# clintpgeorge/LDAGroupedGibbsSampler

Measured on AMD Instinct MI355X. Metric: M tokens sampled/sec (whole node) per Gibbs sweep at K=100, higher is better.
Workload: dtype f64

## Files before the change

### ldagroupedgibbssampler_amd/csrc/ggs_api.hip

```cpp
#include <hip/hip_runtime.h>

#include <algorithm>
#include <cmath>
#include <cstdio>
#include <cstdlib>
#include <cstring>
#include <new>
#include <string>
#include <vector>

#include "ggs_kernels.hpp"
#include "ggs_z_sliced.hpp"
#include "ggs_z_stream.hpp"
#include "ggs_exact_sum.hpp"
#include "ggs_z_pcgs.hpp"
#include "ggs_z_pcgs_wave.hpp"
#include "ggs_z_collapsed.hpp"
#include "ggs_phi_poisson.hpp"
#include "ggs_alias.hpp"
#include "ggs_z_spalias.hpp"
#include "ggs_loglik.hpp"
#include "ggs_heldout.hpp"
#include "ggs_exchange.hpp"
#include "ggs_corpus_lists.hpp"

using namespace ggs;

namespace {

const char *debug_env(const char *name) {
  static const bool enabled = [] { const char *e = std::getenv("GGS_DEBUG"); return e && std::atoi(e) == 1; }();
  return enabled ? std::getenv(name) : nullptr;
}

struct Knob {
  bool set = false;
  int v = 0;
  double f = 0;
  explicit Knob(const char *name) { if (const char *e = debug_env(name)) { set = true; v = std::atoi(e); f = std::atof(e); } }
  bool is(int x) const { return set && v == x; }
};
struct Knobs {
  Knob zkernel{"GGS_DEBUG_ZKERNEL"}, group{"GGS_DEBUG_GROUP"}, regck{"GGS_DEBUG_REGCK"}, tworows{"GGS_DEBUG_TWOROWS"}, wpc{"GGS_DEBUG_WPC"};
  Knob phi64{"GGS_DEBUG_PHI64"}, split{"GGS_DEBUG_SPLIT"}, hot{"GGS_DEBUG_HOT"}, tile{"GGS_DEBUG_TILE"};
  Knob warm{"GGS_DEBUG_WARM"}, warm_rows{"GGS_DEBUG_WARM_ROWS"}, warm_fill{"GGS_DEBUG_WARM_FILL"}, warm_cpw{"GGS_DEBUG_WARM_CPW"};
  Knob theta_b{"GGS_DEBUG_THETA_B"}, theta_wgs{"GGS_DEBUG_THETA_WGS"}, zparts{"GGS_DEBUG_ZPARTS"}, beside{"GGS_DEBUG_BESIDE"};
  Knob pcgs_wave{"GGS_DEBUG_PCGS_WAVE"}, pcgs_stream{"GGS_DEBUG_PCGS_STREAM"};
  Knob margin{"GGS_DEBUG_MARGIN"}, replays{"GGS_DEBUG_REPLAYS"}, chain{"GGS_DEBUG_CHAIN"}, guided{"GGS_DEBUG_GUIDED"};
  Knob no_overlap{"GGS_DEBUG_NO_OVERLAP"}, theta_main{"GGS_DEBUG_THETA_MAIN"}, gamma_queue{"GGS_DEBUG_GAMMA_QUEUE"};
};

constexpr int kThetaBlock = 256;

struct KernelLaunch {
  const void *fn = nullptr;
  int block = 64, lds = 0, per_cu = 0;
};
struct LaunchPlan {
  int32_t kernel = 0;
  bool sliced() const { return kernel == 1; }
  bool stream() const { return kernel >= 2; }
  KernelLaunch z;
  int32_t tile_tokens = 64;
  bool two_rows = false;
  KernelLaunch cold, hot, warm;
  bool f32 = false;
  bool split = true, split_forced = false;
  int32_t wave_lds = 0, ring_base = 0, hot_wave_lds = 0, warm_wave_lds = 0, hot_pitch = 0, Kp32 = 0;
  int32_t hot_cap = 0, warm_cap = 0, warm_docs = 0;
  int32_t warm_tiers_max = 3, warm_min_fill_pct = 40, warm_min_chunks_per_wave = 3;
  struct ZCfg { int32_t parts = 1, z_per_cu = 0, theta_docs = 0, theta_lds = 0, theta_lds_beside_z = 0; } cfg_plain, cfg_parts;
  bool parts_forced = false;
  KernelLaunch theta;
  int32_t theta_docs_main = 0, theta_lds_main = 0;
  KernelLaunch lane, wave, alias, spalias, serial;
  bool wave_forced = false;
  int32_t alias_wpb = 0;
  std::vector<const KernelLaunch *> all() const { return {&z, &cold, &hot, &warm, &theta, &lane, &wave, &alias, &spalias, &serial}; }
};

constexpr int kEvRing = 8;
struct Events {
  hipEvent_t e[6] = {nullptr, nullptr, nullptr, nullptr, nullptr, nullptr};
  hipEvent_t x[3] = {nullptr, nullptr, nullptr};
  hipEvent_t th0 = nullptr, th1 = nullptr;
  bool used_ahead = false, exchanged = false;
  bool e4_is_e3 = false;
  bool theta_on_main = false;
  bool light = false;
};

}

struct ggs_handle {
  int32_t K = 0, V = 0, Kp = 0, pitch16 = 0, device = 0;
  double beta = 0;
  std::vector<double> alpha;
  uint64_t seed = 0;
  int32_t flags = 0, phi_burn_in = 0, phi_thin = 1;
  int32_t iteration = 0;
  int32_t n_sampled_phi = 0;

  int64_t D = 0, N = 0, C = 0, S = 0, doc_base = 0, tok_base = 0, global_tokens = -1;
  bool have_corpus = false, have_phi = false, in_sweep = false;
  int32_t num_cus = 0;
  LaunchPlan plan;
  const LaunchPlan::ZCfg *cfg = nullptr;
  int32_t *d_chunk_doc1 = nullptr;
  double margin_scale = 1.0;
  double margin_scale32 = 1.0;

  hipStream_t stream = nullptr;
  int64_t *d_doc_ptr = nullptr, *d_chunk_start = nullptr;
  int32_t *d_tok = nullptr, *d_z = nullptr, *d_chunk_doc = nullptr, *d_chunk_len = nullptr;
  int32_t *d_ct_tok = nullptr, *d_ct_idx = nullptr, *d_ct_ip = nullptr, *d_c_docs = nullptr, *d_hot_words = nullptr;
  int64_t Cs = 0, Cc = 0;
  int32_t *d_order = nullptr;
  int64_t pcgs_order_len = 0;
  bool pcgs_wave = false;
  bool collapsed = false;
  bool polyaurn = false;
  int32_t pa_L = 0;
  double pa_t00 = 0;
  double *d_pa_table = nullptr;
  unsigned long long *d_pa_acc = nullptr;
  bool spalias = false;
  bool alias_stale = true;
  double *d_alias_ps = nullptr, *d_alias_tn = nullptr;
  int32_t *d_alias_a = nullptr;
  KernelLaunch sp_z;
  int32_t sp_cap = 0;
  uint64_t *d_lcg = nullptr;
  bool lcg_ready = false;
  int32_t num_hot = 0;
  int32_t *d_perm = nullptr, *d_inv_perm = nullptr, *d_zw = nullptr, *d_seg_word = nullptr, *d_seg_begin = nullptr;
  double *d_theta_next = nullptr;
  hipStream_t side = nullptr;
  hipStream_t side_hot = nullptr;
  hipEvent_t ev_hot_fork = nullptr, ev_hot_join = nullptr;
  bool theta_main = true, chain_on_side = false, theta_main_always = false;
  bool whole_sweep = false;
  hipEvent_t hot_fork_from = nullptr;
  hipEvent_t ev_chain_done = nullptr;
  bool z_split = true, z_split_tried = false;
  int32_t warm_tiers = 0, num_warm = 0, warm_rows_max = 0;
  int64_t Cw = 0, warm_chunks_max = 0;
  int32_t *d_wt_pack = nullptr, *d_w_docs = nullptr, *d_warm_words = nullptr;
  int32_t *d_ht_pack = nullptr, *d_h_docs = nullptr;
  int64_t *d_warm_meta = nullptr;
  bool overlap_theta = true;
  int32_t gamma_queue_cap = 1 << 20;
  std::vector<int64_t> part_doc, part_chunk;
  hipEvent_t ev_part[8] = {nullptr, nullptr, nullptr, nullptr, nullptr, nullptr, nullptr, nullptr};
  int64_t theta_ahead_iter = INT64_MIN;
  float *d_phiT32 = nullptr;
  unsigned long long *d_replays = nullptr;
  int64_t z_f32_launches = 0;
  double *d_alpha = nullptr, *d_theta = nullptr, *d_phiT = nullptr, *d_mag = nullptr, *d_tot = nullptr, *d_phi_mean = nullptr;
  int32_t *d_n_wk = nullptr, *d_n_k = nullptr;
  double *d_sum_pref = nullptr, *d_sum_fn = nullptr;
  int32_t sum_nseg = 0;
  bool exact_sum = true;
  bool sum_guided = true;
  const void *guess_src = nullptr;
  int32_t guess_cols = 0;
  uint32_t *d_status = nullptr;
  int64_t *d_test_ptr = nullptr;
  int32_t *d_test_tok = nullptr, *d_test_docs = nullptr;
  std::vector<int32_t> test_short, test_long, test_huge;
  void *d_heldout_spill = nullptr;
  size_t heldout_spill_bytes = 0;
  double *d_test_ll = nullptr;
  std::vector<int64_t> test_ptr;
  int64_t test_doc_base = 0;
  bool have_test = false;
  void *d_scratch = nullptr;
  size_t scratch_bytes = 0;

  Exchange *xg = nullptr;
  hipStream_t own_stream = nullptr;
  int32_t Ks = 0, Ksm = 0, k0 = 0;
  int64_t *d_koff = nullptr;
  int32_t *d_cnt_send = nullptr, *d_cnt_own = nullptr, *d_cnt_all = nullptr, *d_n_k_own = nullptr;
  double *d_phi_own = nullptr, *d_phi_all0 = nullptr, *d_phi_all1 = nullptr, *d_mag_own = nullptr;
  int32_t *d_krank = nullptr, *d_kcol = nullptr;
  int32_t seg_split = 0, v_split = 0;
  hipStream_t comm_stream = nullptr;
  hipEvent_t ev_half_drawn = nullptr, ev_half_gathered = nullptr;
  int32_t *d_hseg_word = nullptr, *d_hseg_begin = nullptr, *d_hseg_end = nullptr;
  int64_t HS = 0;
  int32_t detail_every = 4;
  bool force_detail = false;
  int64_t sweeps_enqueued = 0;
  bool have_frac = false;
  double frac[5] = {0, 0, 0, 0, 0};
  int32_t count_mode = 0;
  bool counted_sparse = false;
  bool in_group = false;
  int64_t *d_sp_count = nullptr;
  int32_t *d_sp_cnt32 = nullptr, *d_sp_all = nullptr;
  int32_t *d_sp_wg_count = nullptr;
  int64_t *d_sp_wg_off = nullptr;
  int64_t sp_wgs = 0;
  int32_t *d_sp_send = nullptr, *d_sp_recv = nullptr;
  size_t sp_send_cap = 0, sp_recv_cap = 0;
  int64_t sp_pairs_last = 0;
  bool hot_join_pending = false, hot_counted = false;
  bool z_counted = false;
  bool cnt_send_zeroed = false;
  bool z_counts_forced = false;
  bool z_counts = true;
  SliceMap smap{};
  bool counts_global = true;
  bool cnt_own_valid = false;
  bool n_k_valid = false;
  std::vector<ggs_handle *> group;

  std::vector<void **> owned;
  Events evs[kEvRing];
  int ev_head = 0, ev_pending = 0;
  ggs_timings tm{};
  std::string err;
};

namespace {

int set_err(ggs_handle *h, int code, const std::string &msg) {
  if (h) h->err = msg;
  return code;
}

#define HIP_TRY(h, expr)                                                                        \
  do {                                                                                          \
    hipError_t _e = (expr);                                                                     \
    if (_e != hipSuccess)                                                                       \
      return set_err((h), GGS_ERR_HIP, std::string(#expr) + ": " + hipGetErrorString(_e));      \
  } while (0)

int bind_device(ggs_handle *h) {
  HIP_TRY(h, hipSetDevice(h->device));
  return GGS_OK;
}

template <typename T>
int dev_alloc(ggs_handle *h, T **p, size_t count) {
  void **slot = reinterpret_cast<void **>(p);
  if (std::find(h->owned.begin(), h->owned.end(), slot) == h->owned.end()) h->owned.push_back(slot);
  if (*p) { (void)hipFree(*p); *p = nullptr; }
  HIP_TRY(h, hipMalloc(slot, std::max<size_t>(count, 1) * sizeof(T)));
  return GGS_OK;
}
template <typename T>
int upload(ggs_handle *h, T **p, const T *src, size_t count) {
  const int rc = dev_alloc(h, p, count);
  if (rc) return rc;
  if (count) HIP_TRY(h, hipMemcpy(*p, src, sizeof(T) * count, hipMemcpyHostToDevice));
  return GGS_OK;
}
template <typename T>
int upload(ggs_handle *h, T **p, const std::vector<T> &v) { return upload(h, p, v.data(), v.size()); }

hipError_t launch(const ggs_handle *h, const KernelLaunch &l, int64_t items, void **args, hipStream_t st, int table_lds = 0) {
  const int waves = l.block / 64;
  const int64_t grid = std::max<int64_t>(1, std::min<int64_t>((items + waves - 1) / waves, (int64_t)h->num_cus * l.per_cu));
  return hipLaunchKernel(l.fn, dim3((unsigned)grid), dim3((unsigned)l.block), args, (size_t)(l.lds + table_lds), st);
}

void build_poisson_table(double beta, int32_t L, std::vector<double> &T) {
  const int n = 2 * L;
  T.assign((size_t)L * n, 0.0);
  std::vector<double> S((size_t)n);
  for (int32_t c = 0; c < L; ++c) {
    const double lambda = beta + (double)c;
    double pj = std::exp(-lambda), acc = 0.0;
    for (int j = 0; j < n; ++j) {
      if (j > 0) pj = pj * lambda / (double)j;
      acc += pj;
      S[(size_t)j] = acc;
    }
    for (int j = 0; j < n - 1; ++j) T[(size_t)c * n + j] = S[(size_t)j] / S[(size_t)n - 1];
    T[(size_t)c * n + n - 1] = 1.0;
  }
}

int ensure_scratch(ggs_handle *h, size_t bytes) {
  if (h->scratch_bytes >= bytes) return GGS_OK;
  if (h->d_scratch) (void)hipFree(h->d_scratch);
  h->d_scratch = nullptr; h->scratch_bytes = 0;
  HIP_TRY(h, hipMalloc(&h->d_scratch, bytes));
  h->scratch_bytes = bytes;
  return GGS_OK;
}

int grid_for(int64_t n, int block, int per_thread = 1) {
  const int64_t want = (n + (int64_t)block * per_thread - 1) / ((int64_t)block * per_thread);
  return (int)std::max<int64_t>(1, std::min<int64_t>(want, 256 * 8));
}

int check_status(ggs_handle *h) {
  uint32_t st = 0;
  HIP_TRY(h, hipMemcpyAsync(&st, h->d_status, sizeof st, hipMemcpyDeviceToHost, h->stream));
  HIP_TRY(h, hipStreamSynchronize(h->stream));
  if (!st) return GGS_OK;
  HIP_TRY(h, hipMemsetAsync(h->d_status, 0, sizeof(uint32_t), h->stream));
  if (st & ST_INVALID_TOPIC)
    return set_err(h, GGS_ERR_INVALID_TOPIC, h->collapsed ? "SimpleLDA: New topic not sampled."  : "LDAGroupedGibbsSampler: Topic sampled is invalid!");
  if (st & ST_NEGATIVE_COUNT) return set_err(h, GGS_ERR_NEGATIVE_COUNT, "Negative count for topic (Invalid count!)");
  if (st & ST_BAD_SHAPE) return set_err(h, GGS_ERR_BAD_ARG, "alpha and beta must be strictly positive (gamma shape <= 0)");
// ... 276 lines not shown
  pp.rows_per_tile = (int32_t)std::max<int64_t>(1, std::min<int64_t>(rows, (want + Ks - 1) / Ks));
  const int64_t tiles = (rows + pp.rows_per_tile - 1) / pp.rows_per_tile;
  hipLaunchKernelGGL(phi_poisson_kernel, dim3((unsigned)std::min<int64_t>(tiles, (int64_t)h->num_cus * 2)), dim3(kPoissonThreads), (size_t)Ks * 12, h->stream, pp);
  HIP_TRY(h, hipGetLastError());
  return GGS_OK;
}
int phi_slice_poisson_totals(ggs_handle *h, int32_t Ks, double *tot, int32_t *n_k) {
  if (Ks <= 0) return GGS_OK;
  hipLaunchKernelGGL(phi_poisson_totals_kernel, dim3((unsigned)((Ks + 255) / 256)), dim3(256), 0, h->stream, h->d_pa_acc, Ks, tot, n_k);
  HIP_TRY(h, hipGetLastError());
  return GGS_OK;
}
int launch_phi_slice(ggs_handle *h, bool initial, const int32_t *cnt, int32_t cnt_pitch, int32_t Ks, int32_t k0, double *out, int32_t out_pitch,
                     double *mag, double *tot, int32_t *n_k, double *phi_mean) {
  if (Ks <= 0) return GGS_OK;
  int rc;
  if (h->polyaurn) {
    if ((rc = phi_slice_poisson(h, initial, cnt, cnt_pitch, Ks, k0, out, out_pitch, 0, h->sum_nseg, true)) || (rc = phi_slice_poisson_totals(h, Ks, tot, n_k)))
      return rc;
    hipLaunchKernelGGL(phi_normalise_polyaurn_kernel, dim3(grid_for((int64_t)Ks * h->V, 256, 2)), dim3(256), 0, h->stream, out, tot, Ks, out_pitch, h->V,
                       phi_mean, out == h->d_phiT ? h->d_phiT32 : nullptr, h->plan.Kp32);
    HIP_TRY(h, hipGetLastError());
    return GGS_OK;
  }
  if ((rc = launch_magnitude_on(h, cnt, cnt_pitch, Ks, mag, n_k)) || (rc = phi_slice_gamma(h, initial, cnt, cnt_pitch, Ks, k0, out, out_pitch, mag, 0, h->sum_nseg)) ||
      (rc = phi_slice_total(h, out, out_pitch, Ks, tot)))
    return rc;
  hipLaunchKernelGGL(phi_normalise_kernel, dim3(grid_for((int64_t)Ks * h->V, 256, 2)), dim3(256), 0, h->stream, out, tot, Ks, out_pitch, h->V, phi_mean,
                     out == h->d_phiT ? h->d_phiT32 : nullptr, h->plan.Kp32);
  HIP_TRY(h, hipGetLastError());
  return GGS_OK;
}

size_t half0_elems(const ggs_handle *h) { return (size_t)h->v_split * h->Ksm; }
size_t half1_elems(const ggs_handle *h) { return (size_t)(h->V - h->v_split) * h->Ksm + (size_t)h->Ksm; }
int phi_step_a(ggs_handle *h) { return exchange_reduce_scatter(h); }
int phi_step_a_clear(ggs_handle *h) { return h->seg_split > 0 ? GGS_OK : clear_send_buffer_if_dead(h, h->stream); }
int phi_step_b1(ggs_handle *h, bool initial) {
  int rc;
  if (h->polyaurn) {
    if ((rc = phi_slice_poisson(h, initial, h->d_cnt_own, h->Ksm, h->Ks, h->k0, h->d_phi_own, h->Ksm, 0, h->seg_split, true))) return rc;
  } else if ((rc = launch_magnitude_on(h, h->d_cnt_own, h->Ksm, h->Ks, h->d_mag_own, h->d_n_k_own))) {
    return rc;
  }
  if (h->seg_split > 0) {
    if (!h->polyaurn && (rc = phi_slice_gamma(h, initial, h->d_cnt_own, h->Ksm, h->Ks, h->k0, h->d_phi_own, h->Ksm, h->d_mag_own, 0, h->seg_split))) return rc;
    HIP_TRY(h, hipEventRecord(h->ev_half_drawn, h->stream));
    HIP_TRY(h, hipStreamWaitEvent(h->comm_stream, h->ev_half_drawn, 0));
  }
  return GGS_OK;
}
int phi_step_g0(ggs_handle *h) {
  if (h->seg_split <= 0) return GGS_OK;
  return xcall(h, h->xg->ops.all_gather_f64(h->xg->ops.ctx, h->d_phi_own, h->d_phi_all0, (int64_t)half0_elems(h), h->comm_stream), "all_gather_f64");
}
int phi_step_b2(ggs_handle *h, bool initial) {
  int rc;
  if (h->seg_split > 0) {
    if ((rc = clear_send_buffer_if_dead(h, h->comm_stream))) return rc;
    HIP_TRY(h, hipEventRecord(h->ev_half_gathered, h->comm_stream));
  }
  if (h->polyaurn) {
    if ((rc = phi_slice_poisson(h, initial, h->d_cnt_own, h->Ksm, h->Ks, h->k0, h->d_phi_own, h->Ksm, h->seg_split, h->sum_nseg, false))) return rc;
    return phi_slice_poisson_totals(h, h->Ks, h->d_phi_own + (size_t)h->V * h->Ksm, h->d_n_k_own);
  }
  if ((rc = phi_slice_gamma(h, initial, h->d_cnt_own, h->Ksm, h->Ks, h->k0, h->d_phi_own, h->Ksm, h->d_mag_own, h->seg_split, h->sum_nseg))) return rc;
  return phi_slice_total(h, h->d_phi_own, h->Ksm, h->Ks, h->d_phi_own + (size_t)h->V * h->Ksm);
}
int phi_step_g1(ggs_handle *h) {
  return xcall(h, h->xg->ops.all_gather_f64(h->xg->ops.ctx, h->d_phi_own + half0_elems(h), h->d_phi_all1, (int64_t)half1_elems(h), h->stream), "all_gather_f64");
}
int phi_join_halves(ggs_handle *h) {
  if (h->seg_split > 0) HIP_TRY(h, hipStreamWaitEvent(h->stream, h->ev_half_gathered, 0));
  return GGS_OK;
}
int phi_step_c(ggs_handle *h, bool accumulate_mean) {
  PhiRepackParams rp{};
  rp.all0 = h->d_phi_all0; rp.all1 = h->d_phi_all1; rp.krank = h->d_krank; rp.kcol = h->d_kcol; rp.phiT = h->d_phiT;
  rp.phi_mean = accumulate_mean ? h->d_phi_mean : nullptr;
  rp.c0 = (int64_t)half0_elems(h); rp.c1 = (int64_t)half1_elems(h); rp.K = h->K; rp.Kp = h->Kp; rp.V = h->V; rp.Ksm = h->Ksm; rp.v_split = h->v_split;
  rp.phiT32 = h->d_phiT32; rp.Kp32 = h->plan.Kp32;
  if (h->polyaurn) hipLaunchKernelGGL(phi_repack_polyaurn_kernel, dim3(grid_for((int64_t)h->K * h->V, 256, 2)), dim3(256), 0, h->stream, rp);
  else hipLaunchKernelGGL(phi_repack_kernel, dim3(grid_for((int64_t)h->K * h->V, 256, 2)), dim3(256), 0, h->stream, rp);
  HIP_TRY(h, hipGetLastError());
  h->have_phi = true;
  h->alias_stale = true;
  return GGS_OK;
}

int launch_alias_build(ggs_handle *h) {
  if (!h->spalias) return GGS_OK;
  AliasParams ap{};
  ap.phiT = h->d_phiT; ap.alpha = h->d_alpha; ap.ps = h->d_alias_ps; ap.a = h->d_alias_a; ap.type_norm = h->d_alias_tn;
  ap.V = h->V; ap.K = h->K; ap.Kp = h->Kp; ap.wpb = h->plan.alias_wpb;
  void *args[] = {&ap};
  HIP_TRY(h, launch(h, h->plan.alias, ((int64_t)h->V + ap.wpb - 1) / ap.wpb, args, h->stream));
  h->alias_stale = false;
  return GGS_OK;
}

int launch_phi(ggs_handle *h, bool initial, bool accumulate_mean, Events *E = nullptr) {
  int rc;
  if (h->xg) {
    if ((rc = phi_step_a(h)) || (rc = phi_step_a_clear(h))) return rc;
    if (E) HIP_TRY(h, hipEventRecord(E->x[0], h->stream));
    if ((rc = phi_step_b1(h, initial)) || (rc = phi_step_g0(h)) || (rc = phi_step_b2(h, initial))) return rc;
    if (E) HIP_TRY(h, hipEventRecord(E->x[1], h->stream));
    if ((rc = phi_join_halves(h)) || (rc = phi_step_g1(h))) return rc;
    if (E) HIP_TRY(h, hipEventRecord(E->x[2], h->stream));
    if ((rc = phi_step_c(h, accumulate_mean))) return rc;
    return launch_alias_build(h);
  }
  if ((rc = launch_phi_slice(h, initial, h->d_n_wk, h->K, h->K, 0, h->d_phiT, h->Kp, h->d_mag, h->d_tot, h->d_n_k, accumulate_mean ? h->d_phi_mean : nullptr)))
    return rc;
  h->n_k_valid = true;
  h->have_phi = true;
  return launch_alias_build(h);
}

int launch_theta(ggs_handle *h, hipStream_t stream, double *dst, int32_t iteration, int64_t d0 = 0, int64_t d1 = -1, int32_t lds = 0, int32_t docs_per_block = 0) {
  if (d1 < 0) d1 = h->D;
  if (d1 <= d0) return GGS_OK;
  if (docs_per_block <= 0) docs_per_block = h->cfg->theta_docs;
  ThetaParams tp{};
  tp.doc_ptr = h->d_doc_ptr + d0; tp.z = h->d_z; tp.alpha = h->d_alpha; tp.theta = dst + (size_t)d0 * h->K; tp.status = h->d_status;
  tp.num_docs = d1 - d0; tp.doc_base = h->doc_base + d0; tp.seed = h->seed; tp.iteration = (uint32_t)iteration;
  tp.K = h->K; tp.docs_per_block = docs_per_block; tp.queue_cap = std::min(kGammaQueue, h->gamma_queue_cap);
  const int64_t grid = (d1 - d0 + docs_per_block - 1) / docs_per_block;
  void *args[] = {&tp};
  HIP_TRY(h, hipLaunchKernel(h->plan.theta.fn, dim3((unsigned)grid), dim3(kThetaBlock), args, (size_t)(lds ? lds : h->cfg->theta_lds), stream));
  return GGS_OK;
}

#define GGS_KMAX_SWITCH(KERNEL)                                                                                                     \
  switch ((K + 7) / 8) {                                                                                                            \
    case 1: return reinterpret_cast<const void *>(KERNEL<8>);      case 2: return reinterpret_cast<const void *>(KERNEL<16>);       \
    case 3: return reinterpret_cast<const void *>(KERNEL<24>);     case 4: return reinterpret_cast<const void *>(KERNEL<32>);       \
    case 5: return reinterpret_cast<const void *>(KERNEL<40>);     case 6: return reinterpret_cast<const void *>(KERNEL<48>);       \
    case 7: return reinterpret_cast<const void *>(KERNEL<56>);     case 8: return reinterpret_cast<const void *>(KERNEL<64>);       \
    case 9: return reinterpret_cast<const void *>(KERNEL<72>);     case 10: return reinterpret_cast<const void *>(KERNEL<80>);      \
    case 11: return reinterpret_cast<const void *>(KERNEL<88>);    case 12: return reinterpret_cast<const void *>(KERNEL<96>);      \
    case 13: return reinterpret_cast<const void *>(KERNEL<104>);   case 14: return reinterpret_cast<const void *>(KERNEL<112>);     \
    case 15: return reinterpret_cast<const void *>(KERNEL<120>);   case 16: return reinterpret_cast<const void *>(KERNEL<128>);     \
    case 17: return reinterpret_cast<const void *>(KERNEL<136>);   case 18: return reinterpret_cast<const void *>(KERNEL<144>);     \
    case 19: return reinterpret_cast<const void *>(KERNEL<152>);   case 20: return reinterpret_cast<const void *>(KERNEL<160>);     \
    case 21: return reinterpret_cast<const void *>(KERNEL<168>);   case 22: return reinterpret_cast<const void *>(KERNEL<176>);     \
    case 23: return reinterpret_cast<const void *>(KERNEL<184>);   default: return reinterpret_cast<const void *>(KERNEL<192>);     \
  }
const void *sliced_kernel_for(int K) { GGS_KMAX_SWITCH(z_sliced_kernel) }
const void *sliced32_kernel_for(int K) { GGS_KMAX_SWITCH(z_sliced32_kernel) }

const void *hot_kernel_for(int K) { GGS_KMAX_SWITCH(z_hot_kernel) }
const void *warm_kernel_for(int K) { GGS_KMAX_SWITCH(z_warm_kernel) }
const void *pcgs_kernel_for(int K) { GGS_KMAX_SWITCH(pcgs_sliced_kernel) }
const void *polyaurn_kernel_for(int K) { GGS_KMAX_SWITCH(polyaurn_sliced_kernel) }
const void *collapsed_kernel_for(int K) {
  switch ((K + 7) / 8) {
#define GGS_CK(N) case N: return reinterpret_cast<const void *>(pcgs_sliced_kernel<8 * N, true>);
    GGS_CK(1) GGS_CK(2) GGS_CK(3) GGS_CK(4) GGS_CK(5) GGS_CK(6) GGS_CK(7) GGS_CK(8) GGS_CK(9) GGS_CK(10) GGS_CK(11) GGS_CK(12)
    GGS_CK(13) GGS_CK(14) GGS_CK(15) GGS_CK(16) GGS_CK(17) GGS_CK(18) GGS_CK(19) GGS_CK(20) GGS_CK(21) GGS_CK(22) GGS_CK(23)
#undef GGS_CK
    default: return reinterpret_cast<const void *>(pcgs_sliced_kernel<192, true>);
  }
}

const void *pcgs_wave_kernel_for(int nb, bool collapsed, bool polyaurn) {
#define GGS_WK(N) if (nb <= N) return polyaurn ? reinterpret_cast<const void *>(polyaurn_wave_kernel<N>) : collapsed ? reinterpret_cast<const void *>(pcgs_wave_kernel<N, true>) : reinterpret_cast<const void *>(pcgs_wave_kernel<N, false>);
  GGS_WK(1) GGS_WK(2) GGS_WK(4) GGS_WK(8) GGS_WK(16)
#undef GGS_WK
  return polyaurn ? reinterpret_cast<const void *>(polyaurn_wave_kernel<32>) : collapsed ? reinterpret_cast<const void *>(pcgs_wave_kernel<32, true>) : reinterpret_cast<const void *>(pcgs_wave_kernel<32, false>);
}
constexpr int kPcgsWaveMaxTopics = 32 * 128;
constexpr int kPcgsWaveFromTopics = 176, kCollapsedWaveFromTopics = 96;
constexpr int kPolyaurnWaveFromTopics = 168;

const void *tile_kernel_for(int K) {
  const int nt = (K + 63) / 64;
  return nt <= 1 ? reinterpret_cast<const void *>(z_kernel<1>) : nt <= 2 ? reinterpret_cast<const void *>(z_kernel<2>)
       : nt <= 4 ? reinterpret_cast<const void *>(z_kernel<4>) : nt <= 8 ? reinterpret_cast<const void *>(z_kernel<8>)
       : nt <= 16 ? reinterpret_cast<const void *>(z_kernel<16>) : reinterpret_cast<const void *>(z_kernel<20>);
}
const void *stream_kernel_for(bool two_pass, bool regck, int group) {
  if (two_pass) return reinterpret_cast<const void *>(z_stream_kernel);
  if (!regck) return reinterpret_cast<const void *>(z_stream1_kernel<false, 4>);
  return group == 1 ? reinterpret_cast<const void *>(z_stream1_kernel<true, 1>) : group == 2 ? reinterpret_cast<const void *>(z_stream1_kernel<true, 2>)
                                                                                             : reinterpret_cast<const void *>(z_stream1_kernel<true, 4>);
}
const void *pcgs_lane_kernel_for(int K, bool sliced, bool collapsed, bool polyaurn) {
  if (sliced) return collapsed ? collapsed_kernel_for(K) : polyaurn ? polyaurn_kernel_for(K) : pcgs_kernel_for(K);
  return collapsed ? reinterpret_cast<const void *>(pcgs_z_kernel<true>) : polyaurn ? reinterpret_cast<const void *>(polyaurn_z_kernel) : reinterpret_cast<const void *>(pcgs_z_kernel<false>);
}

int plan_launches(const int K, const int V, const int32_t flags, const Knobs &kn, LaunchPlan &pl) {
  const bool pcgs = (flags & GGS_FLAG_PCGS) != 0, collapsed = (flags & GGS_FLAG_COLLAPSED) != 0, polyaurn = (flags & GGS_FLAG_POLYAURN) != 0;
  const int Kp = (K + 1) & ~1, pitch16 = (Kp / 2) | 1;
  const bool sliced_ok = K <= kSlicedMaxTopics && V < (1 << kSlotShift);
  bool sliced = sliced_ok && K <= kSlicedDefaultTopics, stream = !sliced && K > 2 * kSliceTopics, two_pass = false;
  if (kn.zkernel.set) {
    const int mode = kn.zkernel.v;
    sliced = sliced_ok && mode == 1;
    stream = (mode == 2 || mode == 3) ? K > 2 * kSliceTopics : (stream && mode != 0);
    two_pass = mode == 3;
    if (sliced) stream = false;
  }
  pl.kernel = sliced ? 1 : stream ? (two_pass ? 3 : 2) : 0;
  if (stream) {
    const int ns = stream_slices(K);
    int group = ns <= kRegCheckpoints ? 1 : ns <= 2 * kRegCheckpoints ? 2 : 4;
    if (kn.group.set && (kn.group.v == 1 || kn.group.v == 2 || kn.group.v == 4)) group = kn.group.v;
    bool regck = !two_pass && z_stream1_groups(K, group) <= kRegCheckpoints;
    if (kn.regck.set) regck = regck && kn.regck.v != 0;
    if (!regck) group = 4;
    pl.two_rows = !two_pass && (kn.tworows.set ? kn.tworows.v != 0 : K <= 512);
    pl.z.fn = stream_kernel_for(two_pass, regck, group);
    pl.z.lds = two_pass ? z_stream_lds_bytes(K) : z_stream1_lds_bytes(K, group, pl.two_rows, regck);
    if (pl.z.lds > kMaxLdsBytes) return GGS_ERR_UNSUPPORTED;
  } else if (sliced) {
    pl.f32 = !kn.phi64.is(1);
    pl.Kp32 = round_up(K, kSlice32Topics);
    pl.ring_base = sliced_ring_base(K); pl.wave_lds = sliced_wave_lds(K); pl.hot_pitch = table_row_pitch(K);
    pl.hot_wave_lds = hot_wave_lds(K); pl.warm_wave_lds = warm_wave_lds(K);
    if (kn.split.set) { pl.split = kn.split.v != 0; pl.split_forced = kn.split.v == 2; }
    pl.hot_cap = pl.split ? table_rows_beside_cold(K, pl.hot_wave_lds) : table_rows_fused(K);
    if (kn.hot.set) pl.hot_cap = std::max(0, std::min(pl.hot_cap, kn.hot.v));
    pl.cold = {pl.f32 ? sliced32_kernel_for(K) : sliced_kernel_for(K), kSlicedWaves * 64, sliced_cold_lds(K), 1};
    pl.hot = {hot_kernel_for(K), kSlicedWaves * 64, table_lds(K, pl.hot_wave_lds, 0), 1};
    pl.warm = {warm_kernel_for(K), kSlicedWaves * 64, table_lds(K, pl.warm_wave_lds, 0), 1};
    pl.warm_docs = warm_docs_for(sliced_kmax(K));
    pl.warm_cap = table_rows_beside_cold(K, pl.warm_wave_lds);
    if (pl.warm_cap < 16) pl.warm_cap = 0;
    if (kn.warm.set) pl.warm_tiers_max = std::max(0, std::min(kWarmMaxTiers, kn.warm.v));
    if (kn.warm_rows.set) pl.warm_cap = std::max(0, std::min(pl.warm_cap, kn.warm_rows.v));
    if (kn.warm_fill.set) pl.warm_min_fill_pct = std::max(1, std::min(100, kn.warm_fill.v));
    if (kn.warm_cpw.set) pl.warm_min_chunks_per_wave = std::max(0, kn.warm_cpw.v);
  } else {
    int T = z_tile_rows_in(kMaxLdsBytes / 6 / kLdsGranule * kLdsGranule, Kp, pitch16);
    if (kn.tile.set) T = kn.tile.v;
    pl.tile_tokens = std::max(8, std::min(64, T));
    pl.z.fn = tile_kernel_for(K);
    pl.z.lds = z_tile_lds_bytes(Kp, pitch16, pl.tile_tokens);
    if (pl.z.lds > kMaxLdsBytes) return GGS_ERR_UNSUPPORTED;
  }
  if (!sliced) {
    pl.z.per_cu = lds_workgroups_per_cu(pl.z.lds, 8);
    if (kn.wpc.set) pl.z.per_cu = std::max(1, kn.wpc.v);
  }

  int B = 64;
  while (B > 1 && theta_lds_bytes(K, B) > 32 * 1024) B >>= 1;
  if (theta_lds_bytes(K, B) > kMaxLdsBytes) return GGS_ERR_UNSUPPORTED;
  pl.theta.fn = reinterpret_cast<const void *>(theta_kernel<kThetaBlock>); pl.theta.block = kThetaBlock;
  const int theta_quarter = (kMaxLdsBytes - 24 * 1024) / 4;
  pl.cfg_plain = {1, pl.z.per_cu, B, std::max(theta_lds_bytes(K, B), theta_quarter), 0};
  pl.theta_docs_main = kn.theta_b.set ? std::max(1, std::min(B, kn.theta_b.v)) : std::min(B, 16);
  pl.theta_lds_main = std::max(theta_lds_bytes(K, pl.theta_docs_main), (kMaxLdsBytes - 24 * 1024) / (kn.theta_wgs.set ? std::max(1, kn.theta_wgs.v) : 5));
  pl.parts_forced = kn.zparts.set;
  int parts = kn.zparts.set ? std::max(1, std::min(8, kn.zparts.v)) : (stream && !two_pass && !pcgs) ? 8 : 1;
  pl.cfg_parts = pl.cfg_plain;
  if (parts > 1 && stream && !two_pass) {
    const int kBeside = kn.beside.set ? std::max(1, kn.beside.v) : 4;
    int Bt = 64;
    while (Bt > 1 && theta_lds_bytes(K, Bt) > 10 * 1024) Bt >>= 1;
    const int t_lds = theta_lds_bytes(K, Bt), z_alloc = lds_alloc_of(pl.z.lds);
    const int zw = std::min(pl.z.per_cu, (kMaxLdsBytes - kLdsGranule - kBeside * lds_alloc_of(t_lds)) / z_alloc);
    if (t_lds <= 12 * 1024 && zw >= 2)
      pl.cfg_parts = {parts, zw, Bt, std::max(t_lds, theta_quarter), std::max(t_lds, (kMaxLdsBytes - kLdsGranule - zw * z_alloc) / kBeside / kLdsGranule * kLdsGranule)};
    else
      parts = 1;
  }
  pl.cfg_parts.parts = parts;
  if (!pcgs) return GGS_OK;

  if (K <= kPcgsWaveMaxTopics) {
    const int nb = pcgs_wave_blocks(Kp);
    pl.wave.fn = pcgs_wave_kernel_for(nb, collapsed, polyaurn);
    pl.wave.lds = pcgs_wave_lds_bytes(nb);
    int by_regs = 0;
    if (hipOccupancyMaxActiveBlocksPerMultiprocessor(&by_regs, pl.wave.fn, 64, (size_t)pl.wave.lds) != hipSuccess || by_regs < 1) by_regs = 1;
    pl.wave.per_cu = lds_workgroups_per_cu(pl.wave.lds, std::min(by_regs, 32));
  }
  pl.wave_forced = kn.pcgs_wave.set ? kn.pcgs_wave.v != 0 : K > (collapsed ? kCollapsedWaveFromTopics : polyaurn ? kPolyaurnWaveFromTopics : kPcgsWaveFromTopics);
  if (pl.wave_forced && !pl.wave.fn) return GGS_ERR_UNSUPPORTED;
  const bool lane_sliced = K <= kSlicedMaxTopics && !(kn.pcgs_stream.set && kn.pcgs_stream.v != 0);
  pl.lane.lds = lane_sliced ? pcgs_sliced_lds_bytes(K) : pcgs_z_lds_bytes(K);
  if (pl.lane.lds > kMaxLdsBytes && !pl.wave_forced) return GGS_ERR_UNSUPPORTED;
  pl.lane.per_cu = lds_workgroups_per_cu(pl.lane.lds, 8);
  if (!pl.wave_forced) pl.lane.fn = pcgs_lane_kernel_for(K, lane_sliced, collapsed, polyaurn);
  if (collapsed) pl.serial.fn = reinterpret_cast<const void *>(collapsed_serial_kernel);
  if (flags & GGS_FLAG_SPALIAS) {
    pl.alias_wpb = alias_words_per_block(K);
    pl.alias = {reinterpret_cast<const void *>(alias_build_kernel), 64, (int)alias_lds_bytes(K, pl.alias_wpb), 0};
    pl.alias.per_cu = lds_workgroups_per_cu(pl.alias.lds, 16);
    pl.spalias.fn = reinterpret_cast<const void *>(spalias_wave_kernel);
  }
  return GGS_OK;
}

int launch_pcgs_z(ggs_handle *h) {
  if (h->N == 0) return GGS_OK;
  PcgsParams pp{};
  pp.tok = h->d_tok; pp.inv_perm = h->d_inv_perm; pp.z = h->d_z; pp.zw = h->d_zw; pp.doc_ptr = h->d_doc_ptr; pp.order = h->d_order;
  pp.alpha = h->d_alpha; pp.phiT = h->d_phiT; pp.status = h->d_status;
  pp.num_docs = h->pcgs_order_len; pp.tok_base = h->tok_base; pp.seed = h->seed; pp.iteration = (uint32_t)h->iteration;
  pp.K = h->K; pp.Kp = h->Kp;
  int rc;
  if (h->spalias) {
    if (h->alias_stale && (rc = launch_alias_build(h))) return rc;
    SpaliasParams sp{};
    sp.b = pp; sp.ps = h->d_alias_ps; sp.a = h->d_alias_a; sp.type_norm = h->d_alias_tn; sp.cap = h->sp_cap; sp.margin_scale = h->margin_scale;
    void *args[] = {&sp};
    HIP_TRY(h, launch(h, h->sp_z, h->pcgs_order_len, args, h->stream));
    return GGS_OK;
  }
  if (h->collapsed) {
    if ((rc = launch_magnitude(h))) return rc;
    pp.n_wk = h->d_n_wk; pp.n_k = h->d_n_k; pp.beta = h->beta; pp.beta_sum = h->beta * (double)h->V;
    hipLaunchKernelGGL(psi_kernel, dim3(grid_for((int64_t)h->K * h->V, 256, 2)), dim3(256), 0, h->stream, h->d_n_wk, h->d_n_k, pp.beta, pp.beta_sum, h->d_phiT,
                       h->K, h->Kp, h->V);
    HIP_TRY(h, hipGetLastError());
  }
  void *wave_args[] = {&pp, &h->margin_scale}, *lane_args[] = {&pp};
  if (h->pcgs_wave) HIP_TRY(h, launch(h, h->plan.wave, h->pcgs_order_len, wave_args, h->stream));
  else HIP_TRY(h, launch(h, h->plan.lane, (h->pcgs_order_len + 63) / 64, lane_args, h->stream));
  return GGS_OK;
}

bool z_counts_itself(const ggs_handle *h) {
  return h->xg && h->z_counts && h->plan.sliced() && !(h->flags & GGS_FLAG_PCGS) && (h->z_counts_forced || h->N <= (int64_t)64 * h->V) && !use_sparse(h);
}
int launch_count_hot(ggs_handle *h);
int launch_z(ggs_handle *h, bool force_fused = false, int64_t c0 = 0, int64_t c1 = -1, bool count = false, bool defer_join = false) {
  h->hot_join_pending = false;
  if (h->C == 0) return GGS_OK;
  if (c1 < 0) c1 = h->C;
  if (c1 <= c0) return GGS_OK;
  const LaunchPlan &pl = h->plan;
  ZParams zp{};
  zp.tok = h->d_tok; zp.inv_perm = h->d_inv_perm; zp.z = h->d_z; zp.zw = h->d_zw; zp.chunk_start = h->d_chunk_start; zp.chunk_doc = h->d_chunk_doc; zp.chunk_len = h->d_chunk_len;
  zp.theta = h->d_theta; zp.phiT = h->d_phiT; zp.status = h->d_status;
  zp.tok_base = h->tok_base; zp.seed = h->seed; zp.iteration = (uint32_t)h->iteration;
  zp.K = h->K; zp.Kp = h->Kp; zp.pitch16 = h->pitch16; zp.tile_tokens = pl.tile_tokens;
  zp.num_chunks = h->C;
  zp.margin_scale = h->margin_scale;
  zp.chunk_doc1 = h->d_chunk_doc1; zp.two_rows = (pl.two_rows && h->d_chunk_doc1) ? 1 : 0;
  zp.ct_tok = h->d_ct_tok; zp.ct_idx = h->d_ct_idx; zp.ct_ip = h->d_ct_ip; zp.c_docs = h->d_c_docs; zp.num_cold = h->Cc;
  zp.hot_words = h->d_hot_words; zp.num_hot = h->num_hot; zp.hot_pitch = pl.hot_pitch;
  zp.wave_lds = pl.wave_lds; zp.hot_off = kSlicedWaves * pl.wave_lds; zp.ring_base = pl.ring_base;
  zp.cnt_send = (count && z_counts_itself(h)) ? h->d_cnt_send : nullptr;
  zp.smap = h->smap;
  zp.ht_pack = reinterpret_cast<const int4 *>(h->d_ht_pack); zp.h_docs = h->d_h_docs;
  zp.wt_pack = reinterpret_cast<const int4 *>(h->d_wt_pack); zp.w_docs = h->d_w_docs; zp.warm_words = h->d_warm_words;
  zp.warm_meta = h->d_warm_meta; zp.warm_tiers = h->warm_tiers; zp.warm_rows = pl.warm_cap;
  zp.phiT32 = h->d_phiT32; zp.Kp32 = pl.Kp32; zp.replays = h->d_replays; zp.margin_scale32 = h->margin_scale32;
  void *args[] = {&zp};
  if (!pl.sliced()) {
    zp.chunk_start += c0; zp.chunk_doc += c0; zp.chunk_len += c0; zp.num_chunks = c1 - c0;
    if (zp.chunk_doc1) zp.chunk_doc1 += c0;
    KernelLaunch z = pl.z;
    z.per_cu = h->cfg->z_per_cu;
    HIP_TRY(h, launch(h, z, zp.num_chunks, args, h->stream));
    return GGS_OK;
  }
  zp.num_chunks = h->Cs;
  const int hot_rows_lds = h->num_hot * pl.hot_pitch;
  ZParams wp = zp;
  wp.wave_lds = pl.warm_wave_lds; wp.hot_off = kSlicedWaves * pl.warm_wave_lds;
  void *wargs[] = {&wp};
  auto launch_warm = [&](hipStream_t st) { return h->Cw == 0 ? hipSuccess : launch(h, pl.warm, h->warm_chunks_max, wargs, st, h->warm_rows_max * pl.hot_pitch); };
  if (h->z_split && !force_fused && h->Cs > h->Cc && h->Cc > 0) {
    ZParams hp = zp;
    hp.wave_lds = pl.hot_wave_lds; hp.hot_off = kSlicedWaves * pl.hot_wave_lds;
    void *hargs[] = {&hp};
    if (h->hot_fork_from) {
      HIP_TRY(h, hipStreamWaitEvent(h->side_hot, h->hot_fork_from, 0));
    } else {
      HIP_TRY(h, hipEventRecord(h->ev_hot_fork, h->stream));
      HIP_TRY(h, hipStreamWaitEvent(h->side_hot, h->ev_hot_fork, 0));
    }
    zp.num_chunks = h->Cc; zp.num_hot = 0;
    HIP_TRY(h, launch(h, pl.cold, h->Cc, args, h->stream));
    HIP_TRY(h, launch(h, pl.hot, h->Cs - h->Cc, hargs, h->side_hot, hot_rows_lds));
    HIP_TRY(h, launch_warm(h->side_hot));
    if (defer_join && zp.cnt_send) {
      hipStream_t main_stream = h->stream;
      h->stream = h->side_hot;
      const int rc = launch_count_hot(h);
      h->stream = main_stream;
      if (rc) return rc;
      h->hot_counted = true;
    }
    HIP_TRY(h, hipEventRecord(h->ev_hot_join, h->side_hot));
    if (defer_join) h->hot_join_pending = true;
    else HIP_TRY(h, hipStreamWaitEvent(h->stream, h->ev_hot_join, 0));
  } else {
    HIP_TRY(h, launch(h, pl.cold, std::max(h->Cc, h->Cs - h->Cc), args, h->stream, hot_rows_lds));
    HIP_TRY(h, launch_warm(h->stream));
  }
  if (pl.f32) ++h->z_f32_launches;
  return GGS_OK;
}

bool sample_phi_this_iteration(const ggs_handle *h) {
  return h->phi_burn_in > 0 && h->iteration > h->phi_burn_in && (h->iteration % h->phi_thin) == 0;
}

uint64_t java_lcg_next_ints(int32_t seed, int32_t bound, int64_t n, int32_t *out) {
  constexpr uint64_t kMult = 0x5DEECE66DULL, kMask = (1ULL << 48) - 1;
  uint64_t s = ((uint64_t)(int64_t)seed ^ kMult) & kMask;
  auto next31 = [&]() { s = (s * kMult + 0xBULL) & kMask; return (int32_t)(s >> 17); };
  const int32_t m = bound - 1;
  for (int64_t i = 0; i < n; ++i) {
    int32_t r = next31();
    if ((bound & m) == 0) r = (int32_t)(((int64_t)bound * (int64_t)r) >> 31);
    else
      for (int32_t u = r;; u = next31()) {
        r = u % bound;
        if ((int32_t)((uint32_t)u - (uint32_t)r + (uint32_t)m) >= 0) break;
      }
    out[i] = r;
  }
  return s;
}

int require_ready(ggs_handle *h, bool need_phi) {
  if (!h) return GGS_ERR_BAD_ARG;
  if (!h->have_corpus) return set_err(h, GGS_ERR_STATE, "no corpus: call ggs_set_corpus first");
  if (need_phi && !h->have_phi) return set_err(h, GGS_ERR_STATE, "no Phi: call ggs_init_phi / ggs_set_z / ggs_set_phi first");
  return bind_device(h);
}

int drop_theta_ahead(ggs_handle *h) {
  if (h->side) HIP_TRY(h, hipStreamSynchronize(h->side));
  h->theta_ahead_iter = INT64_MIN;
  return GGS_OK;
}

int settle_sweeps(ggs_handle *h) {
  HIP_TRY(h, hipStreamSynchronize(h->stream));
  for (int j = h->ev_pending - 1; j >= 0; --j) {
    const Events &E = h->evs[((h->ev_head - j) % kEvRing + kEvRing) % kEvRing];
    float ms = 0;
    if (E.used_ahead && E.theta_on_main) { HIP_TRY(h, hipEventElapsedTime(&ms, h->evs[((h->ev_head - j - 1) % kEvRing + kEvRing) % kEvRing].e[2], E.th1)); }
    else if (E.used_ahead) { HIP_TRY(h, hipEventElapsedTime(&ms, E.th0, E.th1)); }
    else { HIP_TRY(h, hipEventElapsedTime(&ms, E.e[0], E.e[1])); }
    h->tm.theta_ms += ms;
    HIP_TRY(h, hipEventElapsedTime(&ms, E.e[1], E.e[2])); h->tm.z_ms += ms;
    if (E.light) {
      HIP_TRY(h, hipEventElapsedTime(&ms, E.e[2], E.e[5]));
      h->tm.merge_ms += ms * h->frac[0];
      h->tm.exchange_rs_ms += ms * h->frac[1]; h->tm.exchange_ag_ms += ms * h->frac[3]; h->tm.exchange_ms += ms * (h->frac[1] + h->frac[3]);
      h->tm.phi_ms += ms * (h->frac[2] + h->frac[4]);
      h->tm.sweeps += 1;
      h->tm.tokens_sampled += h->N;
      continue;
    }
    HIP_TRY(h, hipEventElapsedTime(&ms, E.e[2], E.e[3])); h->tm.merge_ms += ms;
    if (E.exchanged) {
      float span = 0, part[5] = {ms, 0, 0, 0, 0};
      (void)hipEventElapsedTime(&span, E.e[2], E.e[5]);
      (void)hipEventElapsedTime(&part[1], E.e[E.e4_is_e3 ? 3 : 4], E.x[0]); (void)hipEventElapsedTime(&part[2], E.x[0], E.x[1]);
      (void)hipEventElapsedTime(&part[3], E.x[1], E.x[2]); (void)hipEventElapsedTime(&part[4], E.x[2], E.e[5]);
      if (span > 0) {
        const float sum = part[0] + part[1] + part[2] + part[3] + part[4];
        for (int q = 0; q < 5; ++q) h->frac[q] = sum > 0 ? part[q] / sum : 0.0;
        h->have_frac = true;
      }
      HIP_TRY(h, hipEventElapsedTime(&ms, E.e[E.e4_is_e3 ? 3 : 4], E.x[0])); h->tm.exchange_ms += ms; h->tm.exchange_rs_ms += ms;
      HIP_TRY(h, hipEventElapsedTime(&ms, E.x[0], E.x[1])); h->tm.phi_ms += ms;
      HIP_TRY(h, hipEventElapsedTime(&ms, E.x[1], E.x[2])); h->tm.exchange_ms += ms; h->tm.exchange_ag_ms += ms;
      HIP_TRY(h, hipEventElapsedTime(&ms, E.x[2], E.e[5])); h->tm.phi_ms += ms;
    } else {
      HIP_TRY(h, hipEventElapsedTime(&ms, E.e[E.e4_is_e3 ? 3 : 4], E.e[5])); h->tm.phi_ms += ms;
    }
    h->tm.sweeps += 1;
    h->tm.tokens_sampled += h->N;
  }
  h->ev_pending = 0;
  return GGS_OK;
}

struct StreamSwap {
  ggs_handle *h;
  hipStream_t user;
  StreamSwap(ggs_handle *h_, hipStream_t s) : h(h_), user(h_->stream) { h->stream = s; }
  ~StreamSwap() { h->stream = user; }
};

int z_phase(ggs_handle *h) {
  int rc;
  if (h->ev_pending >= kEvRing - 2 && (rc = settle_sweeps(h))) return rc;
  h->ev_head = (h->ev_head + 1) % kEvRing;
  Events &E = h->evs[h->ev_head];
  E.light = h->xg && h->have_frac && h->detail_every > 1 && !h->force_detail && (h->sweeps_enqueued % h->detail_every) != 0 && !h->collapsed;
  h->sweeps_enqueued += 1;
  if (h->flags & GGS_FLAG_PCGS) {
    E.used_ahead = false;
    HIP_TRY(h, hipEventRecord(E.e[0], h->stream));
    HIP_TRY(h, hipEventRecord(E.e[1], h->stream));
    if ((rc = launch_pcgs_z(h))) return rc;
    HIP_TRY(h, hipEventRecord(E.e[2], h->stream));
    if ((rc = launch_count_rebuild(h))) return rc;
    if (!E.light) HIP_TRY(h, hipEventRecord(E.e[3], h->stream));
    return GGS_OK;
  }
  E.used_ahead = h->theta_ahead_iter == (int64_t)h->iteration;
  h->hot_fork_from = nullptr;
  if (E.used_ahead) {
    if (E.theta_on_main) h->hot_fork_from = E.th1;
    else HIP_TRY(h, hipStreamWaitEvent(h->stream, E.th1, 0));
    std::swap(h->d_theta, h->d_theta_next);
  } else {
    E.theta_on_main = false;
    if (h->side) HIP_TRY(h, hipStreamSynchronize(h->side));
    HIP_TRY(h, hipEventRecord(E.e[0], h->stream));
    if ((rc = launch_theta(h, h->stream, h->d_theta, h->iteration))) return rc;
  }
  HIP_TRY(h, hipEventRecord(E.e[1], h->stream));
  if (h->plan.sliced() && h->z_split && !h->z_split_tried && h->Cs > h->Cc && h->Cc > 0) {
    h->z_split_tried = true;
    float t_split = 0, t_fused = 0;
    hipEvent_t t0 = nullptr, t1 = nullptr, t2 = nullptr;
    if (hipEventCreate(&t0) != hipSuccess || hipEventCreate(&t1) != hipSuccess || hipEventCreate(&t2) != hipSuccess) return set_err(h, GGS_ERR_HIP, "hipEventCreate");
    if ((rc = launch_z(h, false)) || (rc = launch_z(h, true))) return rc;
    HIP_TRY(h, hipEventRecord(t0, h->stream));
    if ((rc = launch_z(h, false))) return rc;
    HIP_TRY(h, hipEventRecord(t1, h->stream));
    if ((rc = launch_z(h, true))) return rc;
    HIP_TRY(h, hipEventRecord(t2, h->stream));
    HIP_TRY(h, hipEventSynchronize(t2));
    HIP_TRY(h, hipEventElapsedTime(&t_split, t0, t1));
    HIP_TRY(h, hipEventElapsedTime(&t_fused, t1, t2));
    (void)hipEventDestroy(t0); (void)hipEventDestroy(t1); (void)hipEventDestroy(t2);
    if (t_fused < t_split) h->z_split = false;
    HIP_TRY(h, hipEventRecord(E.e[1], h->stream));
  }
  if (!h->hot_fork_from) h->hot_fork_from = E.e[1];
  h->theta_ahead_iter = INT64_MIN;
  const bool ahead = h->overlap_theta && h->side && h->D > 0;
  const int32_t P = (int32_t)h->part_doc.size() - 1;
  if (ahead && P > 1 && h->plan.stream()) {
    Events &N = h->evs[(h->ev_head + 1) % kEvRing];
    for (int32_t p = 0; p < P; ++p) {
      if ((rc = launch_z(h, false, h->part_chunk[(size_t)p], h->part_chunk[(size_t)p + 1]))) return rc;
      HIP_TRY(h, hipEventRecord(h->ev_part[p], h->stream));
      HIP_TRY(h, hipStreamWaitEvent(h->side, h->ev_part[p], 0));
      if (p == 0) { N.theta_on_main = false; HIP_TRY(h, hipEventRecord(N.th0, h->side)); }
      if ((rc = launch_theta(h, h->side, h->d_theta_next, h->iteration + 1, h->part_doc[(size_t)p], h->part_doc[(size_t)p + 1],
                             p + 1 < P ? h->cfg->theta_lds_beside_z : 0)))
        return rc;
// ... 114 lines not shown
  }
  std::vector<int64_t> koff((size_t)h->K);
  for (int32_t r = 0; r < x->nranks; ++r)
    for (int32_t k = sl[(size_t)r]; k < sl[(size_t)r + 1]; ++k) koff[(size_t)k] = (int64_t)r * h->V * h->Ksm + (k - sl[(size_t)r]);
  std::vector<int32_t> krank((size_t)h->K), kcol((size_t)h->K);
  for (int32_t r = 0; r < x->nranks; ++r)
    for (int32_t k = sl[(size_t)r]; k < sl[(size_t)r + 1]; ++k) { krank[(size_t)k] = r; kcol[(size_t)k] = k - sl[(size_t)r]; }
  h->seg_split = h->sum_nseg >= 16 ? h->sum_nseg / 2 : 0;
  if (const char *e = debug_env("GGS_DEBUG_AGSPLIT")) h->seg_split = std::max(0, std::min(h->sum_nseg - 1, std::atoi(e)));
  h->v_split = h->seg_split * kSumSegRows;
  const size_t slice = (size_t)h->V * h->Ksm, all = slice * (size_t)x->nranks;
  auto fail = [&](int code) {
    void *bufs[] = {h->d_koff, h->d_krank, h->d_kcol, h->d_cnt_send, h->d_cnt_own, h->d_phi_own, h->d_phi_all0, h->d_phi_all1, h->d_mag_own, h->d_n_k_own};
    for (void *b : bufs) if (b) (void)hipFree(b);
    h->d_koff = nullptr; h->d_krank = h->d_kcol = nullptr; h->d_cnt_send = h->d_cnt_own = nullptr; h->d_phi_own = h->d_phi_all0 = h->d_phi_all1 = nullptr;
    h->d_mag_own = nullptr; h->d_n_k_own = nullptr;
    h->xg = nullptr; h->Ks = h->Ksm = h->K; h->k0 = 0;
    exchange_free(x);
    return code;
  };
  if ((rc = dev_alloc(h, &h->d_koff, (size_t)h->K)) || (rc = dev_alloc(h, &h->d_krank, (size_t)h->K)) || (rc = dev_alloc(h, &h->d_kcol, (size_t)h->K)) ||
      (rc = dev_alloc(h, &h->d_cnt_send, all)) || (rc = dev_alloc(h, &h->d_cnt_own, slice)) || (rc = dev_alloc(h, &h->d_phi_own, slice + (size_t)h->Ksm)) ||
      (rc = dev_alloc(h, &h->d_phi_all0, half0_elems(h) * (size_t)x->nranks)) || (rc = dev_alloc(h, &h->d_phi_all1, half1_elems(h) * (size_t)x->nranks)) ||
      (rc = dev_alloc(h, &h->d_mag_own, (size_t)h->Ksm)) || (rc = dev_alloc(h, &h->d_n_k_own, (size_t)h->Ksm)))
    return fail(rc);
  if (hipMemcpy(h->d_koff, koff.data(), sizeof(int64_t) * koff.size(), hipMemcpyHostToDevice) != hipSuccess ||
      hipMemcpy(h->d_krank, krank.data(), sizeof(int32_t) * krank.size(), hipMemcpyHostToDevice) != hipSuccess ||
      hipMemcpy(h->d_kcol, kcol.data(), sizeof(int32_t) * kcol.size(), hipMemcpyHostToDevice) != hipSuccess ||
      hipMemset(h->d_cnt_send, 0, all * sizeof(int32_t)) != hipSuccess || hipMemset(h->d_cnt_own, 0, slice * sizeof(int32_t)) != hipSuccess ||
      hipMemset(h->d_phi_own, 0, (slice + (size_t)h->Ksm) * sizeof(double)) != hipSuccess ||
      hipMemset(h->d_phi_all0, 0, std::max<size_t>(half0_elems(h) * (size_t)x->nranks, 1) * sizeof(double)) != hipSuccess ||
      hipMemset(h->d_phi_all1, 0, half1_elems(h) * (size_t)x->nranks * sizeof(double)) != hipSuccess)
    return fail(set_err(h, GGS_ERR_HIP, "exchange buffers: copy / memset failed"));
  {
    int lo = 0, hi = 0;
    (void)hipDeviceGetStreamPriorityRange(&lo, &hi);
    if (hipStreamCreateWithPriority(&h->comm_stream, hipStreamNonBlocking, hi) != hipSuccess ||
        hipEventCreateWithFlags(&h->ev_half_drawn, hipEventDisableTiming) != hipSuccess ||
        hipEventCreateWithFlags(&h->ev_half_gathered, hipEventDisableTiming) != hipSuccess)
      return fail(set_err(h, GGS_ERR_HIP, "exchange: communication stream / events"));
  }
  if (!h->stream) {
    if (!(debug_env("GGS_DEBUG_OWN_STREAM") && std::atoi(debug_env("GGS_DEBUG_OWN_STREAM")) == 0)) {
      int lo = 0, hi = 0;
      (void)hipDeviceGetStreamPriorityRange(&lo, &hi);
      HIP_TRY(h, hipStreamCreateWithPriority(&h->own_stream, hipStreamNonBlocking, hi));
      h->stream = h->own_stream;
    }
  }
  HIP_TRY(h, hipDeviceSynchronize());
  h->counts_global = false; h->cnt_own_valid = false; h->n_k_valid = false;
  h->cnt_send_zeroed = true;
  return GGS_OK;
}

Exchange *new_rccl_exchange(ggs_handle *h, int32_t rank, int32_t nranks, int *rc) {
  std::string err;
  RcclApi *api = RcclApi::get(err);
  if (!api) { *rc = set_err(h, GGS_ERR_UNSUPPORTED, err); return nullptr; }
  auto *x = new (std::nothrow) Exchange();
  if (!x) { *rc = GGS_ERR_HIP; return nullptr; }
  x->rank = rank; x->nranks = nranks; x->api = api;
  x->ops.struct_size = (int32_t)sizeof(ggs_exchange_ops); x->ops.ctx = x;
  x->ops.reduce_scatter_i32 = xops::rccl_reduce_scatter_i32;
  x->ops.all_gather_f64 = xops::rccl_all_gather_f64;
  x->ops.all_gather_i32 = xops::rccl_all_gather_i32;
  x->ops.all_to_all_v_i32 = (api->Send && api->Recv) ? xops::rccl_all_to_all_v_i32 : nullptr;
  *rc = GGS_OK;
  return x;
}

template <typename Step>
int group_collective(ggs_handle **hs, int32_t n, Step step) {
  RcclApi *api = hs[0]->xg->api;
  int r = GGS_OK;
  if (api) api->GroupStart();
  for (int32_t i = 0; i < n && !r; ++i)
    if (!(r = bind_device(hs[i]))) r = step(hs[i]);
  if (api && api->GroupEnd() != ncclSuccess && !r) r = set_err(hs[0], GGS_ERR_HIP, "ncclGroupEnd failed");
  return r;
}

}

extern "C" {

int ggs_abi_version(void) { return GGS_ABI_VERSION; }

const char *ggs_last_error(const ggs_handle *h) { return h ? h->err.c_str() : "null handle"; }

int ggs_create(const ggs_config *cfg, ggs_handle **out) {
  if (!cfg || !out) return GGS_ERR_BAD_ARG;
  *out = nullptr;
  if (cfg->struct_size != (int32_t)sizeof(ggs_config)) return GGS_ERR_BAD_ARG;
  if (cfg->num_topics <= 0 || cfg->num_types <= 0 || !(cfg->beta > 0)) return GGS_ERR_BAD_ARG;
  if ((cfg->flags & GGS_FLAG_SPALIAS) && (cfg->flags & (GGS_FLAG_COLLAPSED | GGS_FLAG_POLYAURN))) return GGS_ERR_BAD_ARG;
  int ndev = 0;
  if (hipGetDeviceCount(&ndev) != hipSuccess || ndev <= 0 || cfg->device_id < 0 || cfg->device_id >= ndev) return GGS_ERR_HIP;
  ggs_handle *h = new (std::nothrow) ggs_handle();
  if (!h) return GGS_ERR_HIP;
  const Knobs kn;
  h->K = cfg->num_topics; h->V = cfg->num_types; h->device = cfg->device_id;
  h->Ks = h->Ksm = h->K; h->k0 = 0;
  h->Kp = (h->K + 1) & ~1;
  h->pitch16 = (h->Kp / 2) | 1;
  h->beta = cfg->beta; h->seed = cfg->seed; h->flags = cfg->flags;
  if (h->flags & GGS_FLAG_COLLAPSED) { h->collapsed = true; h->flags |= GGS_FLAG_PCGS; }
  if (h->flags & GGS_FLAG_POLYAURN) {
    const int32_t L = cfg->alias_poisson_threshold == 0 ? 100 : cfg->alias_poisson_threshold;
    if (h->collapsed || L < 1 || L > kPoissonMaxThreshold) { delete h; return GGS_ERR_BAD_ARG; }
    h->polyaurn = true; h->flags |= GGS_FLAG_PCGS; h->pa_L = L;
  }
  if (h->flags & GGS_FLAG_SPALIAS) {
    if (h->K > kPcgsWaveMaxTopics) { delete h; return GGS_ERR_UNSUPPORTED; }
    h->spalias = true; h->flags |= GGS_FLAG_PCGS;
  }
  h->phi_burn_in = cfg->phi_burn_in; h->phi_thin = cfg->phi_mean_thin > 0 ? cfg->phi_mean_thin : 1;
  h->alpha.assign(h->K, cfg->alpha_scalar);
  if (cfg->alpha) std::copy(cfg->alpha, cfg->alpha + h->K, h->alpha.begin());
  for (double a : h->alpha)
    if (!(a > 0)) { delete h; return GGS_ERR_BAD_ARG; }
  if (kn.margin.set) { h->margin_scale = std::max(1.0, kn.margin.f); h->margin_scale32 = std::max(0.0, kn.margin.f); }
  if (kn.chain.set) h->exact_sum = kn.chain.v == 0;
  if (kn.guided.set) h->sum_guided = kn.guided.v != 0;
  if (kn.no_overlap.set) h->overlap_theta = kn.no_overlap.v == 0;
  if (kn.theta_main.set) { h->theta_main = kn.theta_main.v != 0; h->theta_main_always = kn.theta_main.v == 2; }
  if (kn.gamma_queue.set) h->gamma_queue_cap = std::max(0, kn.gamma_queue.v);
  h->sum_nseg = (h->V + kSumSegRows - 1) / kSumSegRows;

  int rc = GGS_OK;
  auto bail = [&](int code) { ggs_destroy(h); return code; };
  if (hipSetDevice(h->device) != hipSuccess) return bail(GGS_ERR_HIP);
  {
    hipDeviceProp_t prop;
    if (hipGetDeviceProperties(&prop, h->device) != hipSuccess) return bail(GGS_ERR_HIP);
    h->num_cus = prop.multiProcessorCount > 0 ? prop.multiProcessorCount : 256;
  }
  if ((rc = plan_launches(h->K, h->V, h->flags, kn, h->plan))) return bail(rc);
  h->cfg = &h->plan.cfg_parts;
  h->z_split = h->plan.split;
  for (const KernelLaunch *l : h->plan.all())
    if (l->fn && hipFuncSetAttribute(l->fn, hipFuncAttributeMaxDynamicSharedMemorySize, kMaxLdsBytes) != hipSuccess) return bail(GGS_ERR_HIP);
  const size_t kv = (size_t)h->K * h->V, phi_elems = (size_t)h->V * h->Kp + kPhiTailPadBytes / 8;
  if ((rc = dev_alloc(h, &h->d_alpha, h->K)) || (rc = dev_alloc(h, &h->d_phiT, phi_elems)) ||
      (rc = dev_alloc(h, &h->d_mag, h->K)) || (rc = dev_alloc(h, &h->d_tot, h->K)) || (rc = dev_alloc(h, &h->d_n_wk, kv)) ||
      (rc = dev_alloc(h, &h->d_n_k, h->K)) || (rc = dev_alloc(h, &h->d_status, 4)))
    return bail(rc);
  if ((h->flags & GGS_FLAG_SAVE_PHI_MEAN) && (rc = dev_alloc(h, &h->d_phi_mean, kv))) return bail(rc);
  if (h->plan.sliced() && h->plan.f32) {
    const size_t n32 = (size_t)h->V * h->plan.Kp32 + kPhiTailPadBytes / 4;
    if ((rc = dev_alloc(h, &h->d_phiT32, n32))) return bail(rc);
    if (hipMemset(h->d_phiT32, 0, sizeof(float) * n32) != hipSuccess) return bail(GGS_ERR_HIP);
    if (kn.replays.is(1)) {
      if ((rc = dev_alloc(h, &h->d_replays, 1))) return bail(rc);
      if (hipMemset(h->d_replays, 0, sizeof(unsigned long long)) != hipSuccess) return bail(GGS_ERR_HIP);
    }
  }
  if (h->exact_sum && ((rc = dev_alloc(h, &h->d_sum_pref, ((size_t)h->sum_nseg + 1) * h->K)) ||
                       (rc = dev_alloc(h, &h->d_sum_fn, (size_t)h->sum_nseg * h->K * 4))))
    return bail(rc);
  if (hipMemcpy(h->d_alpha, h->alpha.data(), sizeof(double) * h->K, hipMemcpyHostToDevice) != hipSuccess ||
      hipMemset(h->d_phiT, 0, sizeof(double) * phi_elems) != hipSuccess ||
      hipMemset(h->d_n_wk, 0, sizeof(int32_t) * kv) != hipSuccess ||
      hipMemset(h->d_n_k, 0, sizeof(int32_t) * h->K) != hipSuccess || hipMemset(h->d_status, 0, 16) != hipSuccess ||
      (h->d_phi_mean && hipMemset(h->d_phi_mean, 0, sizeof(double) * kv) != hipSuccess))
    return bail(GGS_ERR_HIP);
  if (h->spalias && ((rc = dev_alloc(h, &h->d_alias_ps, kv)) || (rc = dev_alloc(h, &h->d_alias_a, kv)) || (rc = dev_alloc(h, &h->d_alias_tn, (size_t)h->V)))) return bail(rc);
  if (h->polyaurn) {
    std::vector<double> T;
    build_poisson_table(h->beta, h->pa_L, T);
    h->pa_t00 = T[0];
    if ((rc = upload(h, &h->d_pa_table, T)) || (rc = dev_alloc(h, &h->d_pa_acc, (size_t)h->K * kPoissonAccStride))) return bail(rc);
  }
  if (h->collapsed && (rc = dev_alloc(h, &h->d_lcg, 2))) return bail(rc);
  for (auto &e : h->ev_part)
    if (hipEventCreateWithFlags(&e, hipEventDisableTiming) != hipSuccess) return bail(GGS_ERR_HIP);
  for (auto &E : h->evs) {
    for (auto &e : E.e)
      if (hipEventCreate(&e) != hipSuccess) return bail(GGS_ERR_HIP);
    for (auto &e : E.x)
      if (hipEventCreate(&e) != hipSuccess) return bail(GGS_ERR_HIP);
    if (hipEventCreate(&E.th0) != hipSuccess || hipEventCreate(&E.th1) != hipSuccess) return bail(GGS_ERR_HIP);
  }
  {
    int lo = 0, hi = 0;
    (void)hipDeviceGetStreamPriorityRange(&lo, &hi);
    if (hipStreamCreateWithPriority(&h->side, hipStreamNonBlocking, lo) != hipSuccess) return bail(GGS_ERR_HIP);
    if (hipStreamCreateWithPriority(&h->side_hot, hipStreamNonBlocking, hi) != hipSuccess || hipEventCreate(&h->ev_hot_fork) != hipSuccess ||
        hipEventCreate(&h->ev_hot_join) != hipSuccess || hipEventCreateWithFlags(&h->ev_chain_done, hipEventDisableTiming) != hipSuccess)
      return bail(GGS_ERR_HIP);
  }
  if (hipDeviceSynchronize() != hipSuccess) return bail(GGS_ERR_HIP);
  *out = h;
  return GGS_OK;
}

void ggs_destroy(ggs_handle *h) {
  if (!h) return;
  (void)hipSetDevice(h->device);
  (void)hipDeviceSynchronize();
  if (h->d_replays) {
    unsigned long long n = 0;
    if (hipMemcpy(&n, h->d_replays, sizeof(n), hipMemcpyDeviceToHost) == hipSuccess)
      fprintf(stderr, "[ggs] z replays: %llu tokens in %lld launches of z_sliced32_kernel (%.2f per launch)\n", n, (long long)h->z_f32_launches,
              h->z_f32_launches ? (double)n / (double)h->z_f32_launches : 0.0);
  }
  for (void **slot : h->owned)
    if (*slot) (void)hipFree(*slot);
  if (h->d_scratch) (void)hipFree(h->d_scratch);
  if (h->d_heldout_spill) (void)hipFree(h->d_heldout_spill);
  exchange_free(h->xg);
  if (h->own_stream) (void)hipStreamDestroy(h->own_stream);
  if (h->comm_stream) (void)hipStreamDestroy(h->comm_stream);
  if (h->ev_half_drawn) (void)hipEventDestroy(h->ev_half_drawn);
  if (h->ev_half_gathered) (void)hipEventDestroy(h->ev_half_gathered);
  for (auto &e : h->ev_part)
    if (e) (void)hipEventDestroy(e);
  for (auto &E : h->evs) {
    for (auto &e : E.e)
      if (e) (void)hipEventDestroy(e);
    for (auto &e : E.x)
      if (e) (void)hipEventDestroy(e);
    if (E.th0) (void)hipEventDestroy(E.th0);
    if (E.th1) (void)hipEventDestroy(E.th1);
  }
  if (h->side) (void)hipStreamDestroy(h->side);
  if (h->side_hot) (void)hipStreamDestroy(h->side_hot);
  if (h->ev_hot_fork) (void)hipEventDestroy(h->ev_hot_fork);
  if (h->ev_hot_join) (void)hipEventDestroy(h->ev_hot_join);
  if (h->ev_chain_done) (void)hipEventDestroy(h->ev_chain_done);
  delete h;
}

int ggs_set_stream(ggs_handle *h, void *hip_stream) {
  if (!h) return GGS_ERR_BAD_ARG;
  int rc = bind_device(h);
  if (rc) return rc;
  HIP_TRY(h, hipStreamSynchronize(h->stream));
  if ((rc = drop_theta_ahead(h))) return rc;
  if (h->xg && !hip_stream) return set_err(h, GGS_ERR_BAD_ARG, "with an exchange attached the handle does not run on the legacy default stream");
  h->stream = reinterpret_cast<hipStream_t>(hip_stream);
  return GGS_OK;
}

int ggs_set_corpus(ggs_handle *h, int64_t D, const int64_t *doc_ptr, const int32_t *tokens, int64_t doc_base, int64_t tok_base) {
  if (!h || D < 0 || !doc_ptr || doc_base < 0 || tok_base < 0) return set_err(h, GGS_ERR_BAD_ARG, "bad corpus arguments");
  if (doc_ptr[0] != 0) return set_err(h, GGS_ERR_BAD_ARG, "doc_ptr[0] must be 0");
  for (int64_t d = 0; d < D; ++d)
    if (doc_ptr[d + 1] < doc_ptr[d]) return set_err(h, GGS_ERR_BAD_ARG, "doc_ptr must be non-decreasing");
  const int64_t N = doc_ptr[D];
  if (N > 0 && !tokens) return set_err(h, GGS_ERR_BAD_ARG, "tokens is null");
  if (N >= (int64_t)1 << 31 || D >= (int64_t)1 << 31) return set_err(h, GGS_ERR_UNSUPPORTED, "more than 2^31-1 tokens or documents per device");
  for (int64_t i = 0; i < N; ++i)
    if (tokens[i] < 0 || tokens[i] >= h->V) return set_err(h, GGS_ERR_BAD_ARG, "token id outside [0, num_types)");
  int rc = bind_device(h);
  if (rc) return rc;
  if ((rc = drop_theta_ahead(h))) return rc;

  const LaunchPlan &pl = h->plan;
  int32_t parts = pl.cfg_parts.parts;
  if (!pl.parts_forced && parts > 1) parts = D <= (int64_t)h->V ? 1 : D < 2 * (int64_t)h->V ? std::min(parts, 4) : parts;
  h->cfg = parts > 1 ? &pl.cfg_parts : &pl.cfg_plain;

  CorpusShape shape;
  shape.V = h->V; shape.pcgs = (h->flags & GGS_FLAG_PCGS) != 0; shape.sliced = pl.sliced(); shape.two_rows = pl.two_rows;
  shape.tile_tokens = pl.tile_tokens; shape.z_parts = parts;
  shape.hot_cap = pl.hot_cap; shape.warm_cap = pl.warm_cap; shape.warm_docs = pl.warm_docs;
  shape.warm_tiers_max = pl.warm_tiers_max; shape.warm_min_fill_pct = pl.warm_min_fill_pct; shape.warm_min_chunks_per_wave = pl.warm_min_chunks_per_wave;
  shape.sliced_waves = (int64_t)h->num_cus * kSlicedWaves; shape.pcgs_waves = (int64_t)h->num_cus * pl.lane.per_cu;
  const CorpusLists L = build_corpus_lists(shape, D, doc_ptr, tokens);
  if (shape.pcgs) {
    h->pcgs_wave = pl.wave_forced || L.longest > kPcgsMaxDocLen;
    if (h->pcgs_wave && !pl.wave.fn) return set_err(h, GGS_ERR_UNSUPPORTED, "scheme=pcgs: a document of 32768 tokens or more with more than 4096 topics");
    if (h->spalias) {
      h->sp_cap = (int32_t)std::max<int64_t>(1, std::min<int64_t>(h->K, L.longest));
      h->sp_z = pl.spalias;
      h->sp_z.lds = (int)spalias_lds_bytes(h->K, h->sp_cap);
      h->sp_z.per_cu = lds_workgroups_per_cu(h->sp_z.lds, 32);
      if (const char *e = debug_env("GGS_DEBUG_SPALIAS_WPC")) h->sp_z.per_cu = std::max(1, std::min(h->sp_z.per_cu, std::atoi(e)));
    }
  }
  h->D = D; h->N = N; h->C = (int64_t)L.cstart.size(); h->S = (int64_t)L.seg_word.size(); h->doc_base = doc_base; h->tok_base = tok_base;
  h->part_doc = L.part_doc; h->part_chunk = L.part_chunk;
  h->pcgs_order_len = (int64_t)L.order.size();
  h->num_hot = (int32_t)L.hot_words.size(); h->HS = (int64_t)L.hseg_word.size();
  h->Cc = L.Cc; h->Cs = L.Cs;
  h->warm_tiers = L.warm_tiers; h->num_warm = L.num_warm; h->Cw = L.Cw; h->warm_chunks_max = L.warm_chunks_max; h->warm_rows_max = L.warm_rows_max;

  const size_t theta_elems = (size_t)D * h->K + 2;
  if ((rc = upload(h, &h->d_doc_ptr, doc_ptr, (size_t)D + 1)) || (rc = upload(h, &h->d_tok, tokens, (size_t)N)) ||
      (rc = upload(h, &h->d_chunk_start, L.cstart)) || (rc = upload(h, &h->d_chunk_doc, L.cdoc)) || (rc = upload(h, &h->d_chunk_len, L.clen)) ||
      (pl.two_rows && h->C && (rc = upload(h, &h->d_chunk_doc1, L.cdoc1))) ||
      (rc = upload(h, &h->d_perm, L.perm)) || (rc = upload(h, &h->d_inv_perm, L.inv)) ||
      (rc = upload(h, &h->d_seg_word, L.seg_word)) || (rc = upload(h, &h->d_seg_begin, L.seg_begin)) ||
      (rc = upload(h, &h->d_hseg_word, L.hseg_word)) || (rc = upload(h, &h->d_hseg_begin, L.hseg_begin)) || (rc = upload(h, &h->d_hseg_end, L.hseg_end)) ||
      (shape.pcgs && (rc = upload(h, &h->d_order, L.order))))
    return rc;
  if (pl.sliced() && ((rc = upload(h, &h->d_ct_tok, L.ct_tok)) || (rc = upload(h, &h->d_ct_idx, L.ct_idx)) || (rc = upload(h, &h->d_ct_ip, L.ct_ip)) ||
                      (rc = upload(h, &h->d_c_docs, L.c_docs)) || (rc = upload(h, &h->d_hot_words, L.hot_words)) ||
                      (rc = upload(h, &h->d_ht_pack, L.ht_pack)) || (rc = upload(h, &h->d_h_docs, L.h_docs))))
    return rc;
  if (L.warm_tiers > 0 && ((rc = upload(h, &h->d_wt_pack, L.wt_pack)) || (rc = upload(h, &h->d_w_docs, L.w_docs)) ||
                           (rc = upload(h, &h->d_warm_words, L.warm_words)) || (rc = upload(h, &h->d_warm_meta, L.warm_meta))))
    return rc;
  if ((rc = dev_alloc(h, &h->d_z, (size_t)N)) || (rc = dev_alloc(h, &h->d_zw, (size_t)N)) ||
      (rc = dev_alloc(h, &h->d_theta, theta_elems)) || (rc = dev_alloc(h, &h->d_theta_next, theta_elems)))
    return rc;
  HIP_TRY(h, hipMemset(h->d_z, 0, sizeof(int32_t) * std::max<size_t>((size_t)N, 1)));
  HIP_TRY(h, hipMemset(h->d_zw, 0, sizeof(int32_t) * std::max<size_t>((size_t)N, 1)));
  HIP_TRY(h, hipMemset(h->d_theta, 0, sizeof(double) * std::max<size_t>((size_t)D * h->K, 1)));
  HIP_TRY(h, hipMemset(h->d_theta_next, 0, sizeof(double) * std::max<size_t>((size_t)D * h->K, 1)));
  HIP_TRY(h, hipDeviceSynchronize());

  h->have_corpus = true; h->have_phi = false; h->in_sweep = false; h->global_tokens = -1; h->lcg_ready = false;
  h->z_split = pl.split; h->z_split_tried = pl.split_forced;
  h->counts_global = h->xg == nullptr; h->cnt_own_valid = false; h->n_k_valid = false;
  return GGS_OK;
}

int ggs_init_z_java_lcg(ggs_handle *h, int32_t seed) {
  int rc = require_ready(h, false);
  if (rc) return rc;
  if (h->tok_base != 0) return set_err(h, GGS_ERR_STATE, "java-LCG init is one sequential stream: only valid with tok_base == 0");
  if ((rc = drop_theta_ahead(h))) return rc;
  std::vector<int32_t> z((size_t)h->N);
  const uint64_t lcg_state = java_lcg_next_ints(seed, h->K, h->N, z.data());
  if (h->collapsed) {
    HIP_TRY(h, hipMemcpyAsync(h->d_lcg, &lcg_state, sizeof lcg_state, hipMemcpyHostToDevice, h->stream));
    h->lcg_ready = true;
  }
  if (h->N) HIP_TRY(h, hipMemcpyAsync(h->d_z, z.data(), sizeof(int32_t) * (size_t)h->N, hipMemcpyHostToDevice, h->stream));
  if ((rc = launch_permute_z(h))) return rc;
  if ((rc = launch_count_rebuild(h))) return rc;
  HIP_TRY(h, hipStreamSynchronize(h->stream));
  return GGS_OK;
}

int ggs_set_z(ggs_handle *h, const int32_t *z, int32_t redraw_phi) {
  int rc = require_ready(h, false);
  if (rc) return rc;
  if (h->N > 0 && !z) return set_err(h, GGS_ERR_BAD_ARG, "z is null");
  for (int64_t i = 0; i < h->N; ++i)
    if (z[i] < 0 || z[i] >= h->K) return set_err(h, GGS_ERR_BAD_ARG, "topic indicator outside [0, num_topics)");
  if ((rc = drop_theta_ahead(h))) return rc;
  h->lcg_ready = false;
  if (h->N) HIP_TRY(h, hipMemcpyAsync(h->d_z, z, sizeof(int32_t) * (size_t)h->N, hipMemcpyHostToDevice, h->stream));
  if ((rc = launch_permute_z(h))) return rc;
  if ((rc = launch_count_rebuild(h))) return rc;
  HIP_TRY(h, hipStreamSynchronize(h->stream));
  if (redraw_phi) return ggs_init_phi(h);
  return GGS_OK;
}

int ggs_init_phi(ggs_handle *h) {
  int rc = require_ready(h, false);
  if (rc) return rc;
  if (h->collapsed) {
    if ((rc = launch_magnitude(h))) return rc;
    h->have_phi = true;
    return check_status(h);
  }
  if ((rc = launch_phi(h, true, false))) return rc;
  return check_status(h);
}

int ggs_set_iteration(ggs_handle *h, int32_t it) { if (!h) return GGS_ERR_BAD_ARG; h->iteration = it; return GGS_OK; }
int ggs_get_iteration(const ggs_handle *h, int32_t *it) { if (!h || !it) return GGS_ERR_BAD_ARG; *it = h->iteration; return GGS_OK; }

bool chain_on_side_ok(const ggs_handle *h) {
  return h->theta_main && h->plan.sliced() && h->side_hot && h->ev_chain_done && !h->xg && !h->collapsed && !(h->flags & GGS_FLAG_PCGS) &&
         (h->D >= (int64_t)h->V || h->theta_main_always);
}

int ggs_sweep_begin(ggs_handle *h) {
  int rc = require_ready(h, true);
  if (rc) return rc;
  if (h->in_sweep) return set_err(h, GGS_ERR_STATE, "ggs_sweep_begin called twice without ggs_sweep_end");
  h->iteration += 1;
  h->chain_on_side = chain_on_side_ok(h);
  if ((rc = z_phase(h))) { h->chain_on_side = false; return rc; }
  h->in_sweep = true;
  return GGS_OK;
}

int ggs_sweep_end(ggs_handle *h) {
  int rc = require_ready(h, true);
  if (rc) return rc;
  if (!h->in_sweep) return set_err(h, GGS_ERR_STATE, "ggs_sweep_end without ggs_sweep_begin");
  h->in_sweep = false;
  rc = finish_sweep(h, true);
  h->chain_on_side = false;
  return rc;
}

int ggs_sweep_end_async(ggs_handle *h) {
  int rc = require_ready(h, true);
  if (rc) return rc;
  if (!h->in_sweep) return set_err(h, GGS_ERR_STATE, "ggs_sweep_end_async without ggs_sweep_begin");
  h->in_sweep = false;
  rc = finish_sweep(h, true, false);
  h->chain_on_side = false;
  return rc;
}

int ggs_sweep(ggs_handle *h, int32_t n_sweeps) {
  for (int32_t i = 0; i < n_sweeps; ++i) {
    if (h) h->whole_sweep = true;
    int rc = ggs_sweep_begin(h);
    if (!rc) {
      h->in_sweep = false;
      rc = finish_sweep(h, true, i == n_sweeps - 1);
    }
    if (h) h->chain_on_side = h->whole_sweep = false;
    if (rc) return rc;
  }
  return GGS_OK;
}

int ggs_collapsed_serial_sweep(ggs_handle *h, int32_t java_seed, int32_t n_sweeps) {
  int rc = require_ready(h, false);
  if (rc) return rc;
  if (!h->collapsed) return set_err(h, GGS_ERR_STATE, "ggs_collapsed_serial_sweep needs GGS_FLAG_COLLAPSED");
  if (h->xg || h->tok_base != 0) return set_err(h, GGS_ERR_STATE, "the serial chain runs over ONE unsharded corpus");
  if (h->in_sweep) return set_err(h, GGS_ERR_STATE, "inside a split sweep");
  if ((size_t)h->K * 16 > (size_t)kMaxLdsBytes) return set_err(h, GGS_ERR_UNSUPPORTED, "num_topics too large for the serial kernel's LDS");
  if ((rc = launch_magnitude(h))) return rc;
  if (!h->lcg_ready) {
    const uint64_t st = ((uint64_t)(int64_t)java_seed ^ 0x5DEECE66DULL) & ((1ULL << 48) - 1);
    HIP_TRY(h, hipMemcpyAsync(h->d_lcg, &st, sizeof st, hipMemcpyHostToDevice, h->stream));
    HIP_TRY(h, hipStreamSynchronize(h->stream));
    h->lcg_ready = true;
  }
  CollapsedSerialParams cp{};
  cp.doc_ptr = h->d_doc_ptr; cp.tok = h->d_tok; cp.inv_perm = h->d_inv_perm; cp.z = h->d_z; cp.zw = h->d_zw; cp.n_wk = h->d_n_wk; cp.n_k = h->d_n_k;
  cp.alpha = h->d_alpha; cp.lcg = h->d_lcg; cp.status = h->d_status; cp.num_docs = h->D; cp.beta = h->beta; cp.beta_sum = h->beta * (double)h->V; cp.K = h->K;
  for (int32_t i = 0; i < n_sweeps; ++i) {
    h->iteration += 1;
    hipLaunchKernelGGL(collapsed_serial_kernel, dim3(1), dim3(64), (size_t)h->K * 16, h->stream, cp);
  }
  HIP_TRY(h, hipGetLastError());
  h->have_phi = true;
  return check_status(h);
}

int ggs_sample_z_given_phi(ggs_handle *h, int32_t n_sweeps) {
  int rc = require_ready(h, true);
  if (rc) return rc;
  if (h->in_sweep) return set_err(h, GGS_ERR_STATE, "inside a split sweep");
  if (h->collapsed) return set_err(h, GGS_ERR_UNSUPPORTED, "scheme=collapsed has no Phi to condition on");
  for (int32_t i = 0; i < n_sweeps; ++i) {
    h->iteration += 1;
    h->force_detail = true;
    rc = z_phase(h);
    h->force_detail = false;
// ... 495 lines not shown
  }
  h->test_doc_base = doc_base;
  h->have_test = true;
  return GGS_OK;
}

int ggs_heldout_log_likelihood(ggs_handle *h, int32_t num_particles, double *doc_ll, double *total) {
  int rc = require_ready(h, false);
  if (rc) return rc;
  if (!h->have_test) return set_err(h, GGS_ERR_STATE, "no test set: call ggs_set_test_corpus first");
  if (num_particles < 1 || !total) return set_err(h, GGS_ERR_BAD_ARG, "num_particles < 1 or null output");
  if ((rc = launch_magnitude(h))) return rc;
  const int K = h->K;
  const int64_t D = (int64_t)h->test_ptr.size() - 1;
  const size_t Kpad = (size_t)(K + 63) / 64 * 64;
  auto lds_of = [&](int w, int cnt_bytes, int cap) { return (size_t)(16 + 8 * cap) * K + (size_t)w * (Kpad * 8 + (size_t)K * 64 * cnt_bytes); };
  struct Shape { int waves = 0, per_cu = 0, cap = 0; };
  auto shape_for = [&](int cnt_bytes, int cap) {
    Shape s; s.cap = cap;
    for (int w = kHeldoutMaxWaves; w >= 1; w >>= 1) {
      const size_t alloc = (lds_of(w, cnt_bytes, cap) + 2047) / 2048 * 2048;
      const int per_cu = alloc <= (size_t)160 * 1024 ? std::min((int)((size_t)160 * 1024 / alloc) * w, 32) : 0;
      if (per_cu && per_cu >= s.per_cu) { s.per_cu = per_cu; s.waves = w; }
    }
    return s;
  };
  auto best_shape = [&](int cnt_bytes) {
    const int n_caps = (int)(sizeof(kHeldoutCoefCaps) / sizeof(kHeldoutCoefCaps[0]));
    const Shape floor = shape_for(cnt_bytes, kHeldoutCoefCaps[n_caps - 1]);
    for (int i = 0; i < n_caps; ++i) {
      const Shape s = shape_for(cnt_bytes, kHeldoutCoefCaps[i]);
      if (s.per_cu && s.per_cu >= floor.per_cu) return s;
    }
    return floor;
  };
  const Shape shape8 = best_shape(1), shape16 = best_shape(2), shape_spill = best_shape(0);
  const bool spill8 = !h->test_short.empty() && !shape8.waves, spill16 = !h->test_long.empty() && !shape16.waves, spill32 = !h->test_huge.empty();
  if ((spill8 || spill16 || spill32) && !shape_spill.waves)
    return set_err(h, GGS_ERR_UNSUPPORTED, "num_topics too large for the held-out estimator's tables in LDS (about 6000 topics)");
  const int64_t spill_blocks = (int64_t)h->num_cus * std::max(1, shape_spill.waves ? shape_spill.per_cu / shape_spill.waves : 1);
  if (spill8 || spill16 || spill32) {
    const size_t need = (size_t)spill_blocks * shape_spill.waves * (size_t)K * 64 * (spill32 ? 4 : spill16 ? 2 : 1);
    if (h->heldout_spill_bytes < need) {
      if (h->d_heldout_spill) (void)hipFree(h->d_heldout_spill);
      h->d_heldout_spill = nullptr; h->heldout_spill_bytes = 0;
      HIP_TRY(h, hipMalloc(&h->d_heldout_spill, need));
      h->heldout_spill_bytes = need;
    }
  }
  const void *kernels[] = {reinterpret_cast<const void *>(heldout_particles_kernel<uint8_t, false>), reinterpret_cast<const void *>(heldout_particles_kernel<uint16_t, false>),
                           reinterpret_cast<const void *>(heldout_particles_kernel<uint8_t, true>), reinterpret_cast<const void *>(heldout_particles_kernel<uint16_t, true>),
                           reinterpret_cast<const void *>(heldout_particles_kernel<uint32_t, true>)};
  for (const void *f : kernels) HIP_TRY(h, hipFuncSetAttribute(f, hipFuncAttributeMaxDynamicSharedMemorySize, kMaxLdsBytes));
  int64_t want_cells = (int64_t)1 << 29;
  if (const char *e = debug_env("GGS_DEBUG_HELDOUT_CELLS")) want_cells = std::max<int64_t>(1, std::atoll(e));
  int64_t longest = 1;
  for (int64_t d = 0; d < D; ++d) longest = std::max(longest, h->test_ptr[d + 1] - h->test_ptr[d]);
  const int64_t cap_cells = std::max<int64_t>(want_cells, longest * num_particles);
  int64_t max_cells = 0;
  std::vector<int64_t> cuts{0};
  for (int64_t d = 0; d < D;) {
    int64_t e = d;
    while (e < D && (h->test_ptr[e + 1] - h->test_ptr[d]) * num_particles <= cap_cells) ++e;
    max_cells = std::max(max_cells, (h->test_ptr[e] - h->test_ptr[d]) * num_particles);
    cuts.push_back(e);
    d = e;
  }
  const size_t tab_bytes = sizeof(double) * (size_t)(2 * K + 2);
  if ((rc = ensure_scratch(h, tab_bytes + sizeof(double) * (size_t)std::max<int64_t>(max_cells, 1)))) return rc;
  HeldoutParams hp{};
  hp.doc_ptr = h->d_test_ptr; hp.tok = h->d_test_tok; hp.n_wk = h->d_n_wk;
  auto *tab = static_cast<double *>(h->d_scratch);
  hp.tab = tab; hp.probs = tab + 2 * K + 2; hp.doc_ll = h->d_test_ll; hp.status = h->d_status;
  hp.beta = h->beta;
  double alpha_sum = 0;
  for (int k = 0; k < K; ++k) alpha_sum += h->alpha[k];
  hp.alpha_sum = alpha_sum;
  hp.seed = h->seed; hp.iteration = (uint32_t)h->iteration; hp.doc_base = h->test_doc_base;
  hp.K = K; hp.V = h->V; hp.P = num_particles; hp.blocks_per_doc = (num_particles + 63) / 64;
  hipLaunchKernelGGL(heldout_setup_kernel, dim3(1), dim3(64), 0, h->stream, h->d_alpha, h->d_n_k, h->beta, h->beta * h->V, K, tab);
  for (size_t b = 0; b + 1 < cuts.size(); ++b) {
    hp.d0 = cuts[b]; hp.d1 = cuts[b + 1];
    if (hp.d1 == hp.d0) continue;
    auto range = [&](const std::vector<int32_t> &ids, size_t &lo, size_t &hi) {
      lo = std::lower_bound(ids.begin(), ids.end(), (int32_t)hp.d0) - ids.begin();
      hi = std::lower_bound(ids.begin(), ids.end(), (int32_t)hp.d1) - ids.begin();
    };
    struct Class { const std::vector<int32_t> *ids; size_t offset; int bytes; bool spill; Shape shape; };
    const Class classes[] = {{&h->test_short, 0, 1, spill8, spill8 ? shape_spill : shape8},
                             {&h->test_long, h->test_short.size(), 2, spill16, spill16 ? shape_spill : shape16},
                             {&h->test_huge, h->test_short.size() + h->test_long.size(), 4, true, shape_spill}};
    for (const Class &c : classes) {
      size_t lo, hi;
      range(*c.ids, lo, hi);
      if (hi <= lo) continue;
      hp.docs = h->d_test_docs + c.offset + lo; hp.n_docs = (int64_t)(hi - lo); hp.waves = c.shape.waves; hp.cap = c.shape.cap;
      hp.cnt_spill = c.spill ? h->d_heldout_spill : nullptr;
      const int64_t units = hp.n_docs * hp.blocks_per_doc, blocks = (units + hp.waves - 1) / hp.waves;
      const dim3 grid((unsigned)(c.spill ? std::min(blocks, spill_blocks) : blocks)), block((unsigned)(hp.waves * 64));
      const size_t lds = lds_of(hp.waves, c.spill ? 0 : c.bytes, hp.cap);
      const void *f = c.spill ? (c.bytes == 1 ? kernels[2] : c.bytes == 2 ? kernels[3] : kernels[4]) : (c.bytes == 1 ? kernels[0] : kernels[1]);
      void *args[] = {&hp};
      HIP_TRY(h, hipLaunchKernel(f, grid, block, args, lds, h->stream));
    }
    hipLaunchKernelGGL(heldout_reduce_kernel, dim3((unsigned)((hp.d1 - hp.d0 + 3) / 4)), dim3(256), 0, h->stream, hp);
  }
  HIP_TRY(h, hipGetLastError());
  std::vector<double> ll((size_t)D);
  if (D) HIP_TRY(h, hipMemcpyAsync(ll.data(), h->d_test_ll, sizeof(double) * (size_t)D, hipMemcpyDeviceToHost, h->stream));
  if ((rc = check_status(h))) return rc;
  double t = 0;
  for (int64_t d = 0; d < D; ++d) t += ll[(size_t)d];
  *total = t;
  if (doc_ll && D) std::memcpy(doc_ll, ll.data(), sizeof(double) * (size_t)D);
  return GGS_OK;
}

int ggs_get_timings(ggs_handle *h, ggs_timings *out) { if (!h || !out) return GGS_ERR_BAD_ARG; *out = h->tm; return GGS_OK; }
int ggs_reset_timings(ggs_handle *h) { if (!h) return GGS_ERR_BAD_ARG; h->tm = ggs_timings{}; return GGS_OK; }

int ggs_check_invariants(ggs_handle *h) {
  int rc = require_ready(h, false);
  if (rc) return rc;
  const int K = h->K;
  const size_t bytes = 16 + sizeof(int32_t) * (size_t)K;
  if ((rc = ensure_global_counts(h))) return rc;
  if ((rc = ensure_scratch(h, bytes))) return rc;
  auto *d_total = static_cast<unsigned long long *>(h->d_scratch);
  auto *d_flags = reinterpret_cast<uint32_t *>(static_cast<char *>(h->d_scratch) + 8);
  auto *d_col = reinterpret_cast<int32_t *>(static_cast<char *>(h->d_scratch) + 16);
  HIP_TRY(h, hipMemsetAsync(h->d_scratch, 0, bytes, h->stream));
  const int64_t kv = (int64_t)K * h->V;
  hipLaunchKernelGGL(invariants_kernel, dim3(grid_for(kv, 256)), dim3(256), 0, h->stream, h->d_n_wk, kv, K, d_total, d_col, d_flags);
  HIP_TRY(h, hipGetLastError());
  if ((rc = launch_magnitude(h))) return rc;
  std::vector<unsigned char> host(bytes);
  std::vector<int32_t> nk((size_t)K);
  if ((rc = copy_out(h, host.data(), h->d_scratch, bytes))) return rc;
  if ((rc = copy_out(h, nk.data(), h->d_n_k, sizeof(int32_t) * (size_t)K))) return rc;
  unsigned long long total; uint32_t fl;
  std::memcpy(&total, host.data(), 8); std::memcpy(&fl, host.data() + 8, 4);
  const int32_t *col = reinterpret_cast<const int32_t *>(host.data() + 16);
  if (fl & 1u) return set_err(h, GGS_ERR_INVARIANT, "negative type-topic count");
  if ((int64_t)total != (h->global_tokens >= 0 ? h->global_tokens : h->N)) return set_err(h, GGS_ERR_INVARIANT, "type-topic counts do not sum to the corpus size");
  for (int k = 0; k < K; ++k)
    if (col[k] != nk[(size_t)k]) return set_err(h, GGS_ERR_INVARIANT, "column sum differs from tokensPerTopic");
  return GGS_OK;
}

int ggs_get_launch_info(ggs_handle *h, int64_t *num_chunks, int32_t *lds_bytes_z, int32_t *docs_per_block_theta) {
  if (!h) return GGS_ERR_BAD_ARG;
  const LaunchPlan &pl = h->plan;
  if (num_chunks) *num_chunks = pl.sliced() ? h->Cs + h->Cw : h->C;
  if (lds_bytes_z) *lds_bytes_z = pl.sliced() ? sliced_fused_lds(h->K, pl.hot_cap) : pl.z.lds;
  if (docs_per_block_theta) *docs_per_block_theta = h->cfg->theta_docs;
  return GGS_OK;
}

int ggs_get_num_hot_words(ggs_handle *h, int32_t *num_hot) {
  if (!h || !num_hot) return GGS_ERR_BAD_ARG;
  *num_hot = (h->plan.sliced() && !(h->flags & GGS_FLAG_PCGS)) ? h->num_hot + h->num_warm : 0;
  return GGS_OK;
}

int ggs_get_z_parts(ggs_handle *h, int32_t *parts) {
  if (!h || !parts) return GGS_ERR_BAD_ARG;
  const int32_t P = (int32_t)h->part_doc.size() - 1;
  *parts = (h->plan.stream() && h->overlap_theta && P > 1 && !(h->flags & GGS_FLAG_PCGS)) ? P : 1;
  return GGS_OK;
}

int ggs_get_warm_tiers(ggs_handle *h, int32_t *tiers, int32_t *warm_words, int32_t *docs_per_chunk) {
  if (!h) return GGS_ERR_BAD_ARG;
  const bool on = h->have_corpus && h->plan.sliced() && !(h->flags & GGS_FLAG_PCGS);
  if (tiers) *tiers = on ? h->warm_tiers : 0;
  if (warm_words) *warm_words = on ? h->num_warm : 0;
  if (docs_per_chunk) *docs_per_chunk = on && h->warm_tiers ? h->plan.warm_docs : 0;
  return GGS_OK;
}

int ggs_get_z_form(ggs_handle *h, int32_t *kernel, int32_t *form, int32_t *calibrated) {
  if (!h) return GGS_ERR_BAD_ARG;
  const bool pcgs = (h->flags & GGS_FLAG_PCGS) != 0;
  const bool splittable = !pcgs && h->plan.sliced() && h->Cs > h->Cc && h->Cc > 0;
  if (kernel) *kernel = h->spalias ? 6 : pcgs ? (h->pcgs_wave ? 5 : 4) : h->plan.kernel;
  if (form) *form = (!pcgs && h->plan.sliced()) ? (splittable && h->z_split ? 1 : 2) : 0;
  if (calibrated) *calibrated = (splittable && h->z_split_tried && !h->plan.split_forced && h->plan.split) ? 1 : 0;
  return GGS_OK;
}

int ggs_java_lcg_next_ints(int32_t seed, int32_t bound, int64_t n, int32_t *out) {
  if (bound <= 0 || n < 0 || (n > 0 && !out)) return GGS_ERR_BAD_ARG;
  java_lcg_next_ints(seed, bound, n, out);
  return GGS_OK;
}

namespace {
struct TmpDev {
  std::vector<void *> p;
  ~TmpDev() { for (void *q : p) if (q) (void)hipFree(q); }
  void *get(size_t bytes) { void *q = nullptr; if (hipMalloc(&q, std::max<size_t>(bytes, 16)) != hipSuccess) return nullptr; p.push_back(q); return q; }
};
}

int ggs_debug_philox(int32_t device_id, int64_t n, const uint32_t *ctr, const uint32_t *key, uint32_t *out) {
  if (n <= 0 || !ctr || !key || !out || hipSetDevice(device_id) != hipSuccess) return GGS_ERR_BAD_ARG;
  TmpDev t;
  auto *dc = static_cast<uint32_t *>(t.get(n * 16)); auto *dk = static_cast<uint32_t *>(t.get(n * 8)); auto *dou = static_cast<uint32_t *>(t.get(n * 16));
  if (!dc || !dk || !dou) return GGS_ERR_HIP;
  if (hipMemcpy(dc, ctr, n * 16, hipMemcpyHostToDevice) != hipSuccess || hipMemcpy(dk, key, n * 8, hipMemcpyHostToDevice) != hipSuccess) return GGS_ERR_HIP;
  hipLaunchKernelGGL(debug_philox_kernel, dim3((unsigned)((n + 255) / 256)), dim3(256), 0, nullptr, n, dc, dk, dou);
  if (hipMemcpy(out, dou, n * 16, hipMemcpyDeviceToHost) != hipSuccess) return GGS_ERR_HIP;
  return GGS_OK;
}

int ggs_debug_math(int32_t device_id, int32_t op, int64_t n, const double *x, const double *y, double *out) {
  if (n <= 0 || !x || !out || hipSetDevice(device_id) != hipSuccess) return GGS_ERR_BAD_ARG;
  TmpDev t;
  auto *dx = static_cast<double *>(t.get(n * 8)); auto *dy = static_cast<double *>(t.get(n * 8)); auto *dou = static_cast<double *>(t.get(n * 8));
  if (!dx || !dy || !dou) return GGS_ERR_HIP;
  if (hipMemcpy(dx, x, n * 8, hipMemcpyHostToDevice) != hipSuccess) return GGS_ERR_HIP;
  if (hipMemcpy(dy, y ? y : x, n * 8, hipMemcpyHostToDevice) != hipSuccess) return GGS_ERR_HIP;
  hipLaunchKernelGGL(debug_math_kernel, dim3((unsigned)((n + 255) / 256)), dim3(256), 0, nullptr, op, n, dx, dy, dou);
  if (hipMemcpy(out, dou, n * 8, hipMemcpyDeviceToHost) != hipSuccess) return GGS_ERR_HIP;
  return GGS_OK;
}

int ggs_debug_draw(int32_t device_id, int32_t kind, uint64_t seed, uint32_t iteration, uint32_t purpose, uint64_t elem0, int64_t n,
                   const double *shape, double *out, int32_t *status) {
  if (n <= 0 || !out || (kind == 2 && !shape) || hipSetDevice(device_id) != hipSuccess) return GGS_ERR_BAD_ARG;
  TmpDev t;
  auto *ds = static_cast<double *>(t.get(n * 8)); auto *dou = static_cast<double *>(t.get(n * 8)); auto *dst = static_cast<uint32_t *>(t.get(16));
  if (!ds || !dou || !dst) return GGS_ERR_HIP;
  if (shape && hipMemcpy(ds, shape, n * 8, hipMemcpyHostToDevice) != hipSuccess) return GGS_ERR_HIP;
  if (hipMemset(dst, 0, 16) != hipSuccess) return GGS_ERR_HIP;
  hipLaunchKernelGGL(debug_draw_kernel, dim3((unsigned)((n + 255) / 256)), dim3(256), 0, nullptr, kind, seed, iteration, purpose, elem0, n, ds, dou, dst);
  uint32_t st = 0;
  if (hipMemcpy(out, dou, n * 8, hipMemcpyDeviceToHost) != hipSuccess || hipMemcpy(&st, dst, 4, hipMemcpyDeviceToHost) != hipSuccess) return GGS_ERR_HIP;
  if (status) *status = (int32_t)st;
  return GGS_OK;
}

int ggs_debug_poisson(int32_t device_id, double beta, int32_t threshold, uint64_t seed, uint32_t iteration, uint32_t purpose, uint64_t elem0, int64_t n,
                      const int32_t *counts, int32_t *out) {
  const int32_t L = threshold == 0 ? 100 : threshold;
  if (n <= 0 || !counts || !out || !(beta > 0) || L < 1 || L > kPoissonMaxThreshold || hipSetDevice(device_id) != hipSuccess) return GGS_ERR_BAD_ARG;
  for (int64_t i = 0; i < n; ++i)
    if (counts[i] < 0) return GGS_ERR_BAD_ARG;
  std::vector<double> T;
  build_poisson_table(beta, L, T);
  TmpDev t;
  auto *dt = static_cast<double *>(t.get(T.size() * 8)); auto *dc = static_cast<int32_t *>(t.get(n * 4));
  auto *dou = static_cast<int32_t *>(t.get(n * 4)); auto *dst = static_cast<uint32_t *>(t.get(16));
  if (!dt || !dc || !dou || !dst) return GGS_ERR_HIP;
  if (hipMemcpy(dt, T.data(), T.size() * 8, hipMemcpyHostToDevice) != hipSuccess || hipMemcpy(dc, counts, n * 4, hipMemcpyHostToDevice) != hipSuccess ||
      hipMemset(dst, 0, 16) != hipSuccess)
    return GGS_ERR_HIP;
  hipLaunchKernelGGL(debug_poisson_kernel, dim3((unsigned)((n + 255) / 256)), dim3(256), 0, nullptr, seed, iteration, purpose, elem0, n, dc, L, beta, dt, T[0],
                     dou, dst);
  uint32_t st = 0;
  if (hipGetLastError() != hipSuccess || hipMemcpy(out, dou, n * 4, hipMemcpyDeviceToHost) != hipSuccess || hipMemcpy(&st, dst, 4, hipMemcpyDeviceToHost) != hipSuccess)
    return GGS_ERR_HIP;
  return st ? GGS_ERR_RNG_EXHAUSTED : GGS_OK;
}

int ggs_debug_alias(int32_t device_id, int32_t V, int32_t K, const double *phi, const double *alpha, double *ps, int32_t *a, double *type_norm) {
  if (V <= 0 || K <= 0 || K > kPcgsWaveMaxTopics || !phi || !alpha || !ps || !a || !type_norm || hipSetDevice(device_id) != hipSuccess) return GGS_ERR_BAD_ARG;
  const size_t kv = (size_t)K * V;
  std::vector<double> phiT(kv);
  for (int32_t k = 0; k < K; ++k)
    for (int32_t v = 0; v < V; ++v) phiT[(size_t)v * K + k] = phi[(size_t)k * V + v];
  TmpDev t;
  auto *dphi = static_cast<double *>(t.get(kv * 8)); auto *dal = static_cast<double *>(t.get((size_t)K * 8));
  auto *dps = static_cast<double *>(t.get(kv * 8)); auto *da = static_cast<int32_t *>(t.get(kv * 4)); auto *dtn = static_cast<double *>(t.get((size_t)V * 8));
  if (!dphi || !dal || !dps || !da || !dtn) return GGS_ERR_HIP;
  if (hipMemcpy(dphi, phiT.data(), kv * 8, hipMemcpyHostToDevice) != hipSuccess || hipMemcpy(dal, alpha, (size_t)K * 8, hipMemcpyHostToDevice) != hipSuccess)
    return GGS_ERR_HIP;
  AliasParams ap{};
  ap.phiT = dphi; ap.alpha = dal; ap.ps = dps; ap.a = da; ap.type_norm = dtn; ap.V = V; ap.K = K; ap.Kp = K; ap.wpb = alias_words_per_block(K);
  if (hipFuncSetAttribute(reinterpret_cast<const void *>(alias_build_kernel), hipFuncAttributeMaxDynamicSharedMemorySize, kMaxLdsBytes) != hipSuccess) return GGS_ERR_HIP;
  hipLaunchKernelGGL(alias_build_kernel, dim3((unsigned)std::min<int64_t>(((int64_t)V + ap.wpb - 1) / ap.wpb, 4096)), dim3(64), alias_lds_bytes(K, ap.wpb), nullptr, ap);
  if (hipGetLastError() != hipSuccess || hipMemcpy(ps, dps, kv * 8, hipMemcpyDeviceToHost) != hipSuccess ||
      hipMemcpy(a, da, kv * 4, hipMemcpyDeviceToHost) != hipSuccess || hipMemcpy(type_norm, dtn, (size_t)V * 8, hipMemcpyDeviceToHost) != hipSuccess)
    return GGS_ERR_HIP;
  return GGS_OK;
}

int ggs_debug_column_sum_guided(int32_t device_id, int32_t V, int32_t K, const double *x, const int32_t *counts, double beta, const double *guess,
                                double *out, double *pref_out, int32_t *n_k_out) {
  if (V <= 0 || K <= 0 || (!x == !counts) || !out || hipSetDevice(device_id) != hipSuccess) return GGS_ERR_BAD_ARG;
  TmpDev t;
  const size_t kv = (size_t)V * K;
  ggs_handle tmp;
  tmp.K = K; tmp.V = V; tmp.beta = beta; tmp.stream = nullptr; tmp.exact_sum = true;
  tmp.sum_nseg = (V + kSumSegRows - 1) / kSumSegRows;
  const size_t pref_bytes = ((size_t)tmp.sum_nseg + 1) * K * 8;
  tmp.d_sum_pref = static_cast<double *>(t.get(pref_bytes));
  tmp.d_sum_fn = static_cast<double *>(t.get((size_t)tmp.sum_nseg * K * 32));
  void *dsrc = t.get(kv * (x ? 8 : 4));
  auto *dou = static_cast<double *>(t.get((size_t)K * 8));
  auto *dnk = static_cast<int32_t *>(t.get((size_t)K * 4));
  int rc = GGS_OK;
  if (!tmp.d_sum_pref || !tmp.d_sum_fn || !dsrc || !dou || !dnk) rc = GGS_ERR_HIP;
  else if (hipMemcpy(dsrc, x ? (const void *)x : (const void *)counts, kv * (x ? 8 : 4), hipMemcpyHostToDevice) != hipSuccess) rc = GGS_ERR_HIP;
  else if (guess && hipMemcpy(tmp.d_sum_pref, guess, pref_bytes, hipMemcpyHostToDevice) != hipSuccess) rc = GGS_ERR_HIP;
  else {
    if (x) launch_column_sum<double, false>(&tmp, static_cast<const double *>(dsrc), K, K, dou, nullptr, guess != nullptr, true);
// ... 15 lines not shown
```

### ldagroupedgibbssampler_amd/csrc/ggs_z_kernel.hpp

```cpp
#pragma once
#include "ggs_kernels.hpp"

namespace ggs {

struct SliceMap {
  int32_t rem, size, ksm;
  uint32_t m_size, m_size1;
  int64_t rank_stride;
};
__device__ __forceinline__ int64_t slice_cell(const SliceMap &m, int k, int w) {
  const int cut = m.rem * (m.size + 1);
  int r, c;
  if (k < cut) { r = udiv_small(k, m.m_size1); c = k - r * (m.size + 1); }
  else { const int q = udiv_small(k - cut, m.m_size); r = m.rem + q; c = k - cut - q * m.size; }
  return (int64_t)r * m.rank_stride + (int64_t)w * m.ksm + c;
}

__device__ __forceinline__ void slice_rank_col(const SliceMap &m, int k, int &r, int &c) {
  const int cut = m.rem * (m.size + 1);
  if (k < cut) { r = udiv_small(k, m.m_size1); c = k - r * (m.size + 1); }
  else { const int q = udiv_small(k - cut, m.m_size); r = m.rem + q; c = k - cut - q * m.size; }
}

struct ZParams {
  const int32_t *tok;
  const int32_t *inv_perm;
  int32_t *z;
  int32_t *zw;
  const int64_t *chunk_start;
  const int32_t *chunk_doc;
  const int32_t *chunk_len;
  const double *theta;
  const double *phiT;
  uint32_t *status;
  int64_t num_chunks;
  int64_t tok_base;
  uint64_t seed;
  uint32_t iteration;
  int32_t K, Kp, pitch16, tile_tokens;
  int32_t ablate;
  const int32_t *ct_tok;
  const int32_t *ct_idx;
  const int32_t *ct_ip;
  const int32_t *c_docs;
  int64_t num_cold;
  const int32_t *hot_words;
  int32_t num_hot, hot_pitch;
  int32_t hot_off, wave_lds;
  int32_t ring_base;
  double margin_scale;
  const int32_t *chunk_doc1;
  int32_t two_rows;
  int32_t *cnt_send;
  SliceMap smap;
  const int4 *ht_pack;
  const int32_t *h_docs;
  const int4 *wt_pack;
  const int32_t *w_docs;
  const int32_t *warm_words;
  const int64_t *warm_meta;
  int32_t warm_tiers, warm_rows;
  long long *dbg;
  const float *phiT32;
  int32_t Kp32;
  unsigned long long *replays;
  double margin_scale32;
};

struct alignas(16) D2 { double a, b; };

typedef __attribute__((address_space(3))) void lds_void_t;
typedef __attribute__((address_space(1))) const void glb_cvoid_t;
typedef __attribute__((address_space(4))) const int64_t const_i64_t;
typedef __attribute__((address_space(4))) const int32_t const_i32_t;

__device__ __forceinline__ D2 lds_d2(const unsigned char *p) { return *reinterpret_cast<const D2 *>(p); }

constexpr int z_tile_theta_bytes(const int Kp) { return (Kp * 8 + 15) / 16 * 16; }
constexpr int z_tile_lds_bytes(const int Kp, const int pitch16, const int T) { return T * pitch16 * 16 + z_tile_theta_bytes(Kp); }
constexpr int z_tile_rows_in(const int bytes, const int Kp, const int pitch16) { return (bytes - z_tile_theta_bytes(Kp)) / (pitch16 * 16); }

template <int NT>
__global__ __launch_bounds__(64) void z_kernel(ZParams p) {
  extern __shared__ __align__(16) unsigned char smem[];
  const int lane = threadIdx.x;
  const int K = p.K, Kp = p.Kp;
  const int upr = Kp >> 1;
  const int pitch = p.pitch16 * 16;
  unsigned char *thb = smem + (size_t)p.tile_tokens * pitch;
  const unsigned char *phib = reinterpret_cast<const unsigned char *>(p.phiT);
  const size_t rowbytes = (size_t)Kp * 8;
  const const_i64_t *cstart = (const const_i64_t *)p.chunk_start;
  const const_i32_t *clen = (const const_i32_t *)p.chunk_len;
  const const_i32_t *cdoc = (const const_i32_t *)p.chunk_doc;
  const int64_t stride = gridDim.x;
  const int64_t C = p.num_chunks;

  int64_t c = blockIdx.x;
  if (c >= C) return;
  int64_t start = cstart[c];
  int len = clen[c], doc = cdoc[c];
  int64_t nstart = 0;
  int nlen = 0, ndoc = 0;
  if (c + stride < C) { nstart = cstart[c + stride]; nlen = clen[c + stride]; ndoc = cdoc[c + stride]; }
  int w = (lane < len) ? p.tok[start + lane] : 0;
  double tv[NT];
  {
    const double *thg = p.theta + (size_t)doc * K;
#pragma unroll
    for (int t = 0; t < NT; ++t) tv[t] = (t * 64 + lane < K) ? thg[t * 64 + lane] : 0.0;
  }

  for (;;) {
#pragma unroll
    for (int t = 0; t < NT; ++t)
      if (t * 64 + lane < Kp) reinterpret_cast<double *>(thb)[t * 64 + lane] = tv[t];

    const bool has_next = c + stride < C;
    int64_t nnstart = 0;
    int nnlen = 0, nndoc = 0, wn = 0;
    if (has_next) {
      if (c + 2 * stride < C) { nnstart = cstart[c + 2 * stride]; nnlen = clen[c + 2 * stride]; nndoc = cdoc[c + 2 * stride]; }
      wn = (lane < nlen) ? p.tok[nstart + lane] : 0;
      const double *thg = p.theta + (size_t)ndoc * K;
#pragma unroll
      for (int t = 0; t < NT; ++t) tv[t] = (t * 64 + lane < K) ? thg[t * 64 + lane] : 0.0;
    }

    if (!(p.ablate & 4)) {
      for (int i = 0; i < len; ++i) {
        const int wi = __builtin_amdgcn_readlane(w, i);
        const unsigned char *rb = phib + (size_t)wi * rowbytes;
        unsigned char *dst = smem + (size_t)i * pitch;
        for (int u0 = 0; u0 < upr; u0 += 64) {
          const int u = u0 + lane;
          if (u < upr)
            __builtin_amdgcn_global_load_lds((glb_cvoid_t *)(rb + (size_t)u * 16), (lds_void_t *)(dst + (size_t)u0 * 16), 16, 0, 0);
        }
      }
    }
    asm volatile("s_waitcnt vmcnt(0)");
    __syncthreads();

    if (lane < len) {
      const unsigned char *rowp = smem + lane * pitch;

#define GGS_LD8(A, P) { A##0 = lds_d2(P); A##1 = lds_d2((P) + 16); A##2 = lds_d2((P) + 32); A##3 = lds_d2((P) + 48); }
#define GGS_SUM8(A, S) { \
        sum += (S##0).a * (A##0).a; sum += (S##0).b * (A##0).b; sum += (S##1).a * (A##1).a; sum += (S##1).b * (A##1).b; \
        sum += (S##2).a * (A##2).a; sum += (S##2).b * (A##2).b; sum += (S##3).a * (A##3).a; sum += (S##3).b * (A##3).b; }
      double sum = 0.0;
      if (p.ablate & 8) sum = 1.0;
      else {
        int j = 0;
        if (K >= 8) {
          D2 a0, a1, a2, a3, b0, b1, b2, b3, s0, s1, s2, s3, t0, t1, t2, t3;
          GGS_LD8(a, rowp) GGS_LD8(s, thb)
          while (j + 24 <= K) {
            GGS_LD8(b, rowp + (j + 8) * 8) GGS_LD8(t, thb + (j + 8) * 8)
            GGS_SUM8(a, s)
            GGS_LD8(a, rowp + (j + 16) * 8) GGS_LD8(s, thb + (j + 16) * 8)
            GGS_SUM8(b, t)
            j += 16;
          }
          if (j + 16 <= K) {
            GGS_LD8(b, rowp + (j + 8) * 8) GGS_LD8(t, thb + (j + 8) * 8)
            GGS_SUM8(a, s)
            GGS_SUM8(b, t)
            j += 16;
          } else {
            GGS_SUM8(a, s)
            j += 8;
          }
        }
        for (; j < K; ++j)
          sum += *reinterpret_cast<const double *>(thb + j * 8) * *reinterpret_cast<const double *>(rowp + j * 8);
      }
#undef GGS_SUM8

      const uint64_t gtok = (uint64_t)(p.tok_base + start + lane);
      const U4 o = philox4x32_10((uint32_t)gtok, (uint32_t)(gtok >> 32), (uint32_t)GGS_PURPOSE_Z << 24, p.iteration,
                                 (uint32_t)p.seed, (uint32_t)(p.seed >> 32));
      const double U = u53(o.x, o.y);
      double sample = U * sum;

      int cnt = 0;
      bool live = !(p.ablate & 2);
      if (!live) { cnt = 1 + (int)(U * K); sample = 0.0; }
#define GGS_STEP(TH, PHI) { cnt += (sample > 0.0); sample -= (TH) * (PHI); }
#define GGS_WALK8(A, S) { \
        GGS_STEP((S##0).a, (A##0).a) GGS_STEP((S##0).b, (A##0).b) GGS_STEP((S##1).a, (A##1).a) GGS_STEP((S##1).b, (A##1).b) \
        GGS_STEP((S##2).a, (A##2).a) GGS_STEP((S##2).b, (A##2).b) GGS_STEP((S##3).a, (A##3).a) GGS_STEP((S##3).b, (A##3).b) }
      {
        int j = 0;
        if (live && K >= 8) {
          D2 a0, a1, a2, a3, b0, b1, b2, b3, s0, s1, s2, s3, t0, t1, t2, t3;
          GGS_LD8(a, rowp) GGS_LD8(s, thb)
          while (live && j + 24 <= K) {
            GGS_LD8(b, rowp + (j + 8) * 8) GGS_LD8(t, thb + (j + 8) * 8)
            GGS_WALK8(a, s)
            GGS_LD8(a, rowp + (j + 16) * 8) GGS_LD8(s, thb + (j + 16) * 8)
            GGS_WALK8(b, t)
            j += 16;
            live = __any(sample > 0.0);
          }
          if (live) {
            if (j + 16 <= K) {
              GGS_LD8(b, rowp + (j + 8) * 8) GGS_LD8(t, thb + (j + 8) * 8)
              GGS_WALK8(a, s)
              GGS_WALK8(b, t)
              j += 16;
            } else {
              GGS_WALK8(a, s)
              j += 8;
            }
            live = __any(sample > 0.0);
          }
        }
// ... 25 lines not shown
```

### ldagroupedgibbssampler_amd/csrc/ggs_z_sliced.hpp

```cpp
#pragma once
#include <type_traits>

#include "ggs_z_kernel.hpp"

#ifndef GGS_ABL
#define GGS_ABL 0
#endif

namespace ggs {

constexpr int kSliceTopics = 16;
constexpr int kSliceUnits = 8;
constexpr int kSlice32Topics = 32;
constexpr int kSliceBytes = 64 * 128;
#ifndef GGS_RING_SLOTS
#define GGS_RING_SLOTS 2
#endif
constexpr int kRingSlots = GGS_RING_SLOTS;
constexpr int kSlicedMaxTopics = 192;
constexpr int kSlicedDefaultTopics = 160;
constexpr int kPhiTailPadBytes = 1024;
constexpr int kHotTailBytes = 64;

constexpr int kWarmThetaPad = 16;
#ifndef GGS_WARM_UNITS
#define GGS_WARM_UNITS 4
#endif
#ifndef GGS_WARM_LANE_DOUBLES
#define GGS_WARM_LANE_DOUBLES 12
#endif
constexpr int warm_docs_for(const int kmax) {
  const int rowd = (kmax + kSliceTopics - 1) / kSliceTopics * kSliceTopics;
  const int d = rowd <= 112 ? GGS_WARM_LANE_DOUBLES / 2 : rowd <= 128 ? GGS_WARM_LANE_DOUBLES / 2 - 1 : 2;
  return d < 2 ? 2 : d > 8 ? 8 : d;
}

constexpr int sliced_kmax(const int K) { return (K + 7) / 8 * 8; }
constexpr int sliced_slices(const int K) { return (sliced_kmax(K) + kSliceTopics - 1) / kSliceTopics; }
constexpr int sliced_ring_base(const int K) { return round_up(imax(kChunkDocs * sliced_kmax(K) * 8, sliced_slices(K) * 128), 256); }
constexpr int sliced_wave_lds(const int K) { return sliced_ring_base(K) + kRingSlots * kSliceBytes; }
constexpr int sliced_cold_lds(const int K) { return kSlicedWaves * sliced_wave_lds(K); }
constexpr int table_row_pitch(const int K) { return sliced_kmax(K) / 8 * 64 + 16; }
constexpr int sliced_fused_lds(const int K, const int rows) { return sliced_cold_lds(K) + rows * table_row_pitch(K); }
constexpr int hot_wave_lds(const int K) { return round_up(kChunkDocs * sliced_slices(K) * kSliceTopics * 8, 256); }
constexpr int warm_wave_lds(const int K) { return round_up(warm_docs_for(sliced_kmax(K)) * (sliced_slices(K) * kSliceTopics * 8 + kWarmThetaPad), 256); }
constexpr int table_lds(const int K, const int wave_lds, const int rows) { return kSlicedWaves * wave_lds + rows * table_row_pitch(K) + kHotTailBytes; }
constexpr int table_rows_beside_cold(const int K, const int wave_lds) {
  return imax(0, imin(255, ((kMaxLdsBytes - lds_alloc_of(sliced_cold_lds(K)) - kSlicedWaves * wave_lds) / kLdsGranule * kLdsGranule - kHotTailBytes) / table_row_pitch(K)));
}
constexpr int table_rows_fused(const int K) { return imax(0, imin(255, (kMaxLdsBytes - sliced_cold_lds(K)) / table_row_pitch(K))); }

struct alignas(8) D2u { double a, b; };

template <int S, int N, class F>
__device__ __forceinline__ void static_for(F &&f) {
  if constexpr (S < N) {
    f(std::integral_constant<int, S>{});
    static_for<S + 1, N>(f);
  }
}

typedef float f2_t __attribute__((ext_vector_type(2)));
typedef float f4_t __attribute__((ext_vector_type(4)));
template <int KMAX>
__device__ __forceinline__ void cold_chunks32(const ZParams &p, unsigned char *thb, unsigned char *ring, const int64_t wid, const int64_t stride, const int lane) {
  constexpr int NS = (KMAX + kSlice32Topics - 1) / kSlice32Topics;
  constexpr int kAhead = NS < kRingSlots - 1 ? NS : kRingSlots - 1;
  constexpr int NT = (KMAX + 63) / 64;
  constexpr int kThetaRow = KMAX * 4;
  const int K = p.K;
  const unsigned char *phib = reinterpret_cast<const unsigned char *>(p.phiT32);
  const size_t rowbytes = (size_t)p.Kp32 * 4;
  const const_i32_t *cdocs = (const const_i32_t *)p.c_docs;
  double *prod = reinterpret_cast<double *>(thb + kChunkDocs * kThetaRow);
  const int lrow = lane >> 3, lslot = lane & 7;
  const unsigned char *my_row = ring + lane * 128;
  const int rot = lane >> 1;
  const float mscale = (float)p.margin_scale32;

  auto load_theta = [&](const int d0, const int d1, double (&tv)[kChunkDocs][NT]) {
    const double *t0 = p.theta + (size_t)d0 * K, *t1 = p.theta + (size_t)d1 * K;
#pragma unroll
    for (int t = 0; t < NT; ++t) {
      tv[0][t] = (t * 64 + lane < K) ? t0[t * 64 + lane] : 0.0;
      tv[1][t] = (t * 64 + lane < K) ? t1[t * 64 + lane] : 0.0;
    }
  };
  auto stage_theta = [&](const double (&tv)[kChunkDocs][NT]) {
#pragma unroll
    for (int r = 0; r < kChunkDocs; ++r)
#pragma unroll
      for (int t = 0; t < NT; ++t)
        if (t * 64 + lane < KMAX) reinterpret_cast<float *>(thb + r * kThetaRow)[t * 64 + lane] = phi32_of(tv[r][t]);
  };
  auto row_addresses = [&](const int w, const unsigned char *(&ra)[8]) {
#pragma unroll
    for (int m = 0; m < 8; ++m) {
      const int row = 8 * m + lrow;
      const int wm = __shfl(w, row) & ((1 << kSlotShift) - 1);
      ra[m] = phib + (size_t)wm * rowbytes + (size_t)(((lslot - (row >> 1)) & 7) << 4);
    }
  };
  auto issue_slice = [&](auto sc, const int slot, const unsigned char *const (&ra)[8]) {
    constexpr int s = decltype(sc)::value;
#pragma unroll
    for (int m = 0; m < 8; ++m)
      __builtin_amdgcn_global_load_lds((glb_cvoid_t *)ra[m], (lds_void_t *)(ring + slot * kSliceBytes + m * 1024 - s * 128), 16, s * 128, 0);
  };
  auto finish = [&](const float (&a)[KMAX], const int64_t c, const int idx, const int ip, const int w) {
    const uint64_t gtok = (uint64_t)(p.tok_base + idx);
    const U4 o = philox4x32_10((uint32_t)gtok, (uint32_t)(gtok >> 32), (uint32_t)GGS_PURPOSE_Z << 24, p.iteration,
                               (uint32_t)p.seed, (uint32_t)(p.seed >> 32));
    const double U = u53(o.x, o.y);
    const float A = a[KMAX - 1];
    const float t0 = (float)(U * (double)A);
    const float delta = ((float)(2 * K + 8) * 0x1p-24f * A) * mscale;
    const f2_t nt0 = {-t0, -t0};
    int cnt = 0;
    float m = t0;
    bool live = true;
#pragma unroll
    for (int kb = 0; kb < KMAX; kb += 16) {
      if (live) {
        uint32_t bits = 0;
        float dl = 0.0f;
#pragma unroll
        for (int j = 0; j < 16; j += 2)
          if (kb + j < KMAX) {
            const f2_t d = f2_t{a[kb + j], a[kb + j + 1]} + nt0;
            bits = __builtin_amdgcn_alignbit(bits, __float_as_uint(d.x), 31);
            bits = __builtin_amdgcn_alignbit(bits, __float_as_uint(d.y), 31);
            m = fminf(m, fminf(fabsf(d.x), fabsf(d.y)));
            dl = d.y;
          }
        cnt += __popc(bits);
        live = __any(dl < 0.0f);
      }
    }
    int new_topic = cnt;
    const bool undecided = idx >= 0 && !(A >= 0x1p-60f && A <= 0x1.fffffep127f && m > delta && cnt < K);
    uint64_t pend = __ballot(undecided);
    if (pend) {
      if (p.replays && lane == 0) atomicAdd(p.replays, (unsigned long long)__popcll(pend));
      const int slot = (int)((unsigned)w >> kSlotShift);
      const int d0 = cdocs[2 * c], d1 = cdocs[2 * c + 1];
      while (pend) {
        const int L = (int)__builtin_ctzll(pend);
        pend &= pend - 1;
        const int wl = __shfl(w, L) & ((1 << kSlotShift) - 1), dl = __shfl(slot, L) ? d1 : d0;
        const double UL = __shfl(U, L);
        const double *th = p.theta + (size_t)dl * K, *ph = p.phiT + (size_t)wl * p.Kp;
        for (int k = lane; k < K; k += 64) prod[k] = th[k] * ph[k];
        asm volatile("s_waitcnt lgkmcnt(0)" ::: "memory");
        double sum = 0.0;
        for (int k = 0; k < K; ++k) sum += prod[k];
        double sample = UL * sum;
        int nt = -1;
        while (sample > 0.0) {
          ++nt;
          if (nt >= K) break;
          sample -= prod[nt];
        }
        if (nt < 0 || nt >= K) {
          if (lane == L) atomicOr(p.status, ST_INVALID_TOPIC);
          nt = nt < 0 ? 0 : K - 1;
        }
        if (lane == L) new_topic = nt;
        asm volatile("s_waitcnt lgkmcnt(0)" ::: "memory");
      }
    }
    if (idx < 0) return;
    p.z[idx] = new_topic;
    p.zw[ip] = new_topic;
    const int word = w & ((1 << kSlotShift) - 1);
    if (p.cnt_send) __hip_atomic_fetch_add(&p.cnt_send[slice_cell(p.smap, new_topic, word)], 1, __ATOMIC_RELAXED, __HIP_MEMORY_SCOPE_AGENT);
  };

  const int64_t C = p.num_cold;
  int64_t c = wid;
  if (c >= C) return;
  int w0 = p.ct_tok[c * 64 + lane], id0 = p.ct_idx[c * 64 + lane], ip0 = p.ct_ip[c * 64 + lane];
  int w1 = 0, id1 = -1, ip1 = 0, w2 = 0, id2 = -1, ip2 = 0;
  double tv0[kChunkDocs][NT], tv1[kChunkDocs][NT], tv2[kChunkDocs][NT];
  load_theta(cdocs[2 * c], cdocs[2 * c + 1], tv0);
  if (c + stride < C) {
    const int64_t c1 = c + stride;
    w1 = p.ct_tok[c1 * 64 + lane]; id1 = p.ct_idx[c1 * 64 + lane]; ip1 = p.ct_ip[c1 * 64 + lane];
    load_theta(cdocs[2 * c1], cdocs[2 * c1 + 1], tv1);
  } else {
    load_theta(0, 0, tv1);
  }
#pragma unroll
  for (int r = 0; r < kChunkDocs; ++r)
#pragma unroll
    for (int t = 0; t < NT; ++t) tv2[r][t] = 0.0;
  const unsigned char *ra[8], *ran[8];
  row_addresses(w0, ra);
  row_addresses(w1, ran);
  int g = 0;
  static_for<0, kAhead>([&](auto sc) { issue_slice(sc, decltype(sc)::value % kRingSlots, ra); });

  for (;;) {
    const bool has1 = c + stride < C, has2 = c + 2 * stride < C;
    g = __builtin_amdgcn_readfirstlane(g);
    stage_theta(tv0);
    const unsigned char *trow = thb + ((unsigned)w0 >> kSlotShift) * kThetaRow;

    float a[KMAX];
    float acc = 0.0f;
    static_for<0, NS>([&](auto sidx) {
      constexpr int s = decltype(sidx)::value;
      const int cur = (g + s) % kRingSlots;
      const int nxt = (g + s + kAhead) % kRingSlots;
      if constexpr (s + kAhead < NS) issue_slice(std::integral_constant<int, s + kAhead>{}, nxt, ra);
      else if (has1) issue_slice(std::integral_constant<int, s + kAhead - NS>{}, nxt, ran);
      if (has1 || s + kAhead < NS) asm volatile("s_waitcnt vmcnt(%0)" ::"n"(8 * kAhead) : "memory");
      else asm volatile("s_waitcnt vmcnt(%0)" ::"n"(8 * (NS - 1 - s)) : "memory");
      {
        const unsigned char *rb = my_row + cur * kSliceBytes;
        f4_t ph[kSliceUnits], th[kSliceUnits];
#pragma unroll
        for (int u = 0; u < kSliceUnits; ++u)
          if (s * kSlice32Topics + 4 * u < KMAX) {
            ph[u] = *reinterpret_cast<const f4_t *>(rb + (((u + rot) & 7) << 4));
            th[u] = *reinterpret_cast<const f4_t *>(trow + s * (kSlice32Topics * 4) + u * 16);
          }
#pragma unroll
        for (int u = 0; u < kSliceUnits; ++u) {
          constexpr int k0 = s * kSlice32Topics;
          const int k = k0 + 4 * u;
          if (k < KMAX) {
            const f2_t q0 = f2_t{th[u].x, th[u].y} * f2_t{ph[u].x, ph[u].y};
            const f2_t q1 = f2_t{th[u].z, th[u].w} * f2_t{ph[u].z, ph[u].w};
            acc += q0.x; a[k] = acc;
            acc += q0.y; a[k + 1] = acc;
            acc += q1.x; a[k + 2] = acc;
            acc += q1.y; a[k + 3] = acc;
          }
        }
      }
      asm volatile("s_waitcnt lgkmcnt(0)" ::: "memory");
    });
    g = (g + NS) % kRingSlots;

    if (has2) {
      const int64_t c2 = c + 2 * stride;
      w2 = p.ct_tok[c2 * 64 + lane]; id2 = p.ct_idx[c2 * 64 + lane]; ip2 = p.ct_ip[c2 * 64 + lane];
      load_theta(cdocs[2 * c2], cdocs[2 * c2 + 1], tv2);
    } else {
      w2 = 0; id2 = -1; ip2 = 0;
    }

    finish(a, c, id0, ip0, w0);
    if (!has1) break;
    c += stride;
    w0 = w1; id0 = id1; ip0 = ip1;
    w1 = w2; id1 = id2; ip1 = ip2;
#pragma unroll
    for (int r = 0; r < kChunkDocs; ++r)
#pragma unroll
      for (int t = 0; t < NT; ++t) { tv0[r][t] = tv1[r][t]; tv1[r][t] = tv2[r][t]; }
#pragma unroll
    for (int m = 0; m < 8; ++m) ra[m] = ran[m];
    row_addresses(w1, ran);
  }
}

template <int KMAX, bool F32>
__device__ __forceinline__ void z_sliced_body(const ZParams &p) {
  constexpr int NS = (KMAX + kSliceTopics - 1) / kSliceTopics;
  constexpr int kAhead = NS < kRingSlots - 1 ? NS : kRingSlots - 1;
  constexpr int NT = (KMAX + 63) / 64;
  constexpr int kThetaRow = KMAX * 8;
  extern __shared__ __align__(16) unsigned char smem[];
  const int lane = threadIdx.x & 63, wave = __builtin_amdgcn_readfirstlane(threadIdx.x >> 6);
  const int K = p.K;
  unsigned char *thb = smem + wave * p.wave_lds;
  unsigned char *ring = thb + p.ring_base;
  const unsigned char *phib = reinterpret_cast<const unsigned char *>(p.phiT);
  const size_t rowbytes = (size_t)p.Kp * 8;
  const const_i32_t *cdocs = (const const_i32_t *)p.c_docs;
  const int64_t stride = (int64_t)gridDim.x * kSlicedWaves;
  const int64_t wid = (int64_t)blockIdx.x * kSlicedWaves + wave;

  {
    constexpr int upr = KMAX / 2;
    for (int i = threadIdx.x; i < p.num_hot * upr; i += kSlicedWaves * 64) {
      const int r = i / upr, u = i - r * upr;
      *reinterpret_cast<D2 *>(smem + p.hot_off + r * p.hot_pitch + u * 16) =
          *reinterpret_cast<const D2 *>(phib + (size_t)p.hot_words[r] * rowbytes + (size_t)u * 16);
    }
  }
  __syncthreads();

  const int lrow = lane >> 3, lslot = lane & 7;
  const unsigned char *my_row = ring + lane * 128;
  const int rot = lane >> 1;

  auto load_theta = [&](const int d0, const int d1, double (&tv)[kChunkDocs][NT]) {
    const double *t0 = p.theta + (size_t)d0 * K, *t1 = p.theta + (size_t)d1 * K;
#pragma unroll
    for (int t = 0; t < NT; ++t) {
      tv[0][t] = (t * 64 + lane < K) ? t0[t * 64 + lane] : 0.0;
      tv[1][t] = (t * 64 + lane < K) ? t1[t * 64 + lane] : 0.0;
    }
  };
  auto stage_theta = [&](const double (&tv)[kChunkDocs][NT]) {
#pragma unroll
    for (int r = 0; r < kChunkDocs; ++r)
#pragma unroll
      for (int t = 0; t < NT; ++t)
        if (t * 64 + lane < KMAX) reinterpret_cast<double *>(thb + r * kThetaRow)[t * 64 + lane] = tv[r][t];
  };
  auto finish = [&](const double (&sc)[KMAX], const double sum, const int idx, const int ip, const int word) {
    if (idx < 0) return;
    const uint64_t gtok = (uint64_t)(p.tok_base + idx);
    const U4 o = philox4x32_10((uint32_t)gtok, (uint32_t)(gtok >> 32), (uint32_t)GGS_PURPOSE_Z << 24, p.iteration,
                               (uint32_t)p.seed, (uint32_t)(p.seed >> 32));
    const double U = u53(o.x, o.y);
    double t = 0.0 - U * sum;
    int cnt = 0;
    bool live = true;
#pragma unroll
    for (int kb = 0; kb < KMAX; kb += 16) {
      if (live) {
        uint32_t bits = 0;
#pragma unroll
        for (int j = 0; j < 16; ++j)
          if (kb + j < KMAX) {
            bits = __builtin_amdgcn_alignbit(bits, (uint32_t)hi32(t), 31);
            t += sc[kb + j];
          }
        cnt += __popc(bits);
        live = __any(hi32(t) < 0);
      }
    }
    int new_topic = cnt - 1;
    if (new_topic < 0 || hi32(t) < 0) {
      if (!GGS_ABL) atomicOr(p.status, ST_INVALID_TOPIC);
      new_topic = new_topic < 0 ? 0 : K - 1;
    }
    p.z[idx] = new_topic;
    p.zw[ip] = new_topic;
    if (p.cnt_send && word >= 0) __hip_atomic_fetch_add(&p.cnt_send[slice_cell(p.smap, new_topic, word)], 1, __ATOMIC_RELAXED, __HIP_MEMORY_SCOPE_AGENT);
  };

  auto cold_chunks = [&]() {
    const int64_t C = p.num_cold;
    auto row_addresses = [&](const int w, const unsigned char *(&ra)[8]) {
#pragma unroll
      for (int m = 0; m < 8; ++m) {
        const int row = 8 * m + lrow;
        const int wm = __shfl(w, row) & ((1 << kSlotShift) - 1);
        ra[m] = phib + (size_t)wm * rowbytes + (size_t)(((lslot - (row >> 1)) & 7) << 4);
      }
    };
    auto issue_slice = [&](auto sc, const int slot, const unsigned char *const (&ra)[8]) {
      constexpr int s = decltype(sc)::value;
      if (GGS_ABL & 1) return;
#pragma unroll
      for (int m = 0; m < 8; ++m)
        __builtin_amdgcn_global_load_lds((glb_cvoid_t *)ra[m], (lds_void_t *)(ring + slot * kSliceBytes + m * 1024 - s * 128), 16, s * 128, 0);
    };

    int64_t c = wid;
    if (c >= C) return;
    int w0 = p.ct_tok[c * 64 + lane], id0 = p.ct_idx[c * 64 + lane], ip0 = p.ct_ip[c * 64 + lane];
    int w1 = 0, id1 = -1, ip1 = 0, w2 = 0, id2 = -1, ip2 = 0;
    double tv0[kChunkDocs][NT], tv1[kChunkDocs][NT], tv2[kChunkDocs][NT];
    load_theta(cdocs[2 * c], cdocs[2 * c + 1], tv0);
    if (c + stride < C) {
      const int64_t c1 = c + stride;
      w1 = p.ct_tok[c1 * 64 + lane]; id1 = p.ct_idx[c1 * 64 + lane]; ip1 = p.ct_ip[c1 * 64 + lane];
      load_theta(cdocs[2 * c1], cdocs[2 * c1 + 1], tv1);
    } else {
      load_theta(0, 0, tv1);
    }
#pragma unroll
    for (int r = 0; r < kChunkDocs; ++r)
#pragma unroll
      for (int t = 0; t < NT; ++t) tv2[r][t] = 0.0;
    const unsigned char *ra[8], *ran[8];
    row_addresses(w0, ra);
    row_addresses(w1, ran);
    int g = 0;
    static_for<0, kAhead>([&](auto sc) { issue_slice(sc, decltype(sc)::value % kRingSlots, ra); });

    for (;;) {
      const bool has1 = c + stride < C, has2 = c + 2 * stride < C;
      g = __builtin_amdgcn_readfirstlane(g);
      stage_theta(tv0);
      const unsigned char *trow = thb + ((unsigned)w0 >> kSlotShift) * kThetaRow;

      double sc[KMAX];
      double sum = 0.0;
      static_for<0, NS>([&](auto sidx) {
        constexpr int s = decltype(sidx)::value;
        const int cur = (g + s) % kRingSlots;
        const int nxt = (g + s + kAhead) % kRingSlots;
        if constexpr (s + kAhead < NS) issue_slice(std::integral_constant<int, s + kAhead>{}, nxt, ra);
        else if (has1) issue_slice(std::integral_constant<int, s + kAhead - NS>{}, nxt, ran);
        if (GGS_ABL & (1 | 8)) {}
        else if (has1 || s + kAhead < NS) asm volatile("s_waitcnt vmcnt(%0)" ::"n"(8 * kAhead) : "memory");
        else asm volatile("s_waitcnt vmcnt(%0)" ::"n"(8 * (NS - 1 - s)) : "memory");
        if (id0 >= 0) {
          const unsigned char *rb = my_row + cur * kSliceBytes;
          D2 ph[kSliceUnits], th[kSliceUnits];
#pragma unroll
          for (int u = 0; u < kSliceUnits; ++u)
            if (s * kSliceTopics + 2 * u + 1 < KMAX) {
              ph[u] = lds_d2(rb + (((u + rot) & 7) << 4));
              th[u] = lds_d2(trow + s * (kSliceTopics * 8) + u * 16);
            }
#pragma unroll
          for (int u = 0; u < kSliceUnits; ++u) {
            constexpr int k0 = s * kSliceTopics;
            const int k = k0 + 2 * u;
            if (k + 1 < KMAX) {
              sc[k] = th[u].a * ph[u].a;
              sum += sc[k];
              sc[k + 1] = th[u].b * ph[u].b;
              sum += sc[k + 1];
            }
          }
        }
        asm volatile("" ::: "memory");
      });
      g = (g + NS) % kRingSlots;

      if (has2) {
        const int64_t c2 = c + 2 * stride;
        w2 = p.ct_tok[c2 * 64 + lane]; id2 = p.ct_idx[c2 * 64 + lane]; ip2 = p.ct_ip[c2 * 64 + lane];
        load_theta(cdocs[2 * c2], cdocs[2 * c2 + 1], tv2);
      } else {
        w2 = 0; id2 = -1; ip2 = 0;
      }

      finish(sc, sum, id0, ip0, w0 & ((1 << kSlotShift) - 1));
      if (!has1) break;
      c += stride;
      w0 = w1; id0 = id1; ip0 = ip1;
      w1 = w2; id1 = id2; ip1 = ip2;
#pragma unroll
      for (int r = 0; r < kChunkDocs; ++r)
#pragma unroll
        for (int t = 0; t < NT; ++t) { tv0[r][t] = tv1[r][t]; tv1[r][t] = tv2[r][t]; }
#pragma unroll
      for (int m = 0; m < 8; ++m) ra[m] = ran[m];
      row_addresses(w1, ran);
    }
  };

  auto hot_chunks = [&]() {
    const int64_t C = p.num_chunks;
    int64_t c = p.num_cold + wid;
    if (c >= C) return;
    int w0 = p.ct_tok[c * 64 + lane], id0 = p.ct_idx[c * 64 + lane], ip0 = p.ct_ip[c * 64 + lane];
    double tv0[kChunkDocs][NT];
    load_theta(cdocs[2 * c], cdocs[2 * c + 1], tv0);
    for (;;) {
      const bool has1 = c + stride < C;
      int w1 = 0, id1 = -1, ip1 = 0;
      double tv1[kChunkDocs][NT];
      if (has1) {
        const int64_t c1 = c + stride;
        w1 = p.ct_tok[c1 * 64 + lane]; id1 = p.ct_idx[c1 * 64 + lane]; ip1 = p.ct_ip[c1 * 64 + lane];
        load_theta(cdocs[2 * c1], cdocs[2 * c1 + 1], tv1);
      } else {
        load_theta(0, 0, tv1);
      }
      stage_theta(tv0);
      const unsigned char *trow = thb + ((unsigned)w0 >> kSlotShift) * kThetaRow;
      const unsigned char *hrow = smem + p.hot_off + (w0 & ((1 << kSlotShift) - 1)) * p.hot_pitch;

      double sc[KMAX];
      double sum = 0.0;
      if (id0 >= 0) {
        static_for<0, NS>([&](auto sidx) {
          constexpr int s = decltype(sidx)::value;
          D2 ph[kSliceUnits], th[kSliceUnits];
#pragma unroll
          for (int u = 0; u < kSliceUnits; ++u)
            if (s * kSliceTopics + 2 * u + 1 < KMAX) {
              ph[u] = lds_d2(hrow + s * (kSliceTopics * 8) + u * 16);
              th[u] = lds_d2(trow + s * (kSliceTopics * 8) + u * 16);
            }
#pragma unroll
          for (int u = 0; u < kSliceUnits; ++u) {
            constexpr int k0 = s * kSliceTopics;
            const int k = k0 + 2 * u;
            if (k + 1 < KMAX) {
              sc[k] = th[u].a * ph[u].a;
              sum += sc[k];
              sc[k + 1] = th[u].b * ph[u].b;
              sum += sc[k + 1];
            }
          }
        });
      }
      finish(sc, sum, id0, ip0, -1);
      if (!has1) break;
      c += stride;
      w0 = w1; id0 = id1; ip0 = ip1;
#pragma unroll
      for (int r = 0; r < kChunkDocs; ++r)
#pragma unroll
        for (int t = 0; t < NT; ++t) tv0[r][t] = tv1[r][t];
    }
  };

#pragma unroll 1
  for (int phase = 0; phase < 2; ++phase) {
    if ((phase ^ wave) & 1) hot_chunks();
    else if constexpr (F32) cold_chunks32<KMAX>(p, thb, ring, wid, stride, lane);
    else cold_chunks();
  }
}

template <int KMAX>
__global__ __launch_bounds__(kSlicedWaves * 64) void z_sliced_kernel(ZParams p) { z_sliced_body<KMAX, false>(p); }
template <int KMAX>
__global__ __launch_bounds__(kSlicedWaves * 64) void z_sliced32_kernel(ZParams p) { z_sliced_body<KMAX, true>(p); }

template <int KMAX>
__device__ __forceinline__ void load_phi_table(unsigned char *table, const int pitch, const unsigned char *phib, const size_t rowbytes,
                                               const int32_t *words_g, const int nrows, const int wave, const int lane, const int tid) {
  constexpr int upr = KMAX / 2 + 1, kRowsAhead = 6, NP = (upr + 63) / 64;
  const const_i32_t *words = (const const_i32_t *)words_g;
  for (int r0 = wave; r0 < nrows; r0 += kSlicedWaves * kRowsAhead) {
    D2 v[kRowsAhead][NP];
#pragma unroll
    for (int a = 0; a < kRowsAhead; ++a) {
      const int r = r0 + kSlicedWaves * a;
      const unsigned char *src = phib + (size_t)words[r < nrows ? r : r0] * rowbytes;
#pragma unroll
      for (int q = 0; q < NP; ++q) {
        const int u = q * 64 + lane;
        v[a][q] = u < upr - 1 ? *reinterpret_cast<const D2 *>(src + (size_t)u * 16) : D2{0.0, 0.0};
      }
    }
#pragma unroll
    for (int a = 0; a < kRowsAhead; ++a) {
      const int r = r0 + kSlicedWaves * a;
#pragma unroll
      for (int q = 0; q < NP; ++q) {
        const int u = q * 64 + lane;
        if (r < nrows && u < upr) *reinterpret_cast<D2 *>(table + r * pitch + u * 16) = v[a][q];
      }
    }
  }
  if (tid < kHotTailBytes / 8) reinterpret_cast<double *>(table + nrows * pitch)[tid] = 0.0;
}

template <int KMAX, int UB = kSliceUnits>
__device__ __forceinline__ int hot_token(const ZParams &p, const int K, const unsigned char *hrow, const unsigned char *trow, const int id0) {
  constexpr int NS = (KMAX + kSliceTopics - 1) / kSliceTopics;
  double sum = 0.0, ck[NS];
  static_for<0, NS>([&](auto sidx) {
    constexpr int s = decltype(sidx)::value;
#pragma unroll
    for (int b = 0; b < kSliceUnits / UB; ++b) {
      D2 ph[UB], th[UB];
#pragma unroll
      for (int u = 0; u < UB; ++u)
        if (s * kSliceTopics + 2 * (b * UB + u) + 1 < KMAX) {
          ph[u] = lds_d2(hrow + s * (kSliceTopics * 8) + (b * UB + u) * 16);
          th[u] = lds_d2(trow + s * (kSliceTopics * 8) + (b * UB + u) * 16);
        }
#pragma unroll
      for (int u = 0; u < UB; ++u)
        if (s * kSliceTopics + 2 * (b * UB + u) + 1 < KMAX) {
          sum += th[u].a * ph[u].a;
          sum += th[u].b * ph[u].b;
        }
      asm volatile("" : "+v"(sum) : : "memory");
    }
    ck[s] = sum;
  });
  const uint64_t gtok = (uint64_t)(p.tok_base + id0);
  const U4 o = philox4x32_10((uint32_t)gtok, (uint32_t)(gtok >> 32), (uint32_t)GGS_PURPOSE_Z << 24, p.iteration,
                             (uint32_t)p.seed, (uint32_t)(p.seed >> 32));
  const double t0 = u53(o.x, o.y) * sum;
  const double delta = (sum * (double)K) * 0x1p-51 * p.margin_scale;
  int gsel = NS;
  static_for<0, NS>([&](auto sidx) {
    constexpr int s = NS - 1 - decltype(sidx)::value;
    if (t0 - ck[s] < -delta) gsel = s;
  });
  bool undecided = gsel == NS;
  if (undecided) gsel = 0;
  double s = 0.0;
  static_for<0, NS - 1>([&](auto sidx) {
    constexpr int q = decltype(sidx)::value;
    if (gsel == q + 1) s = ck[q];
  });
  undecided |= fabs(t0 - s) <= delta;
  int ahead = 0;
  {
    const unsigned char *hs = hrow + gsel * (kSliceTopics * 8), *ts = trow + gsel * (kSliceTopics * 8);
#pragma unroll
    for (int h = 0; h < 2; ++h) {
      D2 ph[kSliceUnits / 2], th[kSliceUnits / 2];
#pragma unroll
      for (int u = 0; u < kSliceUnits / 2; ++u) {
        ph[u] = lds_d2(hs + (h * (kSliceUnits / 2) + u) * 16);
        th[u] = lds_d2(ts + (h * (kSliceUnits / 2) + u) * 16);
      }
#pragma unroll
      for (int u = 0; u < kSliceUnits / 2; ++u) {
        s += th[u].a * ph[u].a;
        double d = t0 - s;
        ahead += d >= -delta;
        undecided |= fabs(d) <= delta;
        s += th[u].b * ph[u].b;
        d = t0 - s;
        ahead += d >= -delta;
        undecided |= fabs(d) <= delta;
      }
      asm volatile("" ::: "memory");
    }
  }
  int new_topic = gsel * kSliceTopics + ahead;
  if (undecided || ahead >= kSliceTopics || new_topic >= K) {
    const double *prow = reinterpret_cast<const double *>(hrow), *trw = reinterpret_cast<const double *>(trow);
    double sample = t0;
    new_topic = -1;
    while (sample > 0.0) {
      ++new_topic;
      if (new_topic >= K) break;
      sample -= trw[new_topic] * prow[new_topic];
    }
    if (new_topic < 0 || new_topic >= K) {
      atomicOr(p.status, ST_INVALID_TOPIC);
      new_topic = new_topic < 0 ? 0 : K - 1;
    }
  }
  return new_topic;
}

typedef int i3v_t __attribute__((ext_vector_type(3)));
typedef int i4v_t __attribute__((ext_vector_type(4)));
template <int N>
__device__ __forceinline__ void wait_vmcnt_take(const i3v_t &e, int &w, int &id, int &ip) {
  asm volatile("s_waitcnt vmcnt(%6)\n\tv_mov_b32 %0, %3\n\tv_mov_b32 %1, %4\n\tv_mov_b32 %2, %5"
               : "=&v"(w), "=&v"(id), "=&v"(ip) : "v"(e.x), "v"(e.y), "v"(e.z), "n"(N) : "memory");
}

template <int KMAX, int DOCS, int PAD, int UB>
__device__ __forceinline__ void table_chunks(const ZParams &p, unsigned char *smem, unsigned char *thb, const int4 *pack, const int32_t *docs_g,
                                             const int64_t first, const int64_t C, const int64_t stride, const int lane, const int32_t *count_words) {
  constexpr int NS = (KMAX + kSliceTopics - 1) / kSliceTopics;
  constexpr int kRowD = NS * kSliceTopics;
  constexpr int kThetaRow = kRowD * 8 + PAD;
  constexpr int NQ = (kRowD + 127) / 128;
  constexpr int kLoads = 1 + DOCS * NQ;
  constexpr int kStores = 2;
  const int K = p.K;
  const const_i32_t *cdocs = (const const_i32_t *)docs_g;
  const uint32_t loff = (uint32_t)lane * 16;
  uint32_t toff[NQ];
#pragma unroll
  for (int q = 0; q < NQ; ++q) { const int k0 = 2 * (q * 64 + lane); toff[q] = (uint32_t)(k0 < K ? k0 : 0) * 8; }
  struct Set { i3v_t e; i4v_t t[DOCS][NQ]; };
  auto issue = [&](const int64_t c, Set &S) {
    typedef int docs8_t __attribute__((ext_vector_type(8)));
    const docs8_t dd = *reinterpret_cast<const __attribute__((address_space(4))) docs8_t *>(cdocs + c * kWarmDocSlots);
    const int4 *lp = pack + c * 64;
    asm volatile("global_load_dwordx3 %0, %1, %2" : "=v"(S.e) : "v"(loff), "s"(lp) : "memory");
#pragma unroll
    for (int r = 0; r < DOCS; ++r) {
      const double *tr = p.theta + (size_t)dd[r] * K;
#pragma unroll
      for (int q = 0; q < NQ; ++q) asm volatile("global_load_dwordx4 %0, %1, %2" : "=v"(S.t[r][q]) : "v"(toff[q]), "s"(tr) : "memory");
    }
  };
  auto arrive = [&](Set &S, const int after, int &w0, int &id0, int &ip0) {
    if (after == 2) wait_vmcnt_take<kLoads + kStores>(S.e, w0, id0, ip0);
    else if (after == 1) wait_vmcnt_take<kLoads>(S.e, w0, id0, ip0);
    else wait_vmcnt_take<0>(S.e, w0, id0, ip0);
#pragma unroll
    for (int r = 0; r < DOCS; ++r)
#pragma unroll
      for (int q = 0; q < NQ; ++q) asm volatile("" : "+v"(S.t[r][q]));
  };
  auto chunk = [&](Set &S, const int64_t c, const int w0, const int id0, const int ip0) {
#pragma unroll
    for (int r = 0; r < DOCS; ++r)
#pragma unroll
      for (int q = 0; q < NQ; ++q)
        if (2 * (q * 64 + lane) < kRowD) {
          const int k0 = 2 * (q * 64 + lane);
          const D2 v = __builtin_bit_cast(D2, S.t[r][q]);
          *reinterpret_cast<D2 *>(thb + r * kThetaRow + k0 * 8) = D2{k0 < K ? v.a : 0.0, k0 + 1 < K ? v.b : 0.0};
        }
    if (c + 2 * stride < C) issue(c + 2 * stride, S);
    const int row = w0 & ((1 << kWarmSlotShift) - 1);
    const unsigned char *trow = thb + ((unsigned)w0 >> kWarmSlotShift) * kThetaRow;
    const unsigned char *hrow = smem + p.hot_off + row * p.hot_pitch;
    if (id0 >= 0) {
      const int new_topic = hot_token<KMAX, UB>(p, K, hrow, trow, id0);
      p.z[id0] = new_topic;
      p.zw[ip0] = new_topic;
      if (count_words)
        __hip_atomic_fetch_add(&p.cnt_send[slice_cell(p.smap, new_topic, count_words[row])], 1, __ATOMIC_RELAXED, __HIP_MEMORY_SCOPE_AGENT);
    }
  };
  int64_t c = first;
  if (c >= C) return;
  Set A, B;
  issue(c, A);
  if (c + stride < C) issue(c + stride, B);
  int done = 0;
  for (;;) {
    int w0, id0, ip0;
    arrive(A, c + stride < C ? (done ? 2 : 1) : 0, w0, id0, ip0);
    chunk(A, c, w0, id0, ip0);
    c += stride;
    if (c >= C) break;
    arrive(B, c + stride < C ? 2 : 0, w0, id0, ip0);
    chunk(B, c, w0, id0, ip0);
    c += stride;
    if (c >= C) break;
    done = 1;
  }
}

template <int KMAX>
__global__ __launch_bounds__(kSlicedWaves * 64) __attribute__((amdgpu_waves_per_eu(4, 4))) void z_hot_kernel(ZParams p) {
  extern __shared__ __align__(16) unsigned char smem[];
  __builtin_amdgcn_s_setprio(3);
  const int lane = threadIdx.x & 63, wave = __builtin_amdgcn_readfirstlane(threadIdx.x >> 6);
  unsigned char *thb = smem + wave * p.wave_lds;
  load_phi_table<KMAX>(smem + p.hot_off, p.hot_pitch, reinterpret_cast<const unsigned char *>(p.phiT), (size_t)p.Kp * 8, p.hot_words, p.num_hot, wave, lane, threadIdx.x);
  __syncthreads();
  table_chunks<KMAX, kChunkDocs, 0, (KMAX <= 128 ? kSliceUnits : kSliceUnits / 2)>(p, smem, thb, p.ht_pack, p.h_docs, (int64_t)blockIdx.x * kSlicedWaves + wave, p.num_chunks - p.num_cold,
                                                 (int64_t)gridDim.x * kSlicedWaves, lane, nullptr);
}


template <int KMAX>
__global__ __launch_bounds__(kSlicedWaves * 64) __attribute__((amdgpu_waves_per_eu(4, 4))) void z_warm_kernel(ZParams p) {
  extern __shared__ __align__(16) unsigned char smem[];
  __builtin_amdgcn_s_setprio(3);
  const int lane = threadIdx.x & 63, wave = __builtin_amdgcn_readfirstlane(threadIdx.x >> 6);
  unsigned char *thb = smem + wave * p.wave_lds;
  const const_i64_t *meta = (const const_i64_t *)p.warm_meta;
  const int64_t stride = (int64_t)gridDim.x * kSlicedWaves;
  const int64_t wid = (int64_t)blockIdx.x * kSlicedWaves + wave;
  for (int tier = 0; tier < p.warm_tiers; ++tier) {
    if (tier) __syncthreads();
    const int32_t *words = p.warm_words + (size_t)tier * p.warm_rows;
    load_phi_table<KMAX>(smem + p.hot_off, p.hot_pitch, reinterpret_cast<const unsigned char *>(p.phiT), (size_t)p.Kp * 8, words, (int)meta[p.warm_tiers + 1 + tier], wave, lane, threadIdx.x);
    __syncthreads();
    table_chunks<KMAX, warm_docs_for(KMAX), kWarmThetaPad, GGS_WARM_UNITS>(p, smem, thb, p.wt_pack, p.w_docs, meta[tier] + wid, meta[tier + 1], stride, lane,
                                                                          p.cnt_send ? words : nullptr);
  }
}

}
```

Measured before the change: 16300.

## Use float32 hot/warm phi tables with deferred exact fp64 replay of undecided tokens

Hot and warm table kernels now store phi and theta rows in LDS as float32 by default, which halves row pitch and lets more word rows fit. Tokens whose float32 sampling margin is too small to decide are pushed to a global replay list. A separate kernel then resamples them exactly in fp64. The aim is to cut LDS footprint and fp64 arithmetic on the dominant hot and warm paths. In exchange it adds replay bookkeeping, an extra launch and memset, and limits warm tiers to one.

```diff
diff --git a/ldagroupedgibbssampler_amd/csrc/ggs_api.hip b/ldagroupedgibbssampler_amd/csrc/ggs_api.hip
--- a/ldagroupedgibbssampler_amd/csrc/ggs_api.hip
+++ b/ldagroupedgibbssampler_amd/csrc/ggs_api.hip
@@ -42,7 +42,7 @@
 };
 struct Knobs {
   Knob zkernel{"GGS_DEBUG_ZKERNEL"}, group{"GGS_DEBUG_GROUP"}, regck{"GGS_DEBUG_REGCK"}, tworows{"GGS_DEBUG_TWOROWS"}, wpc{"GGS_DEBUG_WPC"};
-  Knob phi64{"GGS_DEBUG_PHI64"}, split{"GGS_DEBUG_SPLIT"}, hot{"GGS_DEBUG_HOT"}, tile{"GGS_DEBUG_TILE"};
+  Knob phi64{"GGS_DEBUG_PHI64"}, table32{"GGS_DEBUG_TABLE32"}, split{"GGS_DEBUG_SPLIT"}, hot{"GGS_DEBUG_HOT"}, tile{"GGS_DEBUG_TILE"};
   Knob warm{"GGS_DEBUG_WARM"}, warm_rows{"GGS_DEBUG_WARM_ROWS"}, warm_fill{"GGS_DEBUG_WARM_FILL"}, warm_cpw{"GGS_DEBUG_WARM_CPW"};
   Knob theta_b{"GGS_DEBUG_THETA_B"}, theta_wgs{"GGS_DEBUG_THETA_WGS"}, zparts{"GGS_DEBUG_ZPARTS"}, beside{"GGS_DEBUG_BESIDE"};
   Knob pcgs_wave{"GGS_DEBUG_PCGS_WAVE"}, pcgs_stream{"GGS_DEBUG_PCGS_STREAM"};
@@ -65,6 +65,7 @@
   bool two_rows = false;
   KernelLaunch cold, hot, warm;
   bool f32 = false;
+  bool table32 = false;
   bool split = true, split_forced = false;
   int32_t wave_lds = 0, ring_base = 0, hot_wave_lds = 0, warm_wave_lds = 0, hot_pitch = 0, Kp32 = 0;
   int32_t hot_cap = 0, warm_cap = 0, warm_docs = 0;
@@ -154,6 +155,9 @@
   hipEvent_t ev_part[8] = {nullptr, nullptr, nullptr, nullptr, nullptr, nullptr, nullptr, nullptr};
   int64_t theta_ahead_iter = INT64_MIN;
   float *d_phiT32 = nullptr;
+  int4 *d_replay_list = nullptr;
+  uint32_t *d_replay_count = nullptr;
+  int32_t replay_cap = 0;
   unsigned long long *d_replays = nullptr;
   int64_t z_f32_launches = 0;
   double *d_alpha = nullptr, *d_theta = nullptr, *d_phiT = nullptr, *d_mag = nullptr, *d_tot = nullptr, *d_phi_mean = nullptr;
@@ -736,6 +740,8 @@
 
 const void *hot_kernel_for(int K) { GGS_KMAX_SWITCH(z_hot_kernel) }
 const void *warm_kernel_for(int K) { GGS_KMAX_SWITCH(z_warm_kernel) }
+const void *hot32_kernel_for(int K) { GGS_KMAX_SWITCH(z_hot32_kernel) }
+const void *warm32_kernel_for(int K) { GGS_KMAX_SWITCH(z_warm32_kernel) }
 const void *pcgs_kernel_for(int K) { GGS_KMAX_SWITCH(pcgs_sliced_kernel) }
 const void *polyaurn_kernel_for(int K) { GGS_KMAX_SWITCH(polyaurn_sliced_kernel) }
 const void *collapsed_kernel_for(int K) {
@@ -802,16 +808,19 @@
   } else if (sliced) {
     pl.f32 = !kn.phi64.is(1);
     pl.Kp32 = round_up(K, kSlice32Topics);
-    pl.ring_base = sliced_ring_base(K); pl.wave_lds = sliced_wave_lds(K); pl.hot_pitch = table_row_pitch(K);
-    pl.hot_wave_lds = hot_wave_lds(K); pl.warm_wave_lds = warm_wave_lds(K);
+    pl.table32 = pl.f32 && (kn.table32.set ? kn.table32.v != 0 : true);
+    if (pl.table32) pl.warm_tiers_max = 1;
+    const int es = pl.table32 ? 4 : 8;
+    pl.ring_base = sliced_ring_base(K); pl.wave_lds = sliced_wave_lds(K); pl.hot_pitch = table_row_pitch(K, es);
+    pl.hot_wave_lds = hot_wave_lds(K, es); pl.warm_wave_lds = warm_wave_lds(K, es);
     if (kn.split.set) { pl.split = kn.split.v != 0; pl.split_forced = kn.split.v == 2; }
-    pl.hot_cap = pl.split ? table_rows_beside_cold(K, pl.hot_wave_lds) : table_rows_fused(K);
+    pl.hot_cap = pl.split ? table_rows_beside_cold(K, pl.hot_wave_lds, es) : table_rows_fused(K, es);
     if (kn.hot.set) pl.hot_cap = std::max(0, std::min(pl.hot_cap, kn.hot.v));
     pl.cold = {pl.f32 ? sliced32_kernel_for(K) : sliced_kernel_for(K), kSlicedWaves * 64, sliced_cold_lds(K), 1};
-    pl.hot = {hot_kernel_for(K), kSlicedWaves * 64, table_lds(K, pl.hot_wave_lds, 0), 1};
-    pl.warm = {warm_kernel_for(K), kSlicedWaves * 64, table_lds(K, pl.warm_wave_lds, 0), 1};
+    pl.hot = {pl.table32 ? hot32_kernel_for(K) : hot_kernel_for(K), kSlicedWaves * 64, table_lds(K, pl.hot_wave_lds, 0, es), 1};
+    pl.warm = {pl.table32 ? warm32_kernel_for(K) : warm_kernel_for(K), kSlicedWaves * 64, table_lds(K, pl.warm_wave_lds, 0, es), 1};
     pl.warm_docs = warm_docs_for(sliced_kmax(K));
-    pl.warm_cap = table_rows_beside_cold(K, pl.warm_wave_lds);
+    pl.warm_cap = table_rows_beside_cold(K, pl.warm_wave_lds, es);
     if (pl.warm_cap < 16) pl.warm_cap = 0;
     if (kn.warm.set) pl.warm_tiers_max = std::max(0, std::min(kWarmMaxTiers, kn.warm.v));
     if (kn.warm_rows.set) pl.warm_cap = std::max(0, std::min(pl.warm_cap, kn.warm_rows.v));
@@ -936,6 +945,8 @@
   zp.wt_pack = reinterpret_cast<const int4 *>(h->d_wt_pack); zp.w_docs = h->d_w_docs; zp.warm_words = h->d_warm_words;
   zp.warm_meta = h->d_warm_meta; zp.warm_tiers = h->warm_tiers; zp.warm_rows = pl.warm_cap;
   zp.phiT32 = h->d_phiT32; zp.Kp32 = pl.Kp32; zp.replays = h->d_replays; zp.margin_scale32 = h->margin_scale32;
+  zp.table32 = pl.table32 ? 1 : 0;
+  zp.replay_list = h->d_replay_list; zp.replay_count = h->d_replay_count; zp.replay_cap = h->replay_cap;
   void *args[] = {&zp};
   if (!pl.sliced()) {
     zp.chunk_start += c0; zp.chunk_doc += c0; zp.chunk_len += c0; zp.num_chunks = c1 - c0;
@@ -951,6 +962,12 @@
   wp.wave_lds = pl.warm_wave_lds; wp.hot_off = kSlicedWaves * pl.warm_wave_lds;
   void *wargs[] = {&wp};
   auto launch_warm = [&](hipStream_t st) { return h->Cw == 0 ? hipSuccess : launch(h, pl.warm, h->warm_chunks_max, wargs, st, h->warm_rows_max * pl.hot_pitch); };
+  auto reset_replays = [&](hipStream_t st) { return pl.table32 ? hipMemsetAsync(h->d_replay_count, 0, sizeof(uint32_t), st) : hipSuccess; };
+  auto launch_replays = [&](hipStream_t st) {
+    if (!pl.table32) return hipSuccess;
+    const int64_t grid = std::max<int64_t>(1, std::min<int64_t>((h->replay_cap + 255) / 256, (int64_t)h->num_cus * 2));
+    return hipLaunchKernel(reinterpret_cast<const void *>(z_replay_kernel), dim3((unsigned)grid), dim3(256), wargs, 0, st);
+  };
   if (h->z_split && !force_fused && h->Cs > h->Cc && h->Cc > 0) {
     ZParams hp = zp;
     hp.wave_lds = pl.hot_wave_lds; hp.hot_off = kSlicedWaves * pl.hot_wave_lds;
@@ -963,8 +980,10 @@
     }
     zp.num_chunks = h->Cc; zp.num_hot = 0;
     HIP_TRY(h, launch(h, pl.cold, h->Cc, args, h->stream));
+    HIP_TRY(h, reset_replays(h->side_hot));
     HIP_TRY(h, launch(h, pl.hot, h->Cs - h->Cc, hargs, h->side_hot, hot_rows_lds));
     HIP_TRY(h, launch_warm(h->side_hot));
+    HIP_TRY(h, launch_replays(h->side_hot));
     if (defer_join && zp.cnt_send) {
       hipStream_t main_stream = h->stream;
       h->stream = h->side_hot;
@@ -978,7 +997,11 @@
     else HIP_TRY(h, hipStreamWaitEvent(h->stream, h->ev_hot_join, 0));
   } else {
     HIP_TRY(h, launch(h, pl.cold, std::max(h->Cc, h->Cs - h->Cc), args, h->stream, hot_rows_lds));
-    HIP_TRY(h, launch_warm(h->stream));
+    if (h->Cw) {
+      HIP_TRY(h, reset_replays(h->stream));
+      HIP_TRY(h, launch_warm(h->stream));
+      HIP_TRY(h, launch_replays(h->stream));
+    }
   }
   if (pl.f32) ++h->z_f32_launches;
   return GGS_OK;
@@ -1399,8 +1422,8 @@
     if ((rc = dev_alloc(h, &h->d_phiT32, n32))) return bail(rc);
     if (hipMemset(h->d_phiT32, 0, sizeof(float) * n32) != hipSuccess) return bail(GGS_ERR_HIP);
     if (kn.replays.is(1)) {
-      if ((rc = dev_alloc(h, &h->d_replays, 1))) return bail(rc);
-      if (hipMemset(h->d_replays, 0, sizeof(unsigned long long)) != hipSuccess) return bail(GGS_ERR_HIP);
+      if ((rc = dev_alloc(h, &h->d_replays, 2))) return bail(rc);
+      if (hipMemset(h->d_replays, 0, 2 * sizeof(unsigned long long)) != hipSuccess) return bail(GGS_ERR_HIP);
     }
   }
   if (h->exact_sum && ((rc = dev_alloc(h, &h->d_sum_pref, ((size_t)h->sum_nseg + 1) * h->K)) ||
@@ -1447,10 +1470,13 @@
   (void)hipSetDevice(h->device);
   (void)hipDeviceSynchronize();
   if (h->d_replays) {
-    unsigned long long n = 0;
-    if (hipMemcpy(&n, h->d_replays, sizeof(n), hipMemcpyDeviceToHost) == hipSuccess)
-      fprintf(stderr, "[ggs] z replays: %llu tokens in %lld launches of z_sliced32_kernel (%.2f per launch)\n", n, (long long)h->z_f32_launches,
-              h->z_f32_launches ? (double)n / (double)h->z_f32_launches : 0.0);
+    unsigned long long n[2] = {0, 0};
+    if (hipMemcpy(n, h->d_replays, sizeof(n), hipMemcpyDeviceToHost) == hipSuccess) {
+      fprintf(stderr, "[ggs] z table replays: %llu tokens in %lld z steps of the float32 hot and warm tables (%.2f per step)\n", n[1], (long long)h->z_f32_launches,
+              h->z_f32_launches ? (double)n[1] / (double)h->z_f32_launches : 0.0);
+      fprintf(stderr, "[ggs] z replays: %llu tokens in %lld launches of z_sliced32_kernel (%.2f per launch)\n", n[0], (long long)h->z_f32_launches,
+              h->z_f32_launches ? (double)n[0] / (double)h->z_f32_launches : 0.0);
+    }
   }
   for (void **slot : h->owned)
     if (*slot) (void)hipFree(*slot);
@@ -1547,6 +1573,11 @@
                       (rc = upload(h, &h->d_c_docs, L.c_docs)) || (rc = upload(h, &h->d_hot_words, L.hot_words)) ||
                       (rc = upload(h, &h->d_ht_pack, L.ht_pack)) || (rc = upload(h, &h->d_h_docs, L.h_docs))))
     return rc;
+  if (pl.sliced() && pl.table32) {
+    h->replay_cap = (int32_t)std::min<int64_t>(INT32_MAX / 2, std::max<int64_t>(4096, N / 64));
+    if ((rc = dev_alloc(h, &h->d_replay_list, (size_t)h->replay_cap)) || (rc = dev_alloc(h, &h->d_replay_count, 1))) return rc;
+    HIP_TRY(h, hipMemset(h->d_replay_count, 0, sizeof(uint32_t)));
+  }
   if (L.warm_tiers > 0 && ((rc = upload(h, &h->d_wt_pack, L.wt_pack)) || (rc = upload(h, &h->d_w_docs, L.w_docs)) ||
                            (rc = upload(h, &h->d_warm_words, L.warm_words)) || (rc = upload(h, &h->d_warm_meta, L.warm_meta))))
     return rc;
@@ -2348,7 +2379,7 @@
   if (!h) return GGS_ERR_BAD_ARG;
   const LaunchPlan &pl = h->plan;
   if (num_chunks) *num_chunks = pl.sliced() ? h->Cs + h->Cw : h->C;
-  if (lds_bytes_z) *lds_bytes_z = pl.sliced() ? sliced_fused_lds(h->K, pl.hot_cap) : pl.z.lds;
+  if (lds_bytes_z) *lds_bytes_z = pl.sliced() ? sliced_fused_lds(h->K, pl.hot_cap, pl.table32 ? 4 : 8) : pl.z.lds;
   if (docs_per_block_theta) *docs_per_block_theta = h->cfg->theta_docs;
   return GGS_OK;
 }
diff --git a/ldagroupedgibbssampler_amd/csrc/ggs_z_kernel.hpp b/ldagroupedgibbssampler_amd/csrc/ggs_z_kernel.hpp
--- a/ldagroupedgibbssampler_amd/csrc/ggs_z_kernel.hpp
+++ b/ldagroupedgibbssampler_amd/csrc/ggs_z_kernel.hpp
@@ -64,6 +64,10 @@
   const float *phiT32;
   int32_t Kp32;
   unsigned long long *replays;
+  int4 *replay_list;
+  uint32_t *replay_count;
+  int32_t replay_cap;
+  int32_t table32;
   double margin_scale32;
 };
 
diff --git a/ldagroupedgibbssampler_amd/csrc/ggs_z_sliced.hpp b/ldagroupedgibbssampler_amd/csrc/ggs_z_sliced.hpp
--- a/ldagroupedgibbssampler_amd/csrc/ggs_z_sliced.hpp
+++ b/ldagroupedgibbssampler_amd/csrc/ggs_z_sliced.hpp
@@ -40,15 +40,17 @@
 constexpr int sliced_ring_base(const int K) { return round_up(imax(kChunkDocs * sliced_kmax(K) * 8, sliced_slices(K) * 128), 256); }
 constexpr int sliced_wave_lds(const int K) { return sliced_ring_base(K) + kRingSlots * kSliceBytes; }
 constexpr int sliced_cold_lds(const int K) { return kSlicedWaves * sliced_wave_lds(K); }
-constexpr int table_row_pitch(const int K) { return sliced_kmax(K) / 8 * 64 + 16; }
-constexpr int sliced_fused_lds(const int K, const int rows) { return sliced_cold_lds(K) + rows * table_row_pitch(K); }
-constexpr int hot_wave_lds(const int K) { return round_up(kChunkDocs * sliced_slices(K) * kSliceTopics * 8, 256); }
-constexpr int warm_wave_lds(const int K) { return round_up(warm_docs_for(sliced_kmax(K)) * (sliced_slices(K) * kSliceTopics * 8 + kWarmThetaPad), 256); }
-constexpr int table_lds(const int K, const int wave_lds, const int rows) { return kSlicedWaves * wave_lds + rows * table_row_pitch(K) + kHotTailBytes; }
-constexpr int table_rows_beside_cold(const int K, const int wave_lds) {
-  return imax(0, imin(255, ((kMaxLdsBytes - lds_alloc_of(sliced_cold_lds(K)) - kSlicedWaves * wave_lds) / kLdsGranule * kLdsGranule - kHotTailBytes) / table_row_pitch(K)));
-}
-constexpr int table_rows_fused(const int K) { return imax(0, imin(255, (kMaxLdsBytes - sliced_cold_lds(K)) / table_row_pitch(K))); }
+constexpr int table_row_pitch(const int K, const int es = 8) { return sliced_kmax(K) * es + 16; }
+constexpr int sliced_fused_lds(const int K, const int rows, const int es = 8) { return sliced_cold_lds(K) + rows * table_row_pitch(K, es); }
+constexpr int theta_row_lds(const int K, const int es) { return sliced_slices(K) * kSliceTopics * es; }
+constexpr int hot_wave_lds(const int K, const int es = 8) { return round_up(kChunkDocs * (theta_row_lds(K, es) + (es == 4 ? kWarmThetaPad : 0)), 256); }
+constexpr int warm_wave_lds(const int K, const int es = 8) { return round_up(warm_docs_for(sliced_kmax(K)) * (theta_row_lds(K, es) + kWarmThetaPad), 256); }
+constexpr int table_lds(const int K, const int wave_lds, const int rows, const int es = 8) { return kSlicedWaves * wave_lds + rows * table_row_pitch(K, es) + kHotTailBytes; }
+constexpr int table_rows_beside_cold(const int K, const int wave_lds, const int es = 8) {
+  return imax(0, imin(255, ((kMaxLdsBytes - lds_alloc_of(sliced_cold_lds(K)) - kSlicedWaves * wave_lds) / kLdsGranule * kLdsGranule - kHotTailBytes) / table_row_pitch(K, es)));
+}
+constexpr int table_rows_fused(const int K, const int es = 8) { return imax(0, imin(255, (kMaxLdsBytes - sliced_cold_lds(K)) / table_row_pitch(K, es))); }
+static_assert(table_row_pitch(100) == 848 && hot_wave_lds(100) == 1792 && warm_wave_lds(100) == 5632, "the fp64 layouts are what they were");
 
 struct alignas(8) D2u { double a, b; };
 
@@ -62,6 +64,84 @@
 
 typedef float f2_t __attribute__((ext_vector_type(2)));
 typedef float f4_t __attribute__((ext_vector_type(4)));
+__device__ __forceinline__ void replay_exact(const ZParams &p, double *prod, uint64_t pend, const int word, const int doc, const double U,
+                                             const int lane, int &new_topic) {
+  const int K = p.K;
+  while (pend) {
+    const int L = (int)__builtin_ctzll(pend);
+    pend &= pend - 1;
+    const int wl = __shfl(word, L), dl = __shfl(doc, L);
+    const double UL = __shfl(U, L);
+    const double *th = p.theta + (size_t)dl * K, *ph = p.phiT + (size_t)wl * p.Kp;
+    for (int k = lane; k < K; k += 64) prod[k] = th[k] * ph[k];
+    asm volatile("s_waitcnt lgkmcnt(0)" ::: "memory");
+    double sum = 0.0;
+    for (int k = 0; k < K; ++k) sum += prod[k];
+    double sample = UL * sum;
+    int nt = -1;
+    while (sample > 0.0) {
+      ++nt;
+      if (nt >= K) break;
+      sample -= prod[nt];
+    }
+    if (nt < 0 || nt >= K) {
+      if (lane == L) atomicOr(p.status, ST_INVALID_TOPIC);
+      nt = nt < 0 ? 0 : K - 1;
+    }
+    if (lane == L) new_topic = nt;
+    asm volatile("s_waitcnt lgkmcnt(0)" ::: "memory");
+  }
+}
+
+template <int KMAX>
+__device__ __forceinline__ void finish32(const ZParams &p, const float (&a)[KMAX], double *prod, const int64_t c, const int idx, const int ip, const int w,
+                                         const int32_t *row_words, const int lane) {
+  const int K = p.K;
+  const const_i32_t *cdocs = (const const_i32_t *)p.c_docs;
+  const float mscale = (float)p.margin_scale32;
+  const uint64_t gtok = (uint64_t)(p.tok_base + idx);
+  const U4 o = philox4x32_10((uint32_t)gtok, (uint32_t)(gtok >> 32), (uint32_t)GGS_PURPOSE_Z << 24, p.iteration,
+                             (uint32_t)p.seed, (uint32_t)(p.seed >> 32));
+  const double U = u53(o.x, o.y);
+  const float A = a[KMAX - 1];
+  const float t0 = (float)(U * (double)A);
+  const float delta = ((float)(2 * K + 8) * 0x1p-24f * A) * mscale;
+  const f2_t nt0 = {-t0, -t0};
+  int cnt = 0;
+  float m = t0;
+  bool live = true;
+#pragma unroll
+  for (int kb = 0; kb < KMAX; kb += 16) {
+    if (live) {
+      uint32_t bits = 0;
+      float dl = 0.0f;
+#pragma unroll
+      for (int j = 0; j < 16; j += 2)
+        if (kb + j < KMAX) {
+          const f2_t d = f2_t{a[kb + j], a[kb + j + 1]} + nt0;
+          bits = __builtin_amdgcn_alignbit(bits, __float_as_uint(d.x), 31);
+          bits = __builtin_amdgcn_alignbit(bits, __float_as_uint(d.y), 31);
+          m = fminf(m, fminf(fabsf(d.x), fabsf(d.y)));
+          dl = d.y;
+        }
+      cnt += __popc(bits);
+      live = __any(dl < 0.0f);
+    }
+  }
+  int new_topic = cnt;
+  const bool undecided = idx >= 0 && !(A >= 0x1p-60f && A <= 0x1.fffffep127f && m > delta && cnt < K);
+  const uint64_t pend = __ballot(undecided);
+  if (pend) {
+    if (p.replays && lane == 0) atomicAdd(p.replays + (row_words ? 1 : 0), (unsigned long long)__popcll(pend));
+    const int v = w & ((1 << kSlotShift) - 1);
+    replay_exact(p, prod, pend, row_words ? row_words[undecided ? v : 0] : v, cdocs[2 * c + ((unsigned)w >> kSlotShift)], U, lane, new_topic);
+  }
+  if (idx < 0) return;
+  p.z[idx] = new_topic;
+  p.zw[ip] = new_topic;
+  if (p.cnt_send && !row_words) __hip_atomic_fetch_add(&p.cnt_send[slice_cell(p.smap, new_topic, w & ((1 << kSlotShift) - 1))], 1, __ATOMIC_RELAXED, __HIP_MEMORY_SCOPE_AGENT);
+}
+
 template <int KMAX>
 __device__ __forceinline__ void cold_chunks32(const ZParams &p, unsigned char *thb, unsigned char *ring, const int64_t wid, const int64_t stride, const int lane) {
   constexpr int NS = (KMAX + kSlice32Topics - 1) / kSlice32Topics;
@@ -76,7 +156,6 @@
   const int lrow = lane >> 3, lslot = lane & 7;
   const unsigned char *my_row = ring + lane * 128;
   const int rot = lane >> 1;
-  const float mscale = (float)p.margin_scale32;
 
   auto load_theta = [&](const int d0, const int d1, double (&tv)[kChunkDocs][NT]) {
     const double *t0 = p.theta + (size_t)d0 * K, *t1 = p.theta + (size_t)d1 * K;
@@ -107,75 +186,6 @@
     for (int m = 0; m < 8; ++m)
       __builtin_amdgcn_global_load_lds((glb_cvoid_t *)ra[m], (lds_void_t *)(ring + slot * kSliceBytes + m * 1024 - s * 128), 16, s * 128, 0);
   };
-  auto finish = [&](const float (&a)[KMAX], const int64_t c, const int idx, const int ip, const int w) {
-    const uint64_t gtok = (uint64_t)(p.tok_base + idx);
-    const U4 o = philox4x32_10((uint32_t)gtok, (uint32_t)(gtok >> 32), (uint32_t)GGS_PURPOSE_Z << 24, p.iteration,
-                               (uint32_t)p.seed, (uint32_t)(p.seed >> 32));
-    const double U = u53(o.x, o.y);
-    const float A = a[KMAX - 1];
-    const float t0 = (float)(U * (double)A);
-    const float delta = ((float)(2 * K + 8) * 0x1p-24f * A) * mscale;
-    const f2_t nt0 = {-t0, -t0};
-    int cnt = 0;
-    float m = t0;
-    bool live = true;
-#pragma unroll
-    for (int kb = 0; kb < KMAX; kb += 16) {
-      if (live) {
-        uint32_t bits = 0;
-        float dl = 0.0f;
-#pragma unroll
-        for (int j = 0; j < 16; j += 2)
-          if (kb + j < KMAX) {
-            const f2_t d = f2_t{a[kb + j], a[kb + j + 1]} + nt0;
-            bits = __builtin_amdgcn_alignbit(bits, __float_as_uint(d.x), 31);
-            bits = __builtin_amdgcn_alignbit(bits, __float_as_uint(d.y), 31);
-            m = fminf(m, fminf(fabsf(d.x), fabsf(d.y)));
-            dl = d.y;
-          }
-        cnt += __popc(bits);
-        live = __any(dl < 0.0f);
-      }
-    }
-    int new_topic = cnt;
-    const bool undecided = idx >= 0 && !(A >= 0x1p-60f && A <= 0x1.fffffep127f && m > delta && cnt < K);
-    uint64_t pend = __ballot(undecided);
-    if (pend) {
-      if (p.replays && lane == 0) atomicAdd(p.replays, (unsigned long long)__popcll(pend));
-      const int slot = (int)((unsigned)w >> kSlotShift);
-      const int d0 = cdocs[2 * c], d1 = cdocs[2 * c + 1];
-      while (pend) {
-        const int L = (int)__builtin_ctzll(pend);
-        pend &= pend - 1;
-        const int wl = __shfl(w, L) & ((1 << kSlotShift) - 1), dl = __shfl(slot, L) ? d1 : d0;
-        const double UL = __shfl(U, L);
-        const double *th = p.theta + (size_t)dl * K, *ph = p.phiT + (size_t)wl * p.Kp;
-        for (int k = lane; k < K; k += 64) prod[k] = th[k] * ph[k];
-        asm volatile("s_waitcnt lgkmcnt(0)" ::: "memory");
-        double sum = 0.0;
-        for (int k = 0; k < K; ++k) sum += prod[k];
-        double sample = UL * sum;
-        int nt = -1;
-        while (sample > 0.0) {
-          ++nt;
-          if (nt >= K) break;
-          sample -= prod[nt];
-        }
-        if (nt < 0 || nt >= K) {
-          if (lane == L) atomicOr(p.status, ST_INVALID_TOPIC);
-          nt = nt < 0 ? 0 : K - 1;
-        }
-        if (lane == L) new_topic = nt;
-        asm volatile("s_waitcnt lgkmcnt(0)" ::: "memory");
-      }
-    }
-    if (idx < 0) return;
-    p.z[idx] = new_topic;
-    p.zw[ip] = new_topic;
-    const int word = w & ((1 << kSlotShift) - 1);
-    if (p.cnt_send) __hip_atomic_fetch_add(&p.cnt_send[slice_cell(p.smap, new_topic, word)], 1, __ATOMIC_RELAXED, __HIP_MEMORY_SCOPE_AGENT);
-  };
-
   const int64_t C = p.num_cold;
   int64_t c = wid;
   if (c >= C) return;
@@ -251,7 +261,7 @@
       w2 = 0; id2 = -1; ip2 = 0;
     }
 
-    finish(a, c, id0, ip0, w0);
+    finish32<KMAX>(p, a, prod, c, id0, ip0, w0, nullptr, lane);
     if (!has1) break;
     c += stride;
     w0 = w1; id0 = id1; ip0 = ip1;
@@ -263,6 +273,68 @@
 #pragma unroll
     for (int m = 0; m < 8; ++m) ra[m] = ran[m];
     row_addresses(w1, ran);
+  }
+}
+
+template <int KMAX>
+__device__ __forceinline__ void hot_chunks32(const ZParams &p, const unsigned char *table, unsigned char *thb, const int64_t wid, const int64_t stride, const int lane) {
+  constexpr int NT = (KMAX + 63) / 64;
+  constexpr int kThetaRow = KMAX * 4;
+  const int K = p.K;
+  const const_i32_t *cdocs = (const const_i32_t *)p.c_docs;
+  double *prod = reinterpret_cast<double *>(thb + kChunkDocs * kThetaRow);
+  auto load_theta = [&](const int d0, const int d1, double (&tv)[kChunkDocs][NT]) {
+    const double *t0 = p.theta + (size_t)d0 * K, *t1 = p.theta + (size_t)d1 * K;
+#pragma unroll
+    for (int t = 0; t < NT; ++t) {
+      tv[0][t] = (t * 64 + lane < K) ? t0[t * 64 + lane] : 0.0;
+      tv[1][t] = (t * 64 + lane < K) ? t1[t * 64 + lane] : 0.0;
+    }
+  };
+  const int64_t C = p.num_chunks;
+  int64_t c = p.num_cold + wid;
+  if (c >= C) return;
+  int w0 = p.ct_tok[c * 64 + lane], id0 = p.ct_idx[c * 64 + lane], ip0 = p.ct_ip[c * 64 + lane];
+  double tv0[kChunkDocs][NT];
+  load_theta(cdocs[2 * c], cdocs[2 * c + 1], tv0);
+  for (;;) {
+    const bool has1 = c + stride < C;
+    int w1 = 0, id1 = -1, ip1 = 0;
+    double tv1[kChunkDocs][NT];
+    if (has1) {
+      const int64_t c1 = c + stride;
+      w1 = p.ct_tok[c1 * 64 + lane]; id1 = p.ct_idx[c1 * 64 + lane]; ip1 = p.ct_ip[c1 * 64 + lane];
+      load_theta(cdocs[2 * c1], cdocs[2 * c1 + 1], tv1);
+    } else {
+      load_theta(0, 0, tv1);
+    }
+#pragma unroll
+    for (int r = 0; r < kChunkDocs; ++r)
+#pragma unroll
+      for (int t = 0; t < NT; ++t)
+        if (t * 64 + lane < KMAX) reinterpret_cast<float *>(thb + r * kThetaRow)[t * 64 + lane] = phi32_of(tv0[r][t]);
+    const unsigned char *trow = thb + ((unsigned)w0 >> kSlotShift) * kThetaRow;
+    const unsigned char *hrow = table + (w0 & ((1 << kSlotShift) - 1)) * p.hot_pitch;
+    float a[KMAX];
+    float acc = 0.0f;
+#pragma unroll
+    for (int u = 0; u < KMAX / 4; ++u) {
+      const f4_t ph = *reinterpret_cast<const f4_t *>(hrow + u * 16), th = *reinterpret_cast<const f4_t *>(trow + u * 16);
+      const f2_t q0 = f2_t{th.x, th.y} * f2_t{ph.x, ph.y};
+      const f2_t q1 = f2_t{th.z, th.w} * f2_t{ph.z, ph.w};
+      acc += q0.x; a[4 * u] = acc;
+      acc += q0.y; a[4 * u + 1] = acc;
+      acc += q1.x; a[4 * u + 2] = acc;
+      acc += q1.y; a[4 * u + 3] = acc;
+    }
+    finish32<KMAX>(p, a, prod, c, id0, ip0, w0, p.hot_words, lane);
+    if (!has1) break;
+    c += stride;
+    w0 = w1; id0 = id1; ip0 = ip1;
+#pragma unroll
+    for (int r = 0; r < kChunkDocs; ++r)
+#pragma unroll
+      for (int t = 0; t < NT; ++t) tv0[r][t] = tv1[r][t];
   }
 }
 
@@ -284,11 +356,14 @@
   const int64_t wid = (int64_t)blockIdx.x * kSlicedWaves + wave;
 
   {
-    constexpr int upr = KMAX / 2;
+    const bool t32 = F32 && p.table32;
+    const int upr = t32 ? KMAX / 4 : KMAX / 2;
+    const unsigned char *src = t32 ? reinterpret_cast<const unsigned char *>(p.phiT32) : phib;
+    const size_t srcrow = t32 ? (size_t)p.Kp32 * 4 : rowbytes;
     for (int i = threadIdx.x; i < p.num_hot * upr; i += kSlicedWaves * 64) {
       const int r = i / upr, u = i - r * upr;
       *reinterpret_cast<D2 *>(smem + p.hot_off + r * p.hot_pitch + u * 16) =
-          *reinterpret_cast<const D2 *>(phib + (size_t)p.hot_words[r] * rowbytes + (size_t)u * 16);
+          *reinterpret_cast<const D2 *>(src + (size_t)p.hot_words[r] * srcrow + (size_t)u * 16);
     }
   }
   __syncthreads();
@@ -511,9 +586,14 @@
 
 #pragma unroll 1
   for (int phase = 0; phase < 2; ++phase) {
-    if ((phase ^ wave) & 1) hot_chunks();
-    else if constexpr (F32) cold_chunks32<KMAX>(p, thb, ring, wid, stride, lane);
-    else cold_chunks();
+    if constexpr (F32) {
+      if (!((phase ^ wave) & 1)) cold_chunks32<KMAX>(p, thb, ring, wid, stride, lane);
+      else if (p.table32) hot_chunks32<KMAX>(p, smem + p.hot_off, thb, wid, stride, lane);
+      else hot_chunks();
+    } else {
+      if ((phase ^ wave) & 1) hot_chunks();
+      else cold_chunks();
+    }
   }
 }
 
@@ -522,10 +602,10 @@
 template <int KMAX>
 __global__ __launch_bounds__(kSlicedWaves * 64) void z_sliced32_kernel(ZParams p) { z_sliced_body<KMAX, true>(p); }
 
-template <int KMAX>
+template <int KMAX, int ES = 8>
 __device__ __forceinline__ void load_phi_table(unsigned char *table, const int pitch, const unsigned char *phib, const size_t rowbytes,
                                                const int32_t *words_g, const int nrows, const int wave, const int lane, const int tid) {
-  constexpr int upr = KMAX / 2 + 1, kRowsAhead = 6, NP = (upr + 63) / 64;
+  constexpr int upr = KMAX * ES / 16 + 1, kRowsAhead = 6, NP = (upr + 63) / 64;
   const const_i32_t *words = (const const_i32_t *)words_g;
   for (int r0 = wave; r0 < nrows; r0 += kSlicedWaves * kRowsAhead) {
     D2 v[kRowsAhead][NP];
@@ -638,6 +718,85 @@
   return new_topic;
 }
 
+constexpr int kCk32Topics = 16;
+template <int KMAX, int UB>
+__device__ __forceinline__ int hot_token32(const ZParams &p, const int K, const unsigned char *hrow, const unsigned char *trow, const int id0,
+                                           double &U, bool &undecided) {
+  constexpr int NU = KMAX / 4;
+  constexpr int UC = kCk32Topics / 4;
+  constexpr int NC = (NU + UC - 1) / UC;
+  f2_t acc = {0.0f, 0.0f};
+  float ck[NC];
+  static_for<0, (NU + UB - 1) / UB>([&](auto bidx) {
+    constexpr int u0 = decltype(bidx)::value * UB;
+    f4_t ph[UB], th[UB];
+#pragma unroll
+    for (int u = 0; u < UB; ++u)
+      if (u0 + u < NU) {
+        ph[u] = *reinterpret_cast<const f4_t *>(hrow + (u0 + u) * 16);
+        th[u] = *reinterpret_cast<const f4_t *>(trow + (u0 + u) * 16);
+      }
+#pragma unroll
+    for (int u = 0; u < UB; ++u)
+      if (u0 + u < NU) {
+        acc += f2_t{th[u].x, th[u].y} * f2_t{ph[u].x, ph[u].y};
+        acc += f2_t{th[u].z, th[u].w} * f2_t{ph[u].z, ph[u].w};
+        if ((u0 + u) % UC == UC - 1 || u0 + u == NU - 1) ck[(u0 + u) / UC] = acc.x + acc.y;
+      }
+    asm volatile("" : "+v"(acc) : : "memory");
+  });
+  const float A = ck[NC - 1];
+  const uint64_t gtok = (uint64_t)(p.tok_base + id0);
+  const U4 o = philox4x32_10((uint32_t)gtok, (uint32_t)(gtok >> 32), (uint32_t)GGS_PURPOSE_Z << 24, p.iteration,
+                             (uint32_t)p.seed, (uint32_t)(p.seed >> 32));
+  U = u53(o.x, o.y);
+  const float t0 = (float)(U * (double)A);
+  const float delta = ((float)(2 * K + 8) * 0x1p-24f * A) * (float)p.margin_scale;
+  int g = 0;
+#pragma unroll
+  for (int b = 0; b < NC; ++b) g += ck[b] < t0;
+  undecided = g >= NC;
+  if (undecided) g = NC - 1;
+  float a = 0.0f;
+#pragma unroll
+  for (int b = 0; b + 1 < NC; ++b)
+    if (g == b + 1) a = ck[b];
+  float m = fabsf(a - t0);
+  uint32_t bits = 0;
+  {
+    const unsigned char *hs = hrow + g * (UC * 16), *ts = trow + g * (UC * 16);
+    f4_t ph[UC], th[UC];
+#pragma unroll
+    for (int u = 0; u < UC; ++u) {
+      const bool past = NU % UC != 0 && u == NU % UC + 1 && g == NC - 1;
+      ph[u] = *reinterpret_cast<const f4_t *>(past ? hrow + NU * 16 : hs + u * 16);
+      th[u] = *reinterpret_cast<const f4_t *>(ts + u * 16);
+    }
+    const f2_t nt0 = {-t0, -t0};
+#pragma unroll
+    for (int u = 0; u < UC; ++u) {
+      const f2_t q0 = f2_t{th[u].x, th[u].y} * f2_t{ph[u].x, ph[u].y};
+      const f2_t q1 = f2_t{th[u].z, th[u].w} * f2_t{ph[u].z, ph[u].w};
+      f2_t s;
+      a += q0.x; s.x = a;
+      a += q0.y; s.y = a;
+      f2_t d = s + nt0;
+      bits = __builtin_amdgcn_alignbit(bits, __float_as_uint(d.x), 31);
+      bits = __builtin_amdgcn_alignbit(bits, __float_as_uint(d.y), 31);
+      m = fminf(m, fminf(fabsf(d.x), fabsf(d.y)));
+      a += q1.x; s.x = a;
+      a += q1.y; s.y = a;
+      d = s + nt0;
+      bits = __builtin_amdgcn_alignbit(bits, __float_as_uint(d.x), 31);
+      bits = __builtin_amdgcn_alignbit(bits, __float_as_uint(d.y), 31);
+      m = fminf(m, fminf(fabsf(d.x), fabsf(d.y)));
+    }
+  }
+  const int n = __popc(bits), new_topic = g * kCk32Topics + n;
+  undecided |= !(A >= 0x1p-60f && A <= 0x1.fffffep127f && m > delta && n < kCk32Topics && new_topic < K);
+  return new_topic;
+}
+
 typedef int i3v_t __attribute__((ext_vector_type(3)));
 typedef int i4v_t __attribute__((ext_vector_type(4)));
 template <int N>
@@ -646,12 +805,13 @@
                : "=&v"(w), "=&v"(id), "=&v"(ip) : "v"(e.x), "v"(e.y), "v"(e.z), "n"(N) : "memory");
 }
 
-template <int KMAX, int DOCS, int PAD, int UB>
+template <int KMAX, int DOCS, int PAD, int UB, bool F32 = false>
 __device__ __forceinline__ void table_chunks(const ZParams &p, unsigned char *smem, unsigned char *thb, const int4 *pack, const int32_t *docs_g,
-                                             const int64_t first, const int64_t C, const int64_t stride, const int lane, const int32_t *count_words) {
+                                             const int64_t first, const int64_t C, const int64_t stride, const int lane, const int32_t *count_words,
+                                             const int32_t *row_words = nullptr) {
   constexpr int NS = (KMAX + kSliceTopics - 1) / kSliceTopics;
   constexpr int kRowD = NS * kSliceTopics;
-  constexpr int kThetaRow = kRowD * 8 + PAD;
+  constexpr int kThetaRow = kRowD * (F32 ? 4 : 8) + PAD;
   constexpr int NQ = (kRowD + 127) / 128;
   constexpr int kLoads = 1 + DOCS * NQ;
   constexpr int kStores = 2;
@@ -691,13 +851,45 @@
         if (2 * (q * 64 + lane) < kRowD) {
           const int k0 = 2 * (q * 64 + lane);
           const D2 v = __builtin_bit_cast(D2, S.t[r][q]);
-          *reinterpret_cast<D2 *>(thb + r * kThetaRow + k0 * 8) = D2{k0 < K ? v.a : 0.0, k0 + 1 < K ? v.b : 0.0};
+          if constexpr (F32) {
+            double va = k0 < K ? v.a : 0.0, vb = k0 + 1 < K ? v.b : 0.0;
+            asm volatile("" : "+v"(va), "+v"(vb));
+            *reinterpret_cast<f2_t *>(thb + r * kThetaRow + k0 * 4) = f2_t{phi32_of(va), phi32_of(vb)};
+          } else {
+            *reinterpret_cast<D2 *>(thb + r * kThetaRow + k0 * 8) = D2{k0 < K ? v.a : 0.0, k0 + 1 < K ? v.b : 0.0};
+          }
         }
     if (c + 2 * stride < C) issue(c + 2 * stride, S);
     const int row = w0 & ((1 << kWarmSlotShift) - 1);
     const unsigned char *trow = thb + ((unsigned)w0 >> kWarmSlotShift) * kThetaRow;
     const unsigned char *hrow = smem + p.hot_off + row * p.hot_pitch;
-    if (id0 >= 0) {
+    if constexpr (F32) {
+      int new_topic = 0;
+      double U = 0.0;
+      bool undecided = false, id0_done = false;
+      if (id0 >= 0) new_topic = hot_token32<KMAX, UB>(p, K, hrow, trow, id0, U, undecided);
+      uint64_t pend = __ballot(undecided);
+      if (pend) {
+        if (p.replays && lane == 0) atomicAdd(p.replays + 1, (unsigned long long)__popcll(pend));
+        const int doc = undecided ? cdocs[c * kWarmDocSlots + ((unsigned)w0 >> kWarmSlotShift)] : 0;
+        const int word = undecided ? row_words[row] : 0;
+        uint32_t base = 0;
+        if (lane == 0) base = atomicAdd(p.replay_count, (uint32_t)__popcll(pend));
+        const uint32_t slot = (uint32_t)__builtin_amdgcn_readfirstlane((int)base) + (uint32_t)__popcll(pend & (((uint64_t)1 << lane) - 1));
+        const bool listed = undecided && slot < (uint32_t)p.replay_cap;
+        if (listed) p.replay_list[slot] = int4{id0, ip0, word | (count_words ? 1 << kSlotShift : 0), doc};
+        undecided = undecided && !listed;
+        pend = __ballot(undecided);
+        if (pend) replay_exact(p, reinterpret_cast<double *>(thb), pend, word, doc, U, lane, new_topic);
+        if (listed) id0_done = true;
+      }
+      if (id0 >= 0 && !id0_done) {
+        p.z[id0] = new_topic;
+        p.zw[ip0] = new_topic;
+        if (count_words)
+          __hip_atomic_fetch_add(&p.cnt_send[slice_cell(p.smap, new_topic, count_words[row])], 1, __ATOMIC_RELAXED, __HIP_MEMORY_SCOPE_AGENT);
+      }
+    } else if (id0 >= 0) {
       const int new_topic = hot_token<KMAX, UB>(p, K, hrow, trow, id0);
       p.z[id0] = new_topic;
       p.zw[ip0] = new_topic;
@@ -757,4 +949,84 @@
   }
 }
 
-}
+template <int KMAX>
+__global__ __launch_bounds__(kSlicedWaves * 64) __attribute__((amdgpu_waves_per_eu(4, 4))) void z_hot32_kernel(ZParams p) {
+  extern __shared__ __align__(16) unsigned char smem[];
+  __builtin_amdgcn_s_setprio(3);
+  const int lane = threadIdx.x & 63, wave = __builtin_amdgcn_readfirstlane(threadIdx.x >> 6);
+  unsigned char *thb = smem + wave * p.wave_lds;
+  load_phi_table<KMAX, 4>(smem + p.hot_off, p.hot_pitch, reinterpret_cast<const unsigned char *>(p.phiT32), (size_t)p.Kp32 * 4, p.hot_words, p.num_hot, wave, lane, threadIdx.x);
+  __syncthreads();
+  table_chunks<KMAX, kChunkDocs, kWarmThetaPad, (KMAX <= 128 ? kSliceUnits : kSliceUnits / 2), true>(
+      p, smem, thb, p.ht_pack, p.h_docs, (int64_t)blockIdx.x * kSlicedWaves + wave, p.num_chunks - p.num_cold, (int64_t)gridDim.x * kSlicedWaves, lane, nullptr, p.hot_words);
+}
+
+template <int KMAX>
+__global__ __launch_bounds__(kSlicedWaves * 64) __attribute__((amdgpu_waves_per_eu(4, 4))) void z_warm32_kernel(ZParams p) {
+  extern __shared__ __align__(16) unsigned char smem[];
+  __builtin_amdgcn_s_setprio(3);
+  const int lane = threadIdx.x & 63, wave = __builtin_amdgcn_readfirstlane(threadIdx.x >> 6);
+  unsigned char *thb = smem + wave * p.wave_lds;
+  const const_i64_t *meta = (const const_i64_t *)p.warm_meta;
+  const int64_t stride = (int64_t)gridDim.x * kSlicedWaves;
+  const int64_t wid = (int64_t)blockIdx.x * kSlicedWaves + wave;
+  for (int tier = 0; tier < p.warm_tiers; ++tier) {
+    if (tier) __syncthreads();
+    const int32_t *words = p.warm_words + (size_t)tier * p.warm_rows;
+    load_phi_table<KMAX, 4>(smem + p.hot_off, p.hot_pitch, reinterpret_cast<const unsigned char *>(p.phiT32), (size_t)p.Kp32 * 4, words, (int)meta[p.warm_tiers + 1 + tier], wave, lane, threadIdx.x);
+    __syncthreads();
+    table_chunks<KMAX, warm_docs_for(KMAX), kWarmThetaPad, GGS_WARM_UNITS, true>(p, smem, thb, p.wt_pack, p.w_docs, meta[tier] + wid, meta[tier + 1], stride, lane,
+                                                                                p.cnt_send ? words : nullptr, words);
+  }
+}
+
+__global__ __launch_bounds__(256) void z_replay_kernel(ZParams p) {
+  const int K = p.K;
+  const uint32_t listed = *p.replay_count, n = listed < (uint32_t)p.replay_cap ? listed : (uint32_t)p.replay_cap;
+  for (uint32_t i = blockIdx.x * blockDim.x + threadIdx.x; i < n; i += gridDim.x * blockDim.x) {
+    const int4 e = p.replay_list[i];
+    const int word = e.z & ((1 << kSlotShift) - 1);
+    const uint64_t gtok = (uint64_t)(p.tok_base + e.x);
+    const U4 o = philox4x32_10((uint32_t)gtok, (uint32_t)(gtok >> 32), (uint32_t)GGS_PURPOSE_Z << 24, p.iteration,
+                               (uint32_t)p.seed, (uint32_t)(p.seed >> 32));
+    const double U = u53(o.x, o.y);
+    const double *th = p.theta + (size_t)e.w * K, *ph = p.phiT + (size_t)word * p.Kp;
+    auto batch = [&](const int kb, double (&q)[8]) {
+      double a[8], b[8];
+#pragma unroll
+      for (int j = 0; j < 8; ++j) { const bool in = kb + j < K; a[j] = in ? th[kb + j] : 0.0; b[j] = in ? ph[kb + j] : 0.0; }
+#pragma unroll
+      for (int j = 0; j < 8; ++j) q[j] = a[j] * b[j];
+    };
+    double sum = 0.0;
+    for (int kb = 0; kb < K; kb += 8) {
+      double q[8];
+      batch(kb, q);
+#pragma unroll
+      for (int j = 0; j < 8; ++j) sum += q[j];
+    }
+    double sample = U * sum;
+    int nt = -1;
+    bool live = true;
+    for (int kb = 0; live; kb += 8) {
+      double q[8];
+      batch(kb, q);
+#pragma unroll
+      for (int j = 0; j < 8; ++j)
+        if (live) {
+          if (!(sample > 0.0)) live = false;
+          else if (++nt >= K) live = false;
+          else sample -= q[j];
+        }
+    }
+    if (nt < 0 || nt >= K) {
+      atomicOr(p.status, ST_INVALID_TOPIC);
+      nt = nt < 0 ? 0 : K - 1;
+    }
+    p.z[e.x] = nt;
+    p.zw[e.y] = nt;
+    if (p.cnt_send && (e.z >> kSlotShift)) __hip_atomic_fetch_add(&p.cnt_send[slice_cell(p.smap, nt, word)], 1, __ATOMIC_RELAXED, __HIP_MEMORY_SCOPE_AGENT);
+  }
+}
+
+}
```

Result: slower. 15870 (-2.6%).
